# lukifer23/Matrix0

Hardware: AMD Instinct MI355X
Metric: self-play games/sec at 800 sims/move, ResNet-24 53M; 1/2/4/8 MI355X (higher is better)
Workload: dtype f16

## Files before the change

### include/m0_engine.h

```cpp
#ifndef M0_ENGINE_H
#define M0_ENGINE_H

#include <stddef.h>
#include <stdint.h>

#ifdef __cplusplus
extern "C" {
#endif

#define M0_OK 0
#define M0_ERR_INVALID (-1)
#define M0_ERR_UNSUPPORTED (-2)
#define M0_ERR_HIP (-3)
#define M0_ERR_STATE (-4)
#define M0_ERR_NONFINITE (-5)

#define M0_POLICY_SIZE 4672
#define M0_PLANES 19

#define M0_ACT_RELU 1
#define M0_ACT_SILU 2
#define M0_ACT_LEAKY 3

#define M0_SSL_PIECE 1
// ... 109 lines not shown
typedef struct m0_selfplay_stats {
    uint64_t steps, evals, sims, plies, games_finished, games_started;
    double ms_total, ms_net, ms_tree, ms_host;
    uint64_t arena_overflows;
    uint64_t ssl_dropped;
    uint64_t evals_cached;
    int active_games;
    uint64_t rows_tail;
} m0_selfplay_stats;

typedef struct m0_game_record {
    int game_index, moves, resigned, resigner , draw, total_plies ;
    float result;
    float avg_policy_entropy, avg_sims;
    double secs;
    const float* s;
    const float* pi;
    const float* z;
    const uint8_t* legal_mask;
    const float* search_values;
    const uint16_t* played;
    const float* ssl;
    void* owner;
    const char* start_fen;
} m0_game_record;

m0_selfplay* m0_selfplay_create(m0_net* net, const m0_selfplay_cfg* cfg);
void m0_selfplay_destroy(m0_selfplay* sp);
int m0_selfplay_step(m0_selfplay* sp, int steps);
int m0_selfplay_stats_get(m0_selfplay* sp, m0_selfplay_stats* out);
int m0_selfplay_poll(m0_selfplay* sp, m0_game_record* out);
void m0_game_record_free(m0_game_record* rec);
int m0_selfplay_running(m0_selfplay* sp);
int m0_selfplay_set_openings(m0_selfplay* sp, const char* const* fens, int n);
int m0_selfplay_ext_select(m0_selfplay* sp, int* rows, float* planes, int max_rows);
int m0_selfplay_ext_expand(m0_selfplay* sp, const float* logits, const float* values, int rows);
int m0_selfplay_last_batch_nhwc(m0_selfplay* sp, uint16_t* nhwc, int max_rows, int* rows);

m0_selfplay* m0_arena_create(m0_net* net_a, m0_net* net_b, const m0_selfplay_cfg* cfg);
m0_selfplay* m0_arena_create_ext(const m0_selfplay_cfg* cfg);
int m0_arena_ext_select(m0_selfplay* sp, int* rows_a, int* rows_b, float* planes_a, float* planes_b, int max_rows);
int m0_arena_ext_expand(m0_selfplay* sp, const float* logits_a, const float* values_a, int rows_a, const float* logits_b,
                        const float* values_b, int rows_b);
int m0_arena_choose_move(const int32_t* visits, int n, double temp, int ply, int temp_plies, double u);
int m0_san_legal_fen(const char* fen, uint16_t* moves, char* san, int* nlegal);
int m0_san_game(const uint16_t* moves, int n, char* out, int cap);
int m0_san_game_fen(const char* fen, const uint16_t* moves, int n, char* out, int cap);
int m0_fen_after(const char* fen, const char* const* ucis, int n, char* fen_out, int cap);

int m0_search_begin(m0_selfplay* sp, int g, const char* fen, int sims, int dirichlet, int game_uid);
int m0_search_select(m0_selfplay* sp, int* rows, float* planes, int max_rows);
int m0_search_expand(m0_selfplay* sp, const float* logits, const float* values, int rows);
int m0_search_result(m0_selfplay* sp, int g, int* nchild, int32_t* child_n, uint16_t* child_mv, int32_t* child_idx,
                     double* child_prior, double* child_q, double* root_q, int* root_n, int* finished);
int m0_search_advance(m0_selfplay* sp, int g, int slot, int sims, int dirichlet);


#define M0_AN_MAX_LINES 8
#define M0_AN_MAX_PV    16
typedef struct m0_analysis_opts { int multipv, pv_len, dirichlet; } m0_analysis_opts;
typedef struct m0_analysis_line {
    uint16_t move; int32_t policy_index; int32_t visits; float prior; double q;
    int32_t pv_len; uint16_t pv[M0_AN_MAX_PV];
} m0_analysis_line;
typedef struct m0_analysis_result {
    int64_t id; int32_t status;
    int32_t nlegal, overflow, sims, root_n; uint64_t evals;
    float value;
    double root_q; int32_t nlines; m0_analysis_line lines[M0_AN_MAX_LINES];
    int32_t tb_dtm;
    int32_t line_dtm[M0_AN_MAX_LINES];
} m0_analysis_result;
m0_selfplay* m0_analysis_create(m0_net* net, const m0_selfplay_cfg* cfg, const m0_analysis_opts* opts);
m0_selfplay* m0_analysis_create_ext(const m0_selfplay_cfg* cfg, const m0_analysis_opts* opts);
int m0_analysis_submit(m0_selfplay* sp, const char* fen, const char* const* ucis, int n_moves, int sims, int64_t id);
int m0_analysis_step(m0_selfplay* sp, int steps);
int m0_analysis_ext_select(m0_selfplay* sp, int* rows, float* planes, int max_rows);
int m0_analysis_ext_expand(m0_selfplay* sp, const float* logits, const float* values, int rows);
int m0_analysis_poll(m0_selfplay* sp, m0_analysis_result* out);
int m0_analysis_pending(m0_selfplay* sp);
size_t m0_analysis_result_size(void);

#define M0_DECODE_OK 0
#define M0_DECODE_PIECE_VALUE 1
#define M0_DECODE_SQUARE_CLASH 2
#define M0_DECODE_KINGS 3
#define M0_DECODE_PAWN_RANK 4
#define M0_DECODE_NOT_UNIFORM 5
#define M0_DECODE_FLAG_VALUE 6
#define M0_DECODE_CASTLING 7
#define M0_DECODE_COUNTER 8
#define M0_DECODE_OPPONENT_IN_CHECK 9
#define M0_DECODE_TOO_MANY_MOVES 10
#define M0_DECODE_MASK_MISMATCH 11
#define M0_DECODE_HALFMOVE_SATURATED 1
#define M0_DECODE_FULLMOVE_SATURATED 2
#define M0_DECODE_EP_FROM_MASK 4
#define M0_DECODE_NO_MASK 8
int m0_decode_planes(int hip_device, const float* planes, const uint8_t* mask, int n, int32_t* status, int32_t* flags,
                     int32_t* nlegal, char* fens, int fen_stride);
int m0_analysis_submit_planes(m0_selfplay* sp, const float* planes, const uint8_t* mask, int n, int sims, const int64_t* ids,
                              int32_t* status, int32_t* flags);
int m0_analysis_keep_visits(m0_selfplay* sp, int on);
int m0_analysis_poll_visits(m0_selfplay* sp, m0_analysis_result* out, int32_t* nchild, int32_t* policy_idx, int32_t* visits,
                            int cap);

typedef struct m0_tb m0_tb;
m0_tb* m0_tb_build(int hip_device, int max_men);
m0_tb* m0_tb_build_signatures(int hip_device, const char* const* sigs, int n);
m0_tb* m0_tb_load(const char* path);
int m0_tb_save(const m0_tb* tb, const char* path);
void m0_tb_destroy(m0_tb* tb);
int m0_tb_max_men(const m0_tb* tb);
int m0_tb_table(const m0_tb* tb, const char* sig, const uint8_t** bytes, size_t* n);
int m0_tb_table_info(const m0_tb* tb, int i, char* sig8, int* maxd, int* sweeps, double* build_ms);
int m0_tb_probe_fens(const m0_tb* tb, const char* const* fens, int n, uint8_t* hit, int8_t* wdl, int16_t* dtm);
int m0_selfplay_set_tablebase(m0_selfplay* sp, const m0_tb* tb, int max_pieces);
uint64_t m0_selfplay_tb_adjudications(m0_selfplay* sp);
int m0_selfplay_set_search_tablebase(m0_selfplay* sp, const m0_tb* tb, int max_pieces);
uint64_t m0_selfplay_tb_leaves(m0_selfplay* sp);
int m0_tb_root_lines(const m0_tb* tb, const char* fen, int multipv, int pv_len, m0_analysis_result* out);

int m0_sample_move_index(const int32_t* visits, int n, double temperature, double u);
int m0_playout_cap(int sims, double frac, double u);
double m0_temperature_for(int fullmove_number, double t_start, double t_end, int t_moves);
int m0_rules_probe(const m0_selfplay_cfg* cfg, const char* fen, const char* const* ucis, int n, int* flags, float* result);

int m0_san_pattern(const char* token, uint32_t* pattern);
#define M0_MOVE_UCI 0
#define M0_MOVE_RAW 1
int m0_move_pattern(int kind, const char* uci, uint32_t raw, uint32_t* pattern);
#define M0_REPLAY_OK 0
#define M0_REPLAY_ILLEGAL 1
#define M0_REPLAY_AMBIGUOUS 2
#define M0_REPLAY_TOO_LONG 3
#define M0_REPLAY_END_CHECKMATE 1
#define M0_REPLAY_END_STALEMATE 2
#define M0_REPLAY_END_INSUFFICIENT 4
#define M0_REPLAY_END_WHITE_TO_MOVE 8
int m0_replay_games(int hip_device, const char* const* start_fens, const uint32_t* patterns, const int32_t* offsets, int n_games,
                    int max_plies, int max_positions_per_launch, int32_t* plies, int32_t* status, int32_t* end_flags,
                    uint16_t* moves, int32_t* policy_idx, int32_t* nlegal, int8_t* turn, float* planes, uint8_t* mask, float* ssl);

#ifdef __cplusplus
}
#endif
#include "m0_analysis_live.h"
#include "m0_score.h"
#include "m0_ssl_score.h"
#include "m0_gumbel.h"
#include "m0_augment.h"
#include "m0_proof.h"
#include "m0_rowpack.h"
#endif
```

### matrix0_amd/_abi.py

```python
from __future__ import annotations

import ctypes as C
from ctypes import POINTER as P

M0_OK = 0
M0_ERR_INVALID = -1
M0_ERR_UNSUPPORTED = -2
M0_ERR_HIP = -3
M0_ERR_STATE = -4
M0_ERR_NONFINITE = -5
POLICY_SIZE = 4672
ACT = {"relu": 1, "silu": 2, "leaky_relu": 3}
SSL_BITS = {"piece": 1, "threat": 2, "pin": 4, "fork": 8, "control": 16}
AN_MAX_LINES, AN_MAX_PV = 8, 16
DECODE_STATUS = {0: "ok", 1: "piece_value", 2: "square_clash", 3: "kings", 4: "pawn_rank", 5: "not_uniform", 6: "flag_value",
                 7: "castling", 8: "counter", 9: "opponent_in_check", 10: "too_many_moves", 11: "mask_mismatch"}
DECODE_OK, DECODE_MASK_MISMATCH = 0, 11
HALFMOVE_SATURATED, FULLMOVE_SATURATED, EP_FROM_MASK, NO_MASK = 1, 2, 4, 8
REPLAY_STATUS = {0: "ok", 1: "illegal", 2: "ambiguous", 3: "too_long"}
REPLAY_END_BITS = {"checkmate": 1, "stalemate": 2, "insufficient": 4, "white_to_move": 8}
MOVE_UCI, MOVE_RAW = 0, 1
SCORE_MASK = {"legal": 0, "target": 1, "none": 2}
SCORE_COLS = 8
SCORE_COLUMNS = ("policy_loss", "entropy", "value_loss", "rank", "support_mass", "support_size", "value", "flags")
# ... 106 lines not shown
STRUCTS = {"m0_net_cfg": NetCfg, "m0_selfplay_cfg": SelfplayCfg, "m0_selfplay_stats": SelfplayStats,
           "m0_game_record": GameRecord, "m0_analysis_opts": AnalysisOpts, "m0_analysis_line": AnalysisLine,
           "m0_analysis_result": AnalysisResult}

_cfg, _res, _pi32 = P(SelfplayCfg), P(AnalysisResult), P(i32)
_select = (i32, [vp, _pi32, vp, i32])
_expand = (i32, [vp, vp, vp, i32])
_attach = (i32, [vp, vp, i32])
FUNCTIONS = {
    "m0_last_error": (cstr, []),
    "m0_version": (cstr, []),
    "m0_device_count": (i32, []),
    "m0_net_create": (vp, [P(NetCfg), i32]),
    "m0_net_destroy": (None, [vp]),
    "m0_net_load_weight": (i32, [vp, cstr, vp, i32, P(i64), i32]),
    "m0_net_finalize": (i32, [vp]),
    "m0_net_infer": (i32, [vp, vp, i32, vp, vp, vp]),
    "m0_net_tap_info": (i32, [vp, _pi32, _pi32]),
    "m0_net_infer_tap": (i32, [vp, vp, i32, i32, vp, vp, vp, vp, vp, _pi32]),
    "m0_net_ssl_channels": (i32, [vp]),
    "m0_net_param_count": (i64, [vp]),
    "m0_net_flops_per_position": (f64, [vp, i32]),
    "m0_net_bench_forward": (i32, [vp, i32, i32, i32, P(f32)]),
    "m0_net_profile_enable": (i32, [vp, i32]),
    "m0_net_profile_get": (i32, [vp, P(f64), P(f64), P(i64), i32]),
    "m0_net_profile_get_tail": (i32, [vp, P(f64), P(i64)]),
    "m0_dist_unique_id": (i32, [vp]),
    "m0_dist_create": (vp, [i32, i32, cstr, i32]),
    "m0_dist_destroy": (None, [vp]),
    "m0_dist_rank": (i32, [vp]),
    "m0_dist_world": (i32, [vp]),
    "m0_net_broadcast_weights": (i32, [vp, vp, i32]),
    "m0_encode_fens": (i32, [i32, cstrs, i32, vp, vp, vp, vp, vp]),
    "m0_encode_fens_nhwc": (i32, [i32, cstrs, i32, vp]),
    "m0_decode_move_fen": (i32, [i32, cstr, i32, cstr]),
    "m0_ssl_targets_fens": (i32, [i32, cstrs, i32, vp]),
    "m0_move_to_index_fen": (i32, [i32, cstr, cstr, _pi32]),
    "m0_selfplay_create": (vp, [vp, _cfg]),
    "m0_selfplay_destroy": (None, [vp]),
    "m0_selfplay_step": (i32, [vp, i32]),
    "m0_selfplay_stats_get": (i32, [vp, P(SelfplayStats)]),
    "m0_selfplay_poll": (i32, [vp, P(GameRecord)]),
    "m0_game_record_free": (None, [P(GameRecord)]),
    "m0_selfplay_running": (i32, [vp]),
    "m0_selfplay_set_openings": (i32, [vp, cstrs, i32]),
    "m0_selfplay_ext_select": _select,
    "m0_selfplay_ext_expand": _expand,
    "m0_selfplay_last_batch_nhwc": (i32, [vp, vp, i32, _pi32]),
    "m0_arena_create": (vp, [vp, vp, _cfg]),
    "m0_arena_create_ext": (vp, [_cfg]),
    "m0_arena_ext_select": (i32, [vp, _pi32, _pi32, vp, vp, i32]),
    "m0_arena_ext_expand": (i32, [vp, vp, vp, i32, vp, vp, i32]),
    "m0_arena_choose_move": (i32, [vp, i32, f64, i32, i32, f64]),
    "m0_san_legal_fen": (i32, [cstr, vp, vp, _pi32]),
    "m0_san_game": (i32, [vp, i32, cstr, i32]),
    "m0_san_game_fen": (i32, [cstr, vp, i32, cstr, i32]),
    "m0_fen_after": (i32, [cstr, cstrs, i32, cstr, i32]),
    "m0_search_begin": (i32, [vp, i32, cstr, i32, i32, i32]),
    "m0_search_select": _select,
    "m0_search_expand": _expand,
    "m0_search_result": (i32, [vp, i32, _pi32, vp, vp, vp, vp, vp, P(f64), _pi32, _pi32]),
    "m0_search_advance": (i32, [vp, i32, i32, i32, i32]),
    "m0_analysis_create": (vp, [vp, _cfg, P(AnalysisOpts)]),
    "m0_analysis_create_ext": (vp, [_cfg, P(AnalysisOpts)]),
    "m0_analysis_submit": (i32, [vp, cstr, cstrs, i32, i32, i64]),
    "m0_analysis_step": (i32, [vp, i32]),
    "m0_analysis_ext_select": _select,
    "m0_analysis_ext_expand": _expand,
    "m0_analysis_poll": (i32, [vp, _res]),
    "m0_analysis_pending": (i32, [vp]),
    "m0_analysis_result_size": (C.c_size_t, []),
    "m0_decode_planes": (i32, [i32, vp, vp, i32, vp, vp, vp, cstr, i32]),
    "m0_analysis_submit_planes": (i32, [vp, vp, vp, i32, i32, vp, vp, vp]),
    "m0_analysis_keep_visits": (i32, [vp, i32]),
    "m0_analysis_poll_visits": (i32, [vp, _res, _pi32, vp, vp, i32]),
    "m0_tb_build": (vp, [i32, i32]),
    "m0_tb_build_signatures": (vp, [i32, cstrs, i32]),
    "m0_tb_load": (vp, [cstr]),
    "m0_tb_save": (i32, [vp, cstr]),
    "m0_tb_destroy": (None, [vp]),
    "m0_tb_max_men": (i32, [vp]),
    "m0_tb_table": (i32, [vp, cstr, P(P(u8)), P(C.c_size_t)]),
    "m0_tb_table_info": (i32, [vp, i32, cstr, _pi32, _pi32, P(f64)]),
    "m0_tb_probe_fens": (i32, [vp, cstrs, i32, vp, vp, vp]),
    "m0_selfplay_set_tablebase": _attach,
    "m0_selfplay_tb_adjudications": (u64, [vp]),
    "m0_selfplay_set_search_tablebase": _attach,
    "m0_selfplay_tb_leaves": (u64, [vp]),
    "m0_tb_root_lines": (i32, [vp, cstr, i32, i32, _res]),
    "m0_sample_move_index": (i32, [vp, i32, f64, f64]),
    "m0_playout_cap": (i32, [i32, f64, f64]),
    "m0_temperature_for": (f64, [i32, f64, f64, i32]),
    "m0_rules_probe": (i32, [_cfg, cstr, cstrs, i32, _pi32, P(f32)]),
    "m0_san_pattern": (i32, [cstr, P(u32)]),
    "m0_move_pattern": (i32, [i32, cstr, u32, P(u32)]),
    "m0_replay_games": (i32, [i32, cstrs, vp, vp, i32, i32, i32] + [vp] * 10),
}

LIVE_FUNCTIONS = {
    "m0_analysis_submit_keep": (i32, [vp, cstr, cstrs, i32, i32, i64]),
    "m0_analysis_peek": (i32, [vp, i64, _res]),
    "m0_analysis_stop": (i32, [vp, i64]),
    "m0_analysis_continue": (i32, [vp, i64, cstrs, i32, i32, i64, i32, _pi32]),
    "m0_analysis_release": (i32, [vp, i64]),
    "m0_analysis_held": (i32, [vp]),
}

SCORE_STRUCTS = {"m0_score_opts": ScoreOpts}
SCORE_FUNCTIONS = {
    "m0_score_rows": (i32, [i32, vp, vp, vp, vp, vp, i32, P(ScoreOpts), vp]),
    "m0_net_score": (i32, [vp, vp, vp, vp, vp, i32, P(ScoreOpts), vp]),
    "m0_score_bench": (i32, [i32, i32, i32, P(f32), P(f64)]),
}

SSL_SCORE_FUNCTIONS = {
    "m0_ssl_score_rows": (i32, [i32, vp, i32, vp, vp, i32, vp]),
    "m0_net_score_ssl": (i32, [vp, vp, vp, vp, vp, vp, i32, P(ScoreOpts), vp, vp]),
    "m0_ssl_targets_planes": (i32, [i32, vp, i32, vp, vp]),
    "m0_ssl_score_bench": (i32, [i32, i32, i32, i32, i32, P(f32), P(f64)]),
}

GUMBEL_STRUCTS = {"m0_gumbel_cfg": GumbelCfg}
GUMBEL_FUNCTIONS = {
    "m0_selfplay_set_gumbel": (i32, [vp, P(GumbelCfg)]),
    "m0_search_gumbel_result": (i32, [vp, i32, _pi32, P(f64), vp, vp, _pi32]),
    "m0_gumbel_schedule": (i32, [i32, i32, vp, vp]),
    "m0_gumbel_improve": (i32, [i32, vp, vp, vp, vp, f64, P(GumbelCfg), vp, P(f64), _pi32]),
}

AUGMENT_FUNCTIONS = {
    "m0_augment_rows": (i32, [i32, vp, i32, vp, vp, vp, i32, vp, vp, vp]),
    "m0_net_score_aug": (i32, [vp, vp, vp, vp, vp, vp, i32, P(ScoreOpts), vp]),
    "m0_augment_bench": (i32, [i32, i32, i32, P(f32), P(f64)]),
}

PROOF_STRUCTS = {"m0_proof_lines": ProofLines}
PROOF_FUNCTIONS = {
    "m0_selfplay_set_proof": (i32, [vp, i32]),
    "m0_search_proof_result": (i32, [vp, i32, _pi32, _pi32, vp, vp, _pi32]),
    "m0_analysis_last_proof": (i32, [vp, P(ProofLines)]),
    "m0_proof_combine": (i32, [i32, vp, vp, i32, _pi32, _pi32]),
}

ROWPACK_STRUCTS = {"m0_rowpack_pos": RowpackPos, "m0_rowpack_arrays": RowpackArrays}
ROWPACK_FUNCTIONS = {
    "m0_rowpack_pack": (i32, [i32, vp, vp, vp, vp, i32, P(RowpackArrays), vp]),
    "m0_rowpack_unpack": (i32, [i32, P(RowpackArrays), vp, vp, vp, vp]),
    "m0_rowpack_pack_host": (i32, [vp, vp, vp, vp, i32, P(RowpackArrays), vp]),
    "m0_rowpack_unpack_host": (i32, [P(RowpackArrays), vp, vp, vp, vp]),
    "m0_net_score_packed": (i32, [vp, P(RowpackArrays), P(ScoreOpts), vp]),
    "m0_rowpack_bench": (i32, [i32, i32, i32, P(f32), P(f32), P(f64)]),
}


def bind(L) -> list:
    missing = []
    for name, (restype, argtypes) in (list(FUNCTIONS.items()) + list(LIVE_FUNCTIONS.items()) + list(SCORE_FUNCTIONS.items()) +
                                      list(SSL_SCORE_FUNCTIONS.items()) + list(GUMBEL_FUNCTIONS.items()) +
                                      list(AUGMENT_FUNCTIONS.items()) + list(PROOF_FUNCTIONS.items()) +
                                      list(ROWPACK_FUNCTIONS.items())):
        fn = getattr(L, name, None)
        if fn is None:
            missing.append(name)
        else:
            fn.restype, fn.argtypes = restype, argtypes
    return missing
```

### matrix0_amd/backend.py

```python
from __future__ import annotations

import ctypes as C
import threading
from typing import Dict, Optional, Tuple

import numpy as np

from . import _abi, _lib


def resolve_mask_mode(pi: np.ndarray, legal_mask, mask_mode: Optional[str]) -> str:
    if mask_mode is not None:
        if mask_mode not in _abi.SCORE_MASK:
            raise ValueError(f"mask_mode must be one of {sorted(_abi.SCORE_MASK)} or None, got {mask_mode!r}")
        return mask_mode
    if legal_mask is not None:
        return "legal"
    return "none" if bool(((np.asarray(pi) > 0).sum(axis=1) == 1).all()) else "target"


class NonFiniteScore(ValueError):

    def __init__(self, msg: str, rows: np.ndarray, ssl_rows: Optional[np.ndarray] = None):
        super().__init__(msg)
# ... 36 lines not shown
        b.load_state_dict(sd)
        return b

    @classmethod
    def from_checkpoint(cls, model_cfg: dict, ckpt_path: str, device_index: int = 0) -> "M0Backend":
        import torch
        state = torch.load(ckpt_path, map_location="cpu", weights_only=False)
        sd = state
        if isinstance(state, dict):
            for key in ("model_ema", "model", "model_state_dict"):
                if key in state and isinstance(state[key], dict):
                    sd = state[key]
                    break
        return cls.from_state_dict(model_cfg, sd, device_index)

    def infer_np(self, arr: np.ndarray) -> Tuple[np.ndarray, np.ndarray]:
        p, v, _ = self._infer(arr, False)
        return p, v

    def infer_np_ssl(self, arr: np.ndarray):
        return self._infer(arr, True)

    def tap_info(self) -> Tuple[int, int]:
        steps, width = C.c_int(0), C.c_int(0)
        _lib.check(self._L.m0_net_tap_info(self._h, C.byref(steps), C.byref(width)), "m0_net_tap_info")
        return steps.value, width.value

    def infer_tap(self, arr: np.ndarray, step: int):
        return self._infer(arr, True, int(step))

    def _infer(self, arr: np.ndarray, want_ssl: bool, tap_step: Optional[int] = None):
        if not self._finalized:
            raise RuntimeError("weights not loaded")
        a = np.asarray(arr)
        if a.ndim == 3:
            a = a[None]
        if a.ndim != 4 or a.shape[1:] != (self._cfg.planes, 8, 8):
            raise ValueError(f"expected input [B,{self._cfg.planes},8,8], got {a.shape}")
        a = np.ascontiguousarray(a, dtype=np.float32)
        B = a.shape[0]
        pol = np.empty((B, _lib.POLICY_SIZE), dtype=np.float32)
        val = np.empty((B,), dtype=np.float32)
        sslc = self._L.m0_net_ssl_channels(self._h)
        ssl = np.empty((B, sslc, 8, 8), dtype=np.float32) if (want_ssl and sslc > 0) else None
        if tap_step is None:
            _lib.check(self._L.m0_net_infer(self._h, _lib.ptr(a), B, _lib.ptr(pol), _lib.ptr(val), _lib.ptr(ssl)), "m0_net_infer")
        else:
            width = self.tap_info()[1]
            stream = np.empty((B, 64, width), dtype=np.float32)
            second = np.empty((B, 64, width), dtype=np.float32)
            has_second = C.c_int(0)
            _lib.check(self._L.m0_net_infer_tap(self._h, _lib.ptr(a), B, tap_step, _lib.ptr(pol), _lib.ptr(val), _lib.ptr(ssl),
                                                _lib.ptr(stream), _lib.ptr(second), C.byref(has_second)), "m0_net_infer_tap")
        out = None
        if ssl is not None:
            out, off = {}, 0
            for t in self.ssl_tasks:
                n = _lib.SSL_CH[t]
                out[t] = ssl[:, off:off + n]
                off += n
        if tap_step is not None:
            return pol, val, out, stream, (second if has_second.value else None)
        return pol, val, out

    def _score_inputs(self, s, pi, z, legal_mask):
        if not self._finalized:
            raise RuntimeError("weights not loaded")
        a = np.ascontiguousarray(s, dtype=np.float32)
        if a.ndim != 4 or a.shape[1:] != (self._cfg.planes, 8, 8):
            raise ValueError(f"expected input [B,{self._cfg.planes},8,8], got {a.shape}")
        B = a.shape[0]
        pi = np.ascontiguousarray(pi, dtype=np.float32)
        z = np.ascontiguousarray(np.asarray(z).reshape(-1), dtype=np.float32)
        if pi.shape != (B, _lib.POLICY_SIZE) or z.shape != (B,):
            raise ValueError(f"expected pi [{B},{_lib.POLICY_SIZE}] and z [{B}], got {pi.shape} and {z.shape}")
        if legal_mask is not None:
            legal_mask = np.ascontiguousarray(np.asarray(legal_mask).reshape(B, -1), dtype=np.uint8)
            if legal_mask.shape != pi.shape:
                raise ValueError(f"expected legal_mask [{B},{_lib.POLICY_SIZE}], got {legal_mask.shape}")
        return a, pi, z, legal_mask

    def score(self, s: Optional[np.ndarray] = None, pi: Optional[np.ndarray] = None, z: Optional[np.ndarray] = None,
              legal_mask: Optional[np.ndarray] = None, *, mask_mode: Optional[str] = None, label_smoothing: float = 0.0,
              value_loss: str = "mse", huber_delta: float = 1.0, augment=None, packed=None) -> np.ndarray:
        if packed is not None:
            return self._score_packed(packed, mask_mode, label_smoothing, value_loss, huber_delta, s, pi, z, legal_mask, augment)
        if s is None or pi is None or z is None:
            raise ValueError("score needs s, pi and z, or packed rows")
        a, pi, z, legal_mask = self._score_inputs(s, pi, z, legal_mask)
        B = a.shape[0]
        opts = score_opts(resolve_mask_mode(pi, legal_mask, mask_mode), label_smoothing, value_loss, huber_delta)
        rows = np.empty((B, _abi.SCORE_COLS), dtype=np.float32)
        if augment is None:
            call = "m0_net_score"
            rc = self._L.m0_net_score(self._h, _lib.ptr(a), _lib.ptr(pi), _lib.ptr(z), _lib.ptr(legal_mask), B, C.byref(opts),
                                      _lib.ptr(rows))
        else:
            from .encoding import augment_kinds
            call = "m0_net_score_aug"
            kinds = augment_kinds(augment, B)
            rc = self._L.m0_net_score_aug(self._h, _lib.ptr(a), _lib.ptr(pi), _lib.ptr(z), _lib.ptr(legal_mask), _lib.ptr(kinds), B,
                                          C.byref(opts), _lib.ptr(rows))
        if rc == _lib.M0_ERR_NONFINITE:
            raise NonFiniteScore(f"{call} failed ({rc}): {_lib.last_error()}", rows)
        _lib.check(rc, call)
        return rows

    def _score_packed(self, packed, mask_mode, label_smoothing, value_loss, huber_delta, *dense) -> np.ndarray:
        if not self._finalized:
            raise RuntimeError("weights not loaded")
        if any(d is not None for d in dense):
            raise ValueError("packed rows come instead of s, pi, z and legal_mask, and are not augmented")
        from .rowpack import mask_mode_of
        opts = score_opts(resolve_mask_mode(None, None, mask_mode_of(packed, mask_mode)), label_smoothing, value_loss, huber_delta)
        rows = np.empty((packed.n, _abi.SCORE_COLS), dtype=np.float32)
        arrays = packed.c_arrays()
        rc = self._L.m0_net_score_packed(self._h, C.byref(arrays), C.byref(opts), _lib.ptr(rows))
        if rc == _lib.M0_ERR_NONFINITE:
            raise NonFiniteScore(f"m0_net_score_packed failed ({rc}): {_lib.last_error()}", rows)
        _lib.check(rc, "m0_net_score_packed")
        return rows

    def score_ssl(self, s: np.ndarray, pi: np.ndarray, z: np.ndarray, legal_mask: Optional[np.ndarray] = None,
                  ssl_targets: Optional[np.ndarray] = None, *, mask_mode: Optional[str] = None, label_smoothing: float = 0.0,
                  value_loss: str = "mse", huber_delta: float = 1.0) -> Tuple[np.ndarray, np.ndarray]:
        a, pi, z, legal_mask = self._score_inputs(s, pi, z, legal_mask)
        B = a.shape[0]
        if ssl_targets is not None:
            ssl_targets = np.ascontiguousarray(ssl_targets, dtype=np.float32)
            if ssl_targets.size != B * 17 * 64 or ssl_targets.shape[:2] != (B, 17):
                raise ValueError(f"expected ssl_targets [{B},17,8,8], got {ssl_targets.shape}")
        opts = score_opts(resolve_mask_mode(pi, legal_mask, mask_mode), label_smoothing, value_loss, huber_delta)
        rows = np.empty((B, _abi.SCORE_COLS), dtype=np.float32)
        ssl_rows = np.empty((B, _abi.SSL_SCORE_COLS), dtype=np.float32)
        rc = self._L.m0_net_score_ssl(self._h, _lib.ptr(a), _lib.ptr(pi), _lib.ptr(z), _lib.ptr(legal_mask), _lib.ptr(ssl_targets),
                                      B, C.byref(opts), _lib.ptr(rows), _lib.ptr(ssl_rows))
        if rc == _lib.M0_ERR_NONFINITE:
            raise NonFiniteScore(f"m0_net_score_ssl failed ({rc}): {_lib.last_error()}", rows, ssl_rows)
        _lib.check(rc, "m0_net_score_ssl")
        return rows, ssl_rows

    def param_count(self) -> int:
        return int(self._L.m0_net_param_count(self._h))

    def flops_per_position(self, with_ssl: bool = False) -> float:
        return float(self._L.m0_net_flops_per_position(self._h, int(with_ssl)))

    def bench_forward(self, batch: int, iters: int, with_ssl: bool = False) -> float:
        ms = C.c_float(0)
        _lib.check(self._L.m0_net_bench_forward(self._h, int(batch), int(iters), int(with_ssl), C.byref(ms)),
                   "m0_net_bench_forward")
        return float(ms.value)

    def profile_enable(self, on: bool = True) -> None:
        _lib.check(self._L.m0_net_profile_enable(self._h, int(on)), "m0_net_profile_enable")

    def profile_get(self, reset: bool = False):
        ms, fl, n = C.c_double(0), C.c_double(0), C.c_int64(0)
        tms, tn = C.c_double(0), C.c_int64(0)
        _lib.check(self._L.m0_net_profile_get_tail(self._h, C.byref(tms), C.byref(tn)), "m0_net_profile_get_tail")
        self.last_tail_profile = (tms.value, tn.value)
        _lib.check(self._L.m0_net_profile_get(self._h, C.byref(ms), C.byref(fl), C.byref(n), int(reset)), "m0_net_profile_get")
        return ms.value, fl.value, n.value

    @property
    def handle(self):
        return self._h

    def close(self):
        if getattr(self, "_h", None):
            self._L.m0_net_destroy(self._h)
            self._h = None

    def __del__(self):
        try:
            self.close()
        except Exception:
            pass
```

### matrix0_amd/csrc/capi_net.hip

```cpp
#include <hip/hip_runtime.h>
#include <limits.h>
#include <math.h>
#include <string.h>
#include <mutex>
#include <string>
#include <vector>
#include "../../include/m0_engine.h"
#include "net.h"
#include "capi_common.h"
#include "score_core.h"
#include "score_kernels.h"
#include "ssl_score_core.h"
#include "ssl_score_kernels.h"
#include "augment_kernels.h"

thread_local std::string g_m0_last_error;

void m0_set_error(const std::string& s) { g_m0_last_error = s; }

struct m0_net {
    Net* net = nullptr;
    int device = 0;
    hipStream_t stream = nullptr;
    std::mutex mu;
// ... 272 lines not shown
        M0_HIP(hs, hipMemcpyAsync(n->score_pi_dev, pi, cells * 4, hipMemcpyHostToDevice, n->stream));
        M0_HIP(hs, hipMemcpyAsync(n->score_z_dev, z, (size_t)B * 4, hipMemcpyHostToDevice, n->stream));
        if (masked) M0_HIP(hs, hipMemcpyAsync(n->score_mask_dev, legal_mask, cells, hipMemcpyHostToDevice, n->stream));
    }
    if (ssl_rows && ssl_targets)
        M0_HIP(hs, hipMemcpyAsync(n->ssl_targets_dev, ssl_targets, (size_t)B * m0ssl::TARGET_CH * 64 * 4, hipMemcpyHostToDevice, n->stream));
    if (augmented) M0_HIP(hs, hipMemcpyAsync(n->aug_kinds_dev, kinds, (size_t)B, hipMemcpyHostToDevice, n->stream));
    if (!hs.ok()) return m0_hip_error(hs, "H2D copy");
    const float* planes_in = n->planes_dev;
    const float* pi_in = n->score_pi_dev;
    const uint8_t* mask_in = masked ? n->score_mask_dev : nullptr;
    if (augmented) {
        if (!M0_HIP(hs, launch_augment_rows(planes_in, pi_in, mask_in, n->aug_kinds_dev, M0_AUG_NONE, B, n->net->cfg().planes,
                                            n->aug_planes_dev, n->aug_pi_dev, masked ? n->aug_mask_dev : nullptr, n->stream)))
            return m0_hip_error(hs, "augment kernel");
        planes_in = n->aug_planes_dev;
        pi_in = n->aug_pi_dev;
        if (masked) mask_in = n->aug_mask_dev;
    }
    std::string err;
    rc = n->net->forward(planes_in, nullptr, B, n->logits_dev, n->value_dev, ssl_rows ? n->ssl_dev : nullptr, n->stream, err);
    if (rc != M0_OK) { m0_set_error(err); return rc; }
    M0_HIP(hs, launch_score_rows(n->logits_dev, n->value_dev, pi_in, n->score_z_dev, mask_in, B, *opts, n->score_rows_dev, n->stream));
    M0_HIP(hs, hipMemcpyAsync(rows, n->score_rows_dev, (size_t)B * M0_SCORE_COLS * 4, hipMemcpyDeviceToHost, n->stream));
    if (ssl_rows) {
        M0_HIP(hs, launch_ssl_score(n->ssl_dev, tasks, n->planes_dev, ssl_targets ? n->ssl_targets_dev : nullptr, B, n->ssl_rows_dev,
                                    n->stream));
        M0_HIP(hs, hipMemcpyAsync(ssl_rows, n->ssl_rows_dev, (size_t)B * M0_SSL_SCORE_COLS * 4, hipMemcpyDeviceToHost, n->stream));
    }
    if (!M0_HIP(hs, hipStreamSynchronize(n->stream))) return m0_hip_error(hs, "forward and score failed");
    for (int b = 0; b < B; ++b)
        if (((int)rows[(size_t)b * M0_SCORE_COLS + 7] & M0_SCORE_FLAG_NONFINITE) ||
            (ssl_rows && ((int)ssl_rows[(size_t)b * M0_SSL_SCORE_COLS + 15] & M0_SSL_SCORE_FLAG_NONFINITE))) {
            m0_set_error("network produced non-finite outputs (row " + std::to_string(b) + ")");
            return M0_ERR_NONFINITE;
        }
    return M0_OK;
}

int m0_net_score(m0_net* n, const float* planes, const float* pi, const float* z, const uint8_t* legal_mask, int B,
                 const m0_score_opts* opts, float* rows) {
    return net_score(n, planes, pi, z, legal_mask, nullptr, nullptr, false, B, opts, rows, nullptr);
}

int m0_net_score_packed(m0_net* n, const m0_rowpack_arrays* in, const m0_score_opts* opts, float* rows) {
    if (!in || !in->pos || !in->z || in->n <= 0 || in->n > INT_MAX) { m0_set_error("invalid argument"); return M0_ERR_INVALID; }
    return net_score(n, nullptr, nullptr, in->z, nullptr, nullptr, nullptr, false, (int)in->n, opts, rows, nullptr, in);
}

int m0_net_score_aug(m0_net* n, const float* planes, const float* pi, const float* z, const uint8_t* legal_mask, const uint8_t* kinds,
                     int B, const m0_score_opts* opts, float* rows) {
    return net_score(n, planes, pi, z, legal_mask, nullptr, kinds, true, B, opts, rows, nullptr);
}

int m0_net_score_ssl(m0_net* n, const float* planes, const float* pi, const float* z, const uint8_t* legal_mask,
                     const float* ssl_targets, int B, const m0_score_opts* opts, float* rows, float* ssl_rows) {
    if (!ssl_rows) { m0_set_error("null argument"); return M0_ERR_INVALID; }
    return net_score(n, planes, pi, z, legal_mask, ssl_targets, nullptr, false, B, opts, rows, ssl_rows);
}

int m0_net_tap_info(const m0_net* n, int* steps, int* width) {
    if (!n || !steps || !width) { m0_set_error("null argument"); return M0_ERR_INVALID; }
    *steps = n->net->tap_steps();
    *width = n->net->trunk_width();
    return M0_OK;
}

int m0_net_infer_tap(m0_net* n, const float* planes, int B, int step, float* policy, float* value, float* ssl, float* stream,
                     float* second, int* has_second) {
    if (!n || !planes || !policy || !value || !stream || !second || !has_second) {
        m0_set_error("null argument");
        return M0_ERR_INVALID;
    }
    if (B <= 0) { m0_set_error("batch must be positive"); return M0_ERR_INVALID; }
    if (step < 0 || step >= n->net->tap_steps()) { m0_set_error("tap step out of range"); return M0_ERR_INVALID; }
    std::lock_guard<std::mutex> lk(n->mu);
    n->net->set_tap(step);
    const int rc = infer_locked(n, planes, B, policy, value, ssl, stream, second, has_second);
    n->net->set_tap(-1);
    return rc;
}

int m0_net_ssl_channels(const m0_net* n) { return n ? n->net->ssl_channels_total() : 0; }
int64_t m0_net_param_count(const m0_net* n) { return n ? (int64_t)n->net->param_count() : 0; }
double m0_net_flops_per_position(const m0_net* n, int with_ssl) { return n ? n->net->flops_per_position(with_ssl != 0) : 0.0; }

int m0_net_profile_enable(m0_net* n, int on) {
    if (!n) { m0_set_error("net is null"); return M0_ERR_INVALID; }
    std::lock_guard<std::mutex> lk(n->mu);
    n->net->set_profile(on != 0);
    return M0_OK;
}

int m0_net_profile_get(m0_net* n, double* conv_ms, double* conv_flop, int64_t* launches, int reset) {
    if (!n) { m0_set_error("net is null"); return M0_ERR_INVALID; }
    std::lock_guard<std::mutex> lk(n->mu);
    if (conv_ms) *conv_ms = n->net->prof_conv_ms();
    if (conv_flop) *conv_flop = n->net->prof_conv_flop();
    if (launches) *launches = n->net->prof_conv_launches();
    if (reset) n->net->reset_profile();
    return M0_OK;
}

int m0_net_profile_get_tail(m0_net* n, double* tail_ms, int64_t* tail_launches) {
    if (!n) { m0_set_error("net is null"); return M0_ERR_INVALID; }
    std::lock_guard<std::mutex> lk(n->mu);
    if (tail_ms) *tail_ms = n->net->prof_tail_ms();
    if (tail_launches) *tail_launches = n->net->prof_tail_launches();
    return M0_OK;
}

int m0_net_bench_forward(m0_net* n, int B, int iters, int with_ssl, float* ms_per_forward) {
    if (!n || !ms_per_forward || B <= 0 || iters <= 0) { m0_set_error("invalid argument"); return M0_ERR_INVALID; }
    std::lock_guard<std::mutex> lk(n->mu);
    HipStatus& hs = n->net->hip();
    if (!M0_HIP(hs, hipSetDevice(n->device))) return m0_hip_error(hs);
    int rc = ensure_io(n, B);
    if (rc != M0_OK) return rc;
    std::string err;
    if (!(with_ssl & 2)) {
        const int P = n->net->cfg().planes;
        std::vector<float> h((size_t)B * P * 64, 0.f);
        uint64_t s = 0x9E3779B97F4A7C15ull;
        for (size_t i = 0; i < h.size(); ++i) {
            s ^= s << 13; s ^= s >> 7; s ^= s << 17;
            int p = (int)((i / 64) % P);
            if (p < 12) h[i] = ((s >> 20) % 100) < 8 ? 1.f : 0.f;
            else h[i] = (float)((((i / 64 / P) * 7 + p) % 10) / 10.0);
        }
        if (!M0_HIP(hs, hipMemcpy(n->planes_dev, h.data(), h.size() * 4, hipMemcpyHostToDevice))) return m0_hip_error(hs, "H2D copy");
    }
    float* ssl = ((with_ssl & 1) && n->net->ssl_channels_total() > 0) ? n->ssl_dev : nullptr;
    rc = n->net->forward(n->planes_dev, nullptr, B, n->logits_dev, n->value_dev, ssl, n->stream, err);
    if (rc != M0_OK) { m0_set_error(err); return rc; }
    struct Events {
        hipEvent_t e0 = nullptr, e1 = nullptr;
        ~Events() { if (e0) (void)hipEventDestroy(e0); if (e1) (void)hipEventDestroy(e1); }
    } ev;
    M0_HIP(hs, hipEventCreate(&ev.e0)); M0_HIP(hs, hipEventCreate(&ev.e1));
    M0_HIP(hs, hipEventRecord(ev.e0, n->stream));
    for (int i = 0; i < iters && hs.ok(); ++i) {
        rc = n->net->forward(n->planes_dev, nullptr, B, n->logits_dev, n->value_dev, ssl, n->stream, err);
        if (rc != M0_OK) { m0_set_error(err); return rc; }
    }
    M0_HIP(hs, hipEventRecord(ev.e1, n->stream));
    M0_HIP(hs, hipEventSynchronize(ev.e1));
    float ms = 0.f;
    if (!M0_HIP(hs, hipEventElapsedTime(&ms, ev.e0, ev.e1))) return m0_hip_error(hs, "bench forward failed");
    *ms_per_forward = ms / iters;
    n->net->harvest_profile();
    return M0_OK;
}

}
```

### matrix0_amd/csrc/capi_selfplay.hip

```cpp
#include <string.h>
#include <algorithm>
#include <memory>
#include <vector>
#include "selfplay_engine.h"

using namespace m0;

static void fill_tree_cfg(const m0_selfplay_cfg& c, bool match, TreeCfg& t) {
    t.fpu_reduction = c.fpu_reduction; t.draw_penalty = c.draw_penalty; t.virtual_loss = c.virtual_loss;
    t.selection_jitter = c.selection_jitter; t.cpuct = c.cpuct; t.cpuct_start = c.cpuct_start; t.cpuct_end = c.cpuct_end;
    t.cpuct_plies = c.cpuct_plies; t.use_c_base = c.use_c_base; t.cpuct_c_base = c.cpuct_c_base; t.cpuct_c_init = c.cpuct_c_init;
    t.dirichlet_alpha = c.dirichlet_alpha; t.dirichlet_frac = c.dirichlet_frac; t.legal_softmax = c.legal_softmax;
    t.enable_entropy_noise = c.enable_entropy_noise; t.no_instant_backtrack = c.no_instant_backtrack;
    t.virtual_loss_active = c.virtual_loss_active; t.leaves_per_step = c.inference_batch_size;
    t.tt_merge = c.tt_merge; t.raw_legal_priors = c.raw_legal_priors; t.max_children = c.max_children;
    t.min_child_prior = c.min_child_prior;
    t.gumbel = 0;
    t.gumbel_cfg = m0_gumbel_cfg{0, 0.0, 0.0};
    t.proof = 0;
    t.eval_cache = ((match ? c.arena_eval_cache : c.eval_cache) && c.legal_softmax && !c.raw_legal_priors && !c.tt_merge) ? 1 : 0;
}

static bool alloc_tree_arenas(m0_selfplay* sp) {
    const m0_selfplay_cfg& c = sp->cfg;
    long want = c.arena_nodes > 0 ? c.arena_nodes : (long)(c.num_simulations * 1.3 + 64) * 96;
    if (want < 4096) want = 4096;
    sp->cap = (int)want;
    const size_t N = (size_t)sp->G * 2 * sp->cap;
    TreeArrays& t = sp->d.t;
    t.cap = sp->cap;
    t.prior = dalloc<double>(sp, N); t.w = dalloc<double>(sp, N); t.q = dalloc<double>(sp, N);
    t.n = dalloc<int>(sp, N); t.vl = dalloc<int>(sp, N); t.cbase = dalloc<int>(sp, N);
    t.nch = dalloc<int16_t>(sp, N); t.mv = dalloc<uint16_t>(sp, N); t.midx = dalloc<uint16_t>(sp, N);
    sp->d.games = dalloc<GameDev>(sp, sp->G);
    const size_t LS = (size_t)sp->L + 1;
    sp->d.samples = dalloc<Sample>(sp, (size_t)sp->G * LS);
    sp->d.paths = dalloc<int>(sp, (size_t)sp->G * LS * M0_MAX_DEPTH);
    sp->d.leaf_moves = dalloc<uint16_t>(sp, (size_t)sp->G * LS * M0_MAX_CHILDREN);
    return hip_ok(sp, "hipMalloc failed for the search arenas (lower concurrent_games or arena_nodes)");
}

static bool alloc_position_tables(m0_selfplay* sp) {
    sp->d.tt_sides = 1;
    if (!sp->cfg.tt_merge) return true;
    const size_t LS = (size_t)sp->L + 1;
    int tc = 1024;
    while (tc < 2 * sp->cap) tc <<= 1;
    sp->d.tt_cap = tc;
    sp->d.tt_sides = sp->kind == EngineKind::Match ? 2 : 1;
    sp->d.search_nodes = (int)std::min<long>((long)sp->cfg.num_simulations * 48 + 4 * M0_MAX_CHILDREN, (long)sp->cap / 2);
    sp->d.epaths = dalloc<int>(sp, (size_t)sp->G * LS * M0_MAX_DEPTH);
    sp->d.tt_keys = dalloc<uint64_t>(sp, (size_t)sp->G * sp->d.tt_sides * tc);
    sp->d.tt_nodes = dalloc<int>(sp, (size_t)sp->G * sp->d.tt_sides * tc);
    return hip_ok(sp, "hipMalloc failed for the position tables (tt_merge): lower concurrent_games or arena_nodes");
}

static bool alloc_eval_cache(m0_selfplay* sp) {
    if (!sp->tc.eval_cache) return true;
    const size_t LS = (size_t)sp->L + 1;
    int entries = sp->cfg.eval_cache_entries > 0 ? sp->cfg.eval_cache_entries : 16384;
    int sets = 64;
    while (sets * 4 < entries) sets <<= 1;
    EvalCache& ec = sp->d.ec;
    ec.sets = sets;
    ec.sides = sp->kind == EngineKind::Match ? 2 : 1;
    const size_t entries_all = (size_t)sp->G * ec.sides * sets * 4;
    ec.keys = dalloc<uint64_t>(sp, entries_all);
    ec.stamps = dalloc<uint32_t>(sp, entries_all);
    ec.payload = dalloc<float>(sp, entries_all * M0_EC_WORDS);
    ec.hit_stage = dalloc<float>(sp, (size_t)sp->G * LS * M0_EC_WORDS);
    return hip_ok(sp, "hipMalloc failed for the evaluation cache: lower eval_cache_entries or concurrent_games");
}

static bool alloc_batch_buffers(m0_selfplay* sp) {
    const int nreg = sp->kind == EngineKind::Match ? 2 : 1;
    sp->d.hist = dalloc<uint64_t>(sp, (size_t)sp->G * M0_HIST_CAP);
    sp->d.results = dalloc<RootResult>(sp, sp->G);
    sp->d.row_counter = dalloc<int>(sp, 4);
    sp->d.x0 = dalloc<_Float16>(sp, (size_t)(nreg * sp->rows_max + 4) * 64 * 32);
    sp->logits_dev = dalloc<float>(sp, (size_t)nreg * sp->rows_max * 4672);
    sp->values_dev = dalloc<float>(sp, (size_t)nreg * sp->rows_max + 4);
    sp->d.net_row_base = sp->rows_max;
    if (sp->cfg.ssl_in_forward && sp->net && sp->net->ssl_channels_total() > 0)
        sp->ssl_dev = dalloc<float>(sp, (size_t)sp->rows_max * sp->net->ssl_channels_total() * 64);
    if (sp->cfg.ssl_targets) {
        sp->ssl_cap = sp->cfg.max_game_len > 0 ? sp->cfg.max_game_len + 1 : 513;
        sp->ssl_pos_dev = dalloc<Pos>(sp, sp->ssl_cap);
        sp->ssl_out_dev = dalloc<float>(sp, (size_t)sp->ssl_cap * 17 * 64);
        if (!hip_ok(sp, "hipMalloc failed for the SSL target staging buffers")) return false;
    }
    sp->ids_dev = dalloc<int>(sp, sp->G);
    sp->roots_dev = dalloc<int>(sp, sp->G);
    sp->d.logits = sp->logits_dev; sp->d.values = sp->values_dev;
    sp->d.G = sp->G; sp->d.L = sp->L;
    return hip_ok(sp, "hipMalloc failed for the batch buffers (lower concurrent_games or inference_batch_size)");
}

static bool make_tail_view(m0_selfplay* sp) {
    if (!(sp->cfg.tail_split && sp->net && sp->kind != EngineKind::Match && sp->net->cfg().channels > 256 && sp->net->cfg().channels <= 320 &&
          sp->rows_max >= 2048)) return true;
    M0_HIP(sp->hip, create_stream_cu_mask_env("M0_TAIL_CU_MASK", &sp->stream_tail));
    M0_HIP(sp->hip, hipEventCreateWithFlags(&sp->ev_sel, hipEventDisableTiming));
    M0_HIP(sp->hip, hipEventCreateWithFlags(&sp->ev_tail, hipEventDisableTiming));
    if (!hip_ok(sp, "hipStreamCreate / hipEventCreate failed (tail split)")) return false;
    sp->net_tail = sp->net->shared_view(sp->stream_tail);
    std::string werr;
    sp->half_split = sp->cfg.tail_split == 2;
    if (sp->net_tail->ensure_workspace(sp->half_split ? sp->rows_max / 2 + 1024 : 1023, werr) != M0_OK) {
        m0_set_error("tail split: " + werr);
        return false;
    }
    return true;
}

static bool build_engine(m0_selfplay* sp) {
    if (!alloc_tree_arenas(sp) || !alloc_position_tables(sp) || !alloc_eval_cache(sp) || !alloc_batch_buffers(sp)) return false;
    sp->hg.assign(sp->G, GameDev());
    for (auto& g : sp->hg) memset(&g, 0, sizeof(GameDev));
    sp->games.assign(sp->G, HostGame());
    sp->hres.resize(sp->G);
    sp->hsamples.resize((size_t)sp->G * (sp->L + 1));
    sp->prev_done.assign(sp->G, 0);
    for (hipEvent_t* e : {&sp->ev0, &sp->ev1, &sp->ev2, &sp->ev3}) M0_HIP(sp->hip, hipEventCreate(e));
    if (!hip_ok(sp, "hipEventCreate failed") || !make_tail_view(sp)) return false;
    std::string err;
    if (sp->net && sp->net->ensure_workspace(sp->rows_max, err) != M0_OK) { m0_set_error(err); return false; }
    if (sp->net && sp->net_b && sp->net_b->ensure_workspace(sp->rows_max, err) != M0_OK) { m0_set_error(err); return false; }
    M0_HIP(sp->hip, hipStreamSynchronize(sp->stream));
    return hip_ok(sp, "clearing the search arenas failed");
}

m0_selfplay* m0::engine_create(m0_net* nh, m0_net* nh_b, const m0_selfplay_cfg* cfg, EngineKind kind) {
    if (!cfg) { m0_set_error("cfg is null"); return nullptr; }
    if (cfg->concurrent_games <= 0 || cfg->inference_batch_size <= 0 || cfg->num_simulations <= 0) {
        m0_set_error("concurrent_games, inference_batch_size and num_simulations must be positive");
        return nullptr;
    }
    int ndev = 0;
    if (hipGetDeviceCount(&ndev) != hipSuccess || ndev <= 0) { m0_set_error("no HIP device available (no CPU fallback)"); return nullptr; }
    std::unique_ptr<m0_selfplay, decltype(&m0_selfplay_destroy)> owner(new m0_selfplay(), &m0_selfplay_destroy);
    m0_selfplay* sp = owner.get();
    sp->cfg = *cfg;
    sp->nethandle = nh;
    sp->nethandle_b = nh_b;
    sp->net = m0_net_impl(nh);
    sp->net_b = m0_net_impl(nh_b);
    sp->kind = kind;
    const bool match = kind == EngineKind::Match;
    sp->cfg.arena_mode = match ? 1 : 0;
    if (match) sp->cfg.eval_cache = 0;
    else { sp->cfg.arena_eval_cache = 0; sp->cfg.arena_paired_openings = 0; }
    fill_tree_cfg(sp->cfg, match, sp->tc);
    sp->device = nh ? m0_net_device(nh) : 0;
    if (nh) forward_gate_join(sp);
    M0_HIP(sp->hip, hipSetDevice(sp->device));
    if (nh) sp->stream = m0_net_stream(nh);
    else { M0_HIP(sp->hip, hipStreamCreateWithFlags(&sp->stream, hipStreamNonBlocking)); sp->own_stream = true; }
    sp->G = cfg->concurrent_games;
    sp->L = cfg->inference_batch_size;
    sp->rows_max = (sp->G * (sp->L + 1) + 3) & ~3;
    memset(&sp->stats, 0, sizeof(sp->stats));
    memset(&sp->d, 0, sizeof(sp->d));
    return hip_ok(sp, "engine stream") && build_engine(sp) ? owner.release() : nullptr;
}

static int leaf_planes(m0_selfplay* sp, int rows_a, float* planes_a, int rows_b, float* planes_b) {
    sync_games_d2h(sp);
    if (!M0_HIP(sp->hip, hipMemcpy(sp->hsamples.data(), sp->d.samples, sizeof(Sample) * (size_t)sp->G * (sp->L + 1), hipMemcpyDeviceToHost)))
        return m0_hip_error(sp->hip, "device sync failed");
    const int base = sp->d.net_row_base;
    for (int g = 0; g < sp->G; ++g) {
        if (!sp->hg[g].active) continue;
        for (int s = 0; s < sp->hg[g].nsamples; ++s) {
            const Sample& smp = sp->hsamples[(size_t)g * (sp->L + 1) + s];
            if (!sample_owns_row(smp.kind) || smp.row < 0) continue;
            if (smp.row < rows_a) encode_planes_f32(smp.pos, planes_a + (size_t)smp.row * 19 * 64);
            else if (smp.row >= base && smp.row < base + rows_b) encode_planes_f32(smp.pos, planes_b + (size_t)(smp.row - base) * 19 * 64);
        }
    }
    return M0_OK;
}

static void upload_eval(m0_selfplay* sp, size_t row_base, const float* logits, const float* values, int rows) {
    if (rows <= 0) return;
    M0_HIP(sp->hip, hipMemcpyAsync(sp->logits_dev + row_base * 4672, logits, (size_t)rows * 4672 * 4, hipMemcpyHostToDevice, sp->stream));
    M0_HIP(sp->hip, hipMemcpyAsync(sp->values_dev + row_base, values, (size_t)rows * 4, hipMemcpyHostToDevice, sp->stream));
}

int m0::ext_select_impl(m0_selfplay* sp, int* rows_a, int* rows_b, float* planes_a, float* planes_b, int max_rows) {
    if (sp->ext_pending) { m0_set_error("m0_selfplay_ext_expand outstanding"); return M0_ERR_STATE; }
    if (!planes_a || (sp->kind == EngineKind::Match && !planes_b) || max_rows < sp->G * (sp->L + 1)) {
        m0_set_error("planes buffer too small: concurrent_games * (inference_batch_size + 1) rows are required");
        return M0_ERR_INVALID;
    }
    int rc = refill(sp);
    if (rc != M0_OK) return rc;
    int r = 0;
    if ((rc = run_select(sp, &r)) != M0_OK) return rc;
    const int rb = sp->kind == EngineKind::Match ? sp->rows2[1] : 0;
    if (r > sp->rows_max || rb > sp->rows_max) { m0_set_error("row counter overflow"); return M0_ERR_STATE; }
    *rows_a = r;
    if (rows_b) *rows_b = rb;
    sp->last_rows = r;
    sp->last_rows_b = rb;
    sp->ext_pending = true;
    if (r + rb > 0) return leaf_planes(sp, r, planes_a, rb, planes_b);
    return M0_OK;
}

int m0::ext_expand_impl(m0_selfplay* sp, const float* logits_a, const float* values_a, int rows_a, const float* logits_b,
                           const float* values_b, int rows_b) {
    if (!sp->ext_pending) { m0_set_error("no m0_selfplay_ext_select outstanding"); return M0_ERR_STATE; }
    if (rows_a != sp->last_rows || rows_b != sp->last_rows_b) { m0_set_error("rows does not match the last select"); return M0_ERR_INVALID; }
    if ((rows_a > 0 && (!logits_a || !values_a)) || (rows_b > 0 && (!logits_b || !values_b))) { m0_set_error("null argument"); return M0_ERR_INVALID; }
    upload_eval(sp, 0, logits_a, values_a, rows_a);
    upload_eval(sp, (size_t)sp->d.net_row_base, logits_b, values_b, rows_b);
    sp->ext_pending = false;
    M0_HIP(sp->hip, hipEventRecord(sp->ev0, sp->stream)); M0_HIP(sp->hip, hipEventRecord(sp->ev1, sp->stream));
    return finish_step(sp, rows_a + rows_b, now_ms());
}

bool m0::kind_accepted(const m0_selfplay* sp, const char* what, unsigned kinds) {
    if (kinds & (1u << (int)sp->kind)) return true;
    static const char* const is_a[] = {"a self-play engine", "a match engine", "an analysis engine"};
    const char* only = kinds == KIND_SELFPLAY ? "self-play engines" : kinds == KIND_MATCH ? "match engines"
                     : kinds == KIND_ANALYSIS ? "analysis engines" : "self-play and match engines";
    m0_set_error(std::string(what) + ": " + only + " only, this is " + is_a[(int)sp->kind]);
    return false;
}

extern "C" {

m0_selfplay* m0_selfplay_create(m0_net* nh, const m0_selfplay_cfg* cfg) { return engine_create(nh, nullptr, cfg, EngineKind::SelfPlay); }

m0_selfplay* m0_arena_create(m0_net* net_a, m0_net* net_b, const m0_selfplay_cfg* cfg) {
    if (!net_a || !net_b) { m0_set_error("m0_arena_create needs two networks"); return nullptr; }
    if (m0_net_device(net_a) != m0_net_device(net_b)) { m0_set_error("both networks must live on the same HIP device"); return nullptr; }
    if (cfg && (cfg->ssl_in_forward || cfg->ssl_targets)) { m0_set_error("arena games carry no SSL outputs"); return nullptr; }
    return engine_create(net_a, net_b, cfg, EngineKind::Match);
}

m0_selfplay* m0_arena_create_ext(const m0_selfplay_cfg* cfg) {
    if (cfg && (cfg->ssl_in_forward || cfg->ssl_targets)) { m0_set_error("arena games carry no SSL outputs"); return nullptr; }
    return engine_create(nullptr, nullptr, cfg, EngineKind::Match);
}

void m0_selfplay_destroy(m0_selfplay* sp) {
    if (!sp) return;
    forward_gate_leave(sp);
    (void)hipSetDevice(sp->device);
    if (sp->stream) (void)hipStreamSynchronize(sp->stream);
    if (sp->stream_tail) (void)hipStreamSynchronize(sp->stream_tail);
    delete sp->net_tail;
    if (sp->ev_sel) (void)hipEventDestroy(sp->ev_sel);
    if (sp->ev_tail) (void)hipEventDestroy(sp->ev_tail);
    if (sp->stream_tail) (void)hipStreamDestroy(sp->stream_tail);
    for (void* p : sp->allocs) (void)hipFree(p);
    for (auto& r : sp->done_meta) delete (GameRecordOwner*)r.owner;
    delete sp->an;
    if (sp->ev0) { (void)hipEventDestroy(sp->ev0); (void)hipEventDestroy(sp->ev1); (void)hipEventDestroy(sp->ev2); (void)hipEventDestroy(sp->ev3); }
    if (sp->own_stream && sp->stream) (void)hipStreamDestroy(sp->stream);
    delete sp;
}

int m0_selfplay_set_openings(m0_selfplay* sp, const char* const* fens, int n) {
    if (!sp || n < 0 || (n > 0 && !fens)) { m0_set_error("invalid argument"); return M0_ERR_INVALID; }
    M0_ENGINE_CALL(sp, "m0_selfplay_set_openings", KIND_GAMES, false);
    if (sp->stats.games_started != 0) { m0_set_error("set the opening book before the first step"); return M0_ERR_STATE; }
    std::vector<Pos> book(n);
    for (int i = 0; i < n; ++i)
        if (!fens[i] || parse_fen(fens[i], book[i]) != 0) { m0_set_error(std::string("bad FEN at index ") + std::to_string(i)); return M0_ERR_INVALID; }
    sp->book.swap(book);
    sp->book_fens.assign(fens, fens + n);
    return M0_OK;
}

int m0_selfplay_ext_select(m0_selfplay* sp, int* rows, float* planes, int max_rows) {
    if (!sp || !rows) { m0_set_error("null argument"); return M0_ERR_INVALID; }
    M0_ENGINE_CALL(sp, "m0_selfplay_ext_select", KIND_SELFPLAY, true);
    return ext_select_impl(sp, rows, nullptr, planes, nullptr, max_rows);
}

int m0_selfplay_ext_expand(m0_selfplay* sp, const float* logits, const float* values, int rows) {
    M0_ENGINE_CALL(sp, "m0_selfplay_ext_expand", KIND_SELFPLAY, true);
    return ext_expand_impl(sp, logits, values, rows, nullptr, nullptr, 0);
}

int m0_arena_ext_select(m0_selfplay* sp, int* rows_a, int* rows_b, float* planes_a, float* planes_b, int max_rows) {
    if (!sp || !rows_a || !rows_b) { m0_set_error("null argument"); return M0_ERR_INVALID; }
    M0_ENGINE_CALL(sp, "m0_arena_ext_select", KIND_MATCH, true);
    return ext_select_impl(sp, rows_a, rows_b, planes_a, planes_b, max_rows);
}

int m0_arena_ext_expand(m0_selfplay* sp, const float* logits_a, const float* values_a, int rows_a, const float* logits_b,
                        const float* values_b, int rows_b) {
    M0_ENGINE_CALL(sp, "m0_arena_ext_expand", KIND_MATCH, true);
    return ext_expand_impl(sp, logits_a, values_a, rows_a, logits_b, values_b, rows_b);
}

int m0_selfplay_step(m0_selfplay* sp, int steps) {
    M0_ENGINE_CALL(sp, "m0_selfplay_step", KIND_GAMES, true);
    if (sp->ext_pending) { m0_set_error("m0_selfplay_ext_expand outstanding"); return M0_ERR_STATE; }
    int rc = refill(sp);
    for (int i = 0; i < steps && rc == M0_OK; ++i) {
        if (sp->stats.active_games == 0 && sp->stats.steps > 0) break;
        rc = one_step(sp);
    }
    return rc;
}

int m0_selfplay_stats_get(m0_selfplay* sp, m0_selfplay_stats* out) {
    if (!sp || !out) { m0_set_error("null argument"); return M0_ERR_INVALID; }
    M0_ENGINE_CALL(sp, "m0_selfplay_stats_get", KIND_ANY, false);
    *out = sp->stats;
    return M0_OK;
}

int m0_selfplay_poll(m0_selfplay* sp, m0_game_record* out) {
    if (!sp || !out) { m0_set_error("null argument"); return M0_ERR_INVALID; }
    M0_ENGINE_CALL(sp, "m0_selfplay_poll", KIND_GAMES, false);
    if (sp->done_meta.empty()) return 0;
    *out = sp->done_meta.front();
    sp->done_meta.pop_front();
    return 1;
}

void m0_game_record_free(m0_game_record* rec) {
    if (rec && rec->owner) { delete (GameRecordOwner*)rec->owner; rec->owner = nullptr; }
}

int m0_selfplay_running(m0_selfplay* sp) {
    M0_ENGINE_CALL_OR(0, sp, "m0_selfplay_running", KIND_ANY, false);
    if (sp->stats.games_started == 0) return 1;
    if (sp->stats.active_games > 0) return 1;
    return (sp->cfg.total_games <= 0 || sp->next_game < sp->cfg.total_games) ? 1 : 0;
}

int m0_search_begin(m0_selfplay* sp, int g, const char* fen, int sims, int dirichlet, int game_uid) {
    if (!sp || !fen || g < 0 || g >= sp->G || sims <= 0) { m0_set_error("invalid argument"); return M0_ERR_INVALID; }
// ... 97 lines not shown
```

### matrix0_amd/csrc/conv_epilogue.h

```cpp
#pragma once
#include "kernel_common.h"

typedef _Float16 half2v __attribute__((ext_vector_type(2)));

template <int ACT>
__device__ __forceinline__ float act_fast(float v) {
    if constexpr (ACT == ACT_RELU) return v > 0.f ? v : 0.f;
    else if constexpr (ACT == ACT_SILU) return v * __builtin_amdgcn_rcpf(1.f + __expf(-v));
    else if constexpr (ACT == ACT_LEAKY) return v > 0.f ? v : 0.05f * v;
    else if constexpr (ACT == ACT_SIGMOID) return __builtin_amdgcn_rcpf(1.f + __expf(-v));
    else if constexpr (ACT == ACT_TANH) return tanhf(v);
    else return v;
}
template <int NT>
__device__ __forceinline__ char* conv_stage_base(char* lds_wave, int lane) {
    return lds_wave + (4 * (lane >> 5) + (lane & 1)) * (NT * 64) + ((lane & 31) >> 1) * 4;
}

template <int NT, int MI, int NI>
__device__ __forceinline__ void conv_stage_tile(const float (&v)[16], char* wbase, int lane) {
    constexpr int ROWB = NT * 64;
    const bool odd = (lane & 1) != 0;
    static_for<0, 8>([&](auto rp_) __attribute__((always_inline)) {
        constexpr int r0 = 2 * decltype(rp_)::value;
        const float v0 = v[r0], v1 = v[r0 + 1];
        const float send = odd ? v0 : v1;
        const float recv = __builtin_bit_cast(
            float, __builtin_amdgcn_update_dpp(0, __builtin_bit_cast(int, send), 0xB1, 0xF, 0xF, true));
        const half2v h = {(_Float16)(odd ? recv : v0), (_Float16)(odd ? v1 : recv)};
        *reinterpret_cast<half2v*>(wbase + (MI * 32 + (r0 & 3) + 8 * (r0 >> 2)) * ROWB + NI * 64) = h;
    });
}

template <int NT, int FENCE_EVERY = 0>
__device__ __forceinline__ void conv_stage_flush(const GemmArgs& a, const char* lds_wave, int m0, int n0, int wm, int wn,
                                                 int lane) {
    constexpr int NCH = NT * 4;
    const uint32_t ldo2 = (uint32_t)a.ldo * 2u;
    char* out = reinterpret_cast<char*>(a.out) + ((size_t)(m0 + wm * 64) * a.ldo + n0 + wn * NT * 32) * 2;
    const int rows_valid = a.Mvalid - (m0 + wm * 64);
    int row = lane / NCH, ch = lane - row * NCH;
#pragma unroll
    for (int it = 0; it < NCH; ++it) {
        if (FENCE_EVERY > 0 && it % (FENCE_EVERY > 0 ? FENCE_EVERY : 1) == 0) asm volatile("" ::: "memory");
        const uint4 v = *reinterpret_cast<const uint4*>(lds_wave + (it * 64 + lane) * 16);
        if (row < rows_valid) *reinterpret_cast<uint4*>(out + ((uint32_t)row * ldo2 + (uint32_t)ch * 16u)) = v;
        ch += 64 % NCH; row += 64 / NCH;
        if (ch >= NCH) { ch -= NCH; row += 1; }
    }
}

__device__ __forceinline__ void gn16_mean_rstd(float s, float ss, float& mean, float& rstd) {
    mean = s * (1.f / 1024.f);
    float var = ss * (1.f / 1024.f) - mean * mean;
    var = var > 0.f ? var : 0.f;
    rstd = rsqrtf(var + 1e-5f);
}
__device__ __forceinline__ void gn16_affine(float mean, float rstd, const float& gamma, const float& beta, float& scale,
                                            float& shift) {
    scale = gamma * rstd;
    shift = beta - mean * scale;
}

template <int NI, int NT>
__device__ __forceinline__ void conv_gn_column(const float16v (&acc)[2][NT], const float* gamma, const float* beta, int col,
                                               float& scale, float& shift) {
    float s = 0.f, ss = 0.f;
    static_for<0, 2>([&](auto mi_) __attribute__((always_inline)) {
        const float16v av = acc[decltype(mi_)::value][NI];
        static_for<0, 16>([&](auto r_) __attribute__((always_inline)) { const float v = av[decltype(r_)::value]; s += v; ss += v * v; });
    });
#pragma unroll
    for (int o = 1; o <= 8; o <<= 1) { s += __shfl_xor(s, o); ss += __shfl_xor(ss, o); }
    s += __shfl_xor(s, 32); ss += __shfl_xor(ss, 32);
    float mean, rstd;
    gn16_mean_rstd(s, ss, mean, rstd);
    gn16_affine(mean, rstd, gamma[col], beta[col], scale, shift);
}

template <ConvEpi EPI, int ACT, int NT>
__device__ __forceinline__ void conv_tile_epilogue(float16v (&acc)[2][NT], const GemmArgs& a, char* lds_wave, int m0,
                                                   int n0, int wm, int wn, int lane, int out_col0 = 0) {
    const int half = lane >> 5;
    const int r31 = lane & 31;
    const int colbase = n0 + wn * NT * 32 + r31;
    char* wbase = conv_stage_base<NT>(lds_wave, lane);
    if constexpr (EPI == EPI_GN) {
        static_for<0, NT>([&](auto ni_) __attribute__((always_inline)) {
            constexpr int ni = decltype(ni_)::value;
            const int col = colbase + ni * 32;
            float g, sh;
            conv_gn_column<ni>(acc, a.gn_gamma, a.gn_beta, col, g, sh);
            static_for<0, 2>([&](auto mi_) __attribute__((always_inline)) {
                constexpr int mi = decltype(mi_)::value;
                float v[16];
                static_for<0, 16>([&](auto r_) __attribute__((always_inline)) {
                    constexpr int r = decltype(r_)::value;
                    v[r] = act_fast<ACT>(acc[mi][ni][r] * g + sh);
                });
                if (a.posenc != nullptr) {
                    static_for<0, 16>([&](auto r_) __attribute__((always_inline)) {
                        constexpr int r = decltype(r_)::value;
                        const int sq = mi * 32 + (r & 3) + 8 * (r >> 2) + 4 * half;
                        v[r] += a.posenc[(size_t)sq * a.N + col];
                    });
                }
                conv_stage_tile<NT, mi, ni>(v, wbase, lane);
            });
        });
        conv_stage_flush<NT>(a, lds_wave, m0, n0 - out_col0, wm, wn, lane);
    }
    if constexpr (EPI == EPI_PLAIN) {
        const float oscale = a.out_scale;
        const bool want_stats = a.out_stats != nullptr;
        float* stats = a.out_stats + ((size_t)(m0 / 64 + wm) * a.N + colbase) * 2;
        static_for<0, NT>([&](auto ni_) __attribute__((always_inline)) {
            constexpr int ni = decltype(ni_)::value;
            const float bias = a.bias != nullptr ? a.bias[colbase + ni * 32] : 0.f;
            float s = 0.f, ss = 0.f;
            static_for<0, 2>([&](auto mi_) __attribute__((always_inline)) {
                constexpr int mi = decltype(mi_)::value;
                float v[16];
                static_for<0, 16>([&](auto r_) __attribute__((always_inline)) {
                    constexpr int r = decltype(r_)::value;
                    v[r] = act_fast<ACT>(acc[mi][ni][r] + bias) * oscale;
                    s += v[r]; ss += v[r] * v[r];
                });
                conv_stage_tile<NT, mi, ni>(v, wbase, lane);
            });
            if (want_stats) {
                s += __shfl_xor(s, 32);
                ss += __shfl_xor(ss, 32);
                if (lane < 32) { stats[ni * 64] = s; stats[ni * 64 + 1] = ss; }
            }
        });
        conv_stage_flush<NT>(a, lds_wave, m0, n0, wm, wn, lane);
    }
    if constexpr (EPI == EPI_ELEMENT) {
        const int ldo = a.ldo;
        const int rowbase = m0 + wm * 64 + 4 * half;
        const int epi_act = a.epi_act;
        const float oscale = a.out_scale;
        const bool want_stats = a.out_stats != nullptr;
        const bool has_mul = a.mul != nullptr;
        const bool f32out = a.out_f32 != 0;
        static_for<0, NT>([&](auto ni_) __attribute__((always_inline)) {
            constexpr int ni = decltype(ni_)::value;
            const int col = colbase + ni * 32;
            const float bias = a.bias != nullptr ? a.bias[col] : 0.f;
            float s = 0.f, ss = 0.f;
            static_for<0, 2>([&](auto mi_) __attribute__((always_inline)) {
                constexpr int mi = decltype(mi_)::value;
                const float16v av = acc[mi][ni];
                static_for<0, 16>([&](auto r_) __attribute__((always_inline)) {
                    constexpr int r = decltype(r_)::value;
                    const int row = rowbase + mi * 32 + (r & 3) + 8 * (r >> 2);
                    float v = av[r] + bias;
                    if (epi_act != ACT_NONE) v = act_apply(v, epi_act);
                    if (has_mul) v *= (float)a.mul[(size_t)row * ldo + col];
                    v *= oscale;
                    s += v; ss += v * v;
                    if (row < a.Mvalid) {
                        if (f32out) reinterpret_cast<float*>(a.out)[(size_t)row * ldo + col] = v;
                        else reinterpret_cast<_Float16*>(a.out)[(size_t)row * ldo + col] = (_Float16)v;
                    }
                });
            });
            if (want_stats) {
                s += __shfl_xor(s, 32);
                ss += __shfl_xor(ss, 32);
                if (lane < 32) {
                    float* st = a.out_stats + ((size_t)(m0 / 64 + wm) * a.N + col) * 2;
                    st[0] = s; st[1] = ss;
                }
            }
        });
    }
}
```

### matrix0_amd/csrc/conv_gemm.hip

```cpp
#include "kernel_common.h"
#include "conv_epilogue.h"

template <int TAPS, int WN, int NT, int KC, ConvEpi EPI = EPI_ELEMENT, int ACT = ACT_NONE>
__global__ __launch_bounds__(256 * WN) void conv_gemm_kernel(GemmArgs a) {
    constexpr int NB = WN * NT * 32;
    constexpr int NTHR = 256 * WN;
    constexpr int AST = KC + 8;
    constexpr int APIX = (TAPS == 9) ? 100 : 64;
    constexpr int A_ELEMS = 4 * APIX * AST;
    constexpr int W_ELEMS = NB * AST;
    constexpr int A_PIECES = 4 * 64 * KC / 8;
    constexpr int W_PIECES = NB * KC / 8;
    constexpr int A_PER = (A_PIECES + NTHR - 1) / NTHR;
    constexpr int W_PER = (W_PIECES + NTHR - 1) / NTHR;
    constexpr int K8 = KC / 8;

    extern __shared__ __attribute__((aligned(16))) char smem[];
    _Float16* A_lds = reinterpret_cast<_Float16*>(smem);
    _Float16* W_lds = A_lds + A_ELEMS;

    const int tid = threadIdx.x;
    const int lane = tid & 63;
    const int wave = tid >> 6;
    const int wm = wave % 4;
    const int wn = wave / 4;
    const int m0 = blockIdx.x * 256;
    const int n0 = blockIdx.y * NB;
    const int Cin = a.Cin;
    const int nchunk = Cin / KC;
    const int Npad = a.Npad;

    if (TAPS == 9) {
        for (int i = tid; i < A_ELEMS / 8; i += NTHR)
            reinterpret_cast<uint4*>(A_lds)[i] = make_uint4(0, 0, 0, 0);
    }
    __syncthreads();

    float16v acc[2][NT];
    static_for<0, 2>([&](auto mi) __attribute__((always_inline)) {
        static_for<0, NT>([&](auto ni) __attribute__((always_inline)) {
            acc[decltype(mi)::value][decltype(ni)::value] = float16v{0.f, 0.f, 0.f, 0.f, 0.f, 0.f, 0.f, 0.f,
                                                                      0.f, 0.f, 0.f, 0.f, 0.f, 0.f, 0.f, 0.f};
        });
    });

    int apix[2];
#pragma unroll
    for (int mi = 0; mi < 2; ++mi) {
        int px = mi * 32 + (lane & 31);
        if (TAPS == 9) apix[mi] = wm * 100 + ((px >> 3) + 1) * 10 + (px & 7) + 1;
        else apix[mi] = wm * 64 + px;
    }
    const int khalf = 8 * (lane >> 5);

    uint4 areg[A_PER];
    uint4 wreg[W_PER];

    auto load_A = [&](int chunk) {
#pragma unroll
        for (int i = 0; i < A_PER; ++i) {
            int p = tid + i * NTHR;
            if (A_PIECES % NTHR == 0 || p < A_PIECES) {
                int row = p / K8, c8 = p % K8;
                areg[i] = *reinterpret_cast<const uint4*>(a.in + (size_t)(m0 + row) * Cin + chunk * KC + c8 * 8);
            }
        }
    };
    auto store_A = [&](int chunk) {
#pragma unroll
        for (int i = 0; i < A_PER; ++i) {
            int p = tid + i * NTHR;
            if (A_PIECES % NTHR == 0 || p < A_PIECES) {
                int row = p / K8, c8 = p % K8;
                int b = row >> 6, px = row & 63;
                uint4 v = areg[i];
                int pix = (TAPS == 9) ? (b * 100 + ((px >> 3) + 1) * 10 + (px & 7) + 1) : row;
                *reinterpret_cast<uint4*>(A_lds + pix * AST + c8 * 8) = v;
            }
        }
    };
    auto load_W = [&](int step) {
        int chunk = step / TAPS, tap = step % TAPS;
        const _Float16* src = a.w + ((size_t)(tap * nchunk + chunk) * Npad + n0) * KC;
#pragma unroll
        for (int i = 0; i < W_PER; ++i) {
            int p = tid + i * NTHR;
            if (W_PIECES % NTHR == 0 || p < W_PIECES)
                wreg[i] = *reinterpret_cast<const uint4*>(src + (size_t)p * 8);
        }
    };
    auto store_W = [&](int buf) {
#pragma unroll
        for (int i = 0; i < W_PER; ++i) {
            int p = tid + i * NTHR;
            if (W_PIECES % NTHR == 0 || p < W_PIECES) {
                int n = p / K8, k8 = p % K8;
                *reinterpret_cast<uint4*>(W_lds + buf * W_ELEMS + n * AST + k8 * 8) = wreg[i];
            }
        }
    };

    const int nsteps = nchunk * TAPS;
    load_A(0);
    load_W(0);
    for (int s = 0; s < nsteps; ++s) {
        const int chunk = s / TAPS, tap = s % TAPS;
        if (tap == 0) {
            if (s > 0) __syncthreads();
            store_A(chunk);
        }
        store_W(s & 1);
        __syncthreads();
        if (s + 1 < nsteps) {
            load_W(s + 1);
            if ((s + 1) % TAPS == 0) load_A((s + 1) / TAPS);
        }
        const int tapoff = (TAPS == 9) ? ((tap / 3 - 1) * 10 + (tap % 3 - 1)) : 0;
        const _Float16* Wb = W_lds + (s & 1) * W_ELEMS + (wn * NT * 32 + (lane & 31)) * AST + khalf;
        static_for<0, KC / 16>([&](auto kk_) __attribute__((always_inline)) {
            constexpr int kk = decltype(kk_)::value;
            half8 af0 = *reinterpret_cast<const half8*>(A_lds + (apix[0] + tapoff) * AST + kk * 16 + khalf);
            half8 af1 = *reinterpret_cast<const half8*>(A_lds + (apix[1] + tapoff) * AST + kk * 16 + khalf);
            static_for<0, NT>([&](auto ni_) __attribute__((always_inline)) {
                constexpr int ni = decltype(ni_)::value;
                half8 bf = *reinterpret_cast<const half8*>(Wb + ni * 32 * AST + kk * 16);
                acc[0][ni] = __builtin_amdgcn_mfma_f32_32x32x16_f16(af0, bf, acc[0][ni], 0, 0, 0);
                acc[1][ni] = __builtin_amdgcn_mfma_f32_32x32x16_f16(af1, bf, acc[1][ni], 0, 0, 0);
            });
        });
    }

    if constexpr (EPI == EPI_GN) {
        __syncthreads();
        GemmArgs o = a;
        int out_col0 = 0;
        if (a.out2 != nullptr && n0 + wn * NT * 32 >= a.nsplit) { o.out = a.out2; o.ldo = a.ldo2; out_col0 = a.nsplit; }
        conv_tile_epilogue<EPI_GN, ACT, NT>(acc, o, smem + wave * (64 * 64 * NT), m0, n0, wm, wn, lane, out_col0);
    } else {
        conv_tile_epilogue<EPI_ELEMENT, ACT_NONE, NT>(acc, a, smem, m0, n0, wm, wn, lane);
    }
}

template <int TAPS, int WN, int NT, int KC>
static size_t conv_gemm_lds() {
    constexpr int NB = WN * NT * 32;
    constexpr int AST = KC + 8;
    constexpr int APIX = (TAPS == 9) ? 100 : 64;
    const size_t main_loop = (size_t)(4 * APIX * AST + 2 * NB * AST) * 2 + 64;
    const size_t staging = (size_t)WN * 4 * 64 * 64 * NT;
    return main_loop > staging ? main_loop : staging;
}

template <int TAPS, int WN, int NT, int KC, ConvEpi EPI = EPI_ELEMENT, int ACT = ACT_NONE>
static hipError_t launch_conv_gemm_t(const GemmArgs& a, hipStream_t st) {
    constexpr int NB = WN * NT * 32;
    size_t lds = conv_gemm_lds<TAPS, WN, NT, KC>();
    static DeviceOnce once;
    hipError_t e = once.run([] {
        return hipFuncSetAttribute(reinterpret_cast<const void*>(&conv_gemm_kernel<TAPS, WN, NT, KC, EPI, ACT>),
                                   hipFuncAttributeMaxDynamicSharedMemorySize, 160 * 1024);
    });
    if (e != hipSuccess) return e;
    dim3 grid(a.Mrows / 256, a.Npad / NB);
    hipLaunchKernelGGL((conv_gemm_kernel<TAPS, WN, NT, KC, EPI, ACT>), grid, dim3(256 * WN), lds, st, a);
    return hipGetLastError();
}
template <int ACT>
static hipError_t launch_conv_gemm_gn(const GemmArgs& a, int taps, hipStream_t st) {
    if (a.bias != nullptr || a.mul != nullptr || a.out_stats != nullptr || a.out_f32 || a.out_scale != 1.f || a.Npad != a.N)
        return hipErrorInvalidValue;
    if (taps == 9) return a.Npad % 64 == 0 && a.out2 == nullptr ? launch_conv_gemm_t<9, 1, 2, 32, EPI_GN, ACT>(a, st) : hipErrorInvalidValue;
    if (a.posenc != nullptr) return hipErrorInvalidValue;
    if (a.out2 != nullptr) return a.Npad == 192 && a.nsplit == 64 ? launch_conv_gemm_t<1, 3, 2, 32, EPI_GN, ACT>(a, st) : hipErrorInvalidValue;
    if (a.Npad == 160) return launch_conv_gemm_t<1, 1, 5, 32, EPI_GN, ACT>(a, st);
    if (a.Npad == 128) return launch_conv_gemm_t<1, 2, 2, 32, EPI_GN, ACT>(a, st);
    if (a.Npad == 64) return launch_conv_gemm_t<1, 1, 2, 32, EPI_GN, ACT>(a, st);
    if (a.Npad == 32) return launch_conv_gemm_t<1, 1, 1, 32, EPI_GN, ACT>(a, st);
    return hipErrorInvalidValue;
}

hipError_t launch_conv_big(const GemmArgs& a, int taps, hipStream_t st);
hipError_t launch_conv_zs(const GemmArgs& a, hipStream_t st);

int conv_gemm_tile_n(int Cin, int Npad) {
    return (Npad % 320 == 0 && Cin % 64 == 0) ? 320 : 32;
}
int conv_gemm_kc(int Cin, int Npad) {
    return (Npad % 320 == 0 && Cin % 64 == 0) ? 64 : 32;
}

hipError_t launch_conv_gemm(const GemmArgs& a, int taps, hipStream_t st) {
    if (a.Mrows % 256 != 0 || a.Cin % 32 != 0 || a.Npad % 32 != 0) return hipErrorInvalidValue;
    const bool big = conv_gemm_tile_n(a.Cin, a.Npad) == 320;
    if (a.gn_gamma != nullptr && !big) {
        if (a.epi_act == ACT_SILU) return launch_conv_gemm_gn<ACT_SILU>(a, taps, st);
        if (a.epi_act == ACT_RELU) return launch_conv_gemm_gn<ACT_RELU>(a, taps, st);
        return hipErrorInvalidValue;
    }
    if (taps == 9) {
        if (big) {
            if (!a.w_pp) return hipErrorInvalidValue;
            return launch_conv_zs(a, st);
        }
        return launch_conv_gemm_t<9, 1, 1, 32>(a, st);
    } else if (taps == 1) {
        if (big) return a.w_pp ? hipErrorInvalidValue : launch_conv_big(a, 1, st);
        if (a.Mrows / 256 >= 256 && a.Npad % 64 == 0) return launch_conv_gemm_t<1, 1, 2, 32>(a, st);
        return launch_conv_gemm_t<1, 1, 1, 32>(a, st);
    }
    return hipErrorInvalidValue;
}
```

### matrix0_amd/csrc/net.h

```cpp
#pragma once
#include <hip/hip_runtime.h>
#include <stdint.h>
#include <map>
#include <string>
#include <vector>
#include "../../include/m0_engine.h"
#include "hip_check.h"
#include "net_kernels.h"

namespace net_pack { struct GemmShape; }

inline int ceil_to(int v, int m) { return (v + m - 1) / m * m; }

struct HostTensor {
    std::vector<float> data;
    std::vector<int64_t> shape;
};

struct PackedGemm {
    _Float16* w = nullptr;
    float* bias = nullptr;
    int taps = 1, Cin = 0, N = 0;
    bool pp = false;
};

struct NormParams {
    float* gamma = nullptr;
    float* beta = nullptr;
};

struct HostNorm { std::vector<float> gamma, beta; };

struct ResBlockW {
    PackedGemm conv1, conv2;
    NormParams bn1, bn2;
    float *se_w1 = nullptr, *se_b1 = nullptr, *se_w2 = nullptr, *se_b2 = nullptr;
    void* se_wf = nullptr;
    int se_hidden = 0;
};

struct AttnW {
    PackedGemm qkv, proj;
    NormParams ln;
    float* rel_bias = nullptr;
    void* blk_w = nullptr;
    _Float16* blk_bias = nullptr;
};

struct TowerLayer {
    int kind;
    int index;
    bool skip;
    int next_bn1 = -1;
};

struct SslHeadW {
    PackedGemm c0, c1;
    NormParams n;
    int out_ch = 0;
};

struct ConvNormOpts {
    const float* posenc = nullptr;
    const _Float16* res = nullptr;
    const NormParams* next_bn1 = nullptr;
};

class Net {
public:
    explicit Net(const m0_net_cfg& cfg, int device, hipStream_t stream);
    ~Net();
    Net* shared_view(hipStream_t stream) const;
    static const char* check_supported(const m0_net_cfg& cfg);
    int load(const char* name, const void* data, int dtype, const int64_t* shape, int ndim, std::string& err);
    int finalize(std::string& err);
    bool ready() const { return finalized_; }
    HipStatus& hip() { return *hip_; }
    const std::vector<void*>& device_buffers() const { return dev_allocs_; }
    const std::vector<size_t>& device_buffer_bytes() const { return dev_sizes_; }

    int forward(const float* planes_dev, const _Float16* nhwc_dev, int B, float* logits_dev, float* value_dev,
                float* ssl_dev, hipStream_t st, std::string& err);
    int ensure_workspace(int B, std::string& err);
    int ssl_channels_total() const;
    const m0_net_cfg& cfg() const { return cfg_; }
    size_t param_count() const { return nparams_; }
    double flops_per_position(bool with_ssl) const;
    _Float16* input_nhwc() { return X0_; }
    int tap_steps() const { return 3 + (int)tower_.size(); }
    int trunk_width() const { return Cp_; }
    void set_tap(int step) { tap_step_ = step; }
    const _Float16* tap_stream() const { return TAPX_; }
    const _Float16* tap_second() const { return TAPA_; }
    bool tap_has_second() const { return tap_second_; }
    void set_profile(bool on) { profile_ = on; }
    void harvest_profile();
    double prof_conv_ms() const { return prof_ms_; }
    double prof_conv_flop() const { return prof_flop_; }
    long prof_conv_launches() const { return prof_launches_; }
    void reset_profile() { prof_ms_ = 0; prof_flop_ = 0; prof_launches_ = 0; prof_tail_ms_ = 0; prof_tail_launches_ = 0; }
    double prof_tail_ms() const { return prof_tail_ms_; }
    long prof_tail_launches() const { return prof_tail_launches_; }

private:
    m0_net_cfg cfg_;
    int device_;
    hipStream_t stream_ = nullptr;
    HipStatus own_hip_, *hip_ = &own_hip_;
    struct Switches { bool fuse_tail = true, fuse_attn = true; int attn_grid = 0; } sw_;
    struct Plan {
        bool fuse_tail = false;
        bool fuse_attn = false;
        bool gn_small = false;
        int act = 0, vact = 0;
        int first_bn1 = -1;
    } plan_;
    bool finalized_ = false;
    size_t nparams_ = 0;
    std::map<std::string, HostTensor> sd_;
    std::vector<void*> dev_allocs_;
    std::vector<size_t> dev_sizes_;
    std::vector<void*> ws_allocs_;

    int C_ = 0, Cs_ = 0 ;
    int Cp_ = 0;
    PackedGemm stem_;
    NormParams stem_n_;
    float* posenc_ = nullptr;
    PackedGemm pst_, inter_;
    NormParams pst_n_, inter_n_;
    std::vector<ResBlockW> res_;
    std::vector<AttnW> att_;
    std::vector<TowerLayer> tower_;
    PackedGemm ph_conv_, pfc1_, pfc2_;
    PackedGemm hv_;
    NormParams hv_n_;
    NormParams ph_n_;
    float logit_scale_ = 1.f;
    PackedGemm vh0_, vh3_, vfc1_, vfc2_, vgate_, vfc3_;
    NormParams vh1_n_, vh4_n_;
    std::vector<SslHeadW> ssl_;
    uint64_t* mask_dev_ = nullptr;

    bool profile_ = false;
    std::vector<hipEvent_t> pev_;
    std::vector<double> pflop_;
    std::vector<char> ptail_;
    size_t pev_used_ = 0;
    double prof_ms_ = 0, prof_flop_ = 0, prof_tail_ms_ = 0;
    long prof_launches_ = 0, prof_tail_launches_ = 0;

    int wsB_ = 0, wsM_ = 0;
    _Float16 *X0_ = nullptr, *XA_ = nullptr, *XB_ = nullptr, *T1_ = nullptr, *T2_ = nullptr, *QKV_ = nullptr,
             *O_ = nullptr, *AA_ = nullptr;
    float *S1_ = nullptr, *S2_ = nullptr, *G_ = nullptr;
    _Float16 *PH_ = nullptr, *PH2_ = nullptr, *VH_ = nullptr, *VH2_ = nullptr, *F1_ = nullptr, *F2_ = nullptr,
             *F3_ = nullptr, *F4_ = nullptr, *SH_ = nullptr, *SH2_ = nullptr, *SO_ = nullptr;
    float* VAL_ = nullptr;
    float* SPK_ = nullptr;
    int tap_step_ = -1;
    bool tap_second_ = false;
    _Float16 *TAPX_ = nullptr, *TAPA_ = nullptr;

    const HostTensor* get(const std::string& k, std::string& err);
    const HostTensor* get(const std::string& k, size_t count, std::string& err);
    int upload_bytes(void*& dst, const void* src, size_t bytes, std::string& err);
    template <class P, class T>
    int upload(P*& dst, const std::vector<T>& v, std::string& err);
    int pack_gemm(PackedGemm& g, const std::string& wkey, const std::string& bkey, const net_pack::GemmShape& s, std::string& err,
                  std::vector<_Float16>* keep = nullptr);
    int upload_norm(NormParams& n, const std::string& prefix, int C_real, int C_pad, std::string& err, HostNorm* keep = nullptr);
    int pack_chess_features(std::string& err);
    int pack_se(ResBlockW& r, const std::string& prefix, std::string& err);
    int pack_attn(AttnW& a, bool skip, const std::string& prefix, std::string& err);
    int pack_joint_head(const std::vector<_Float16>& ph_w, const std::vector<_Float16>& vh_w, const HostNorm& ph_n,
                        const HostNorm& vh_n, std::string& err);
    int pack_ssl_heads(std::string& err);
    void make_plan();
    void* dalloc(size_t bytes, bool ws);
    const NormParams* bn1(int res_index) const { return res_index < 0 ? nullptr : &res_[res_index].bn1; }
    template <class Launch>
    hipError_t profiled(bool on, hipStream_t st, double flop, bool tail, Launch&& launch);
    hipError_t run_gemm(const PackedGemm& g, GemmArgs a, hipStream_t st);
    hipError_t conv_norm_act(const PackedGemm& g, const NormParams& n, const _Float16* in, _Float16* out, _Float16* scratch,
                             int Mrows, hipStream_t st, const ConvNormOpts& o = ConvNormOpts());
    hipError_t se_gate(const ResBlockW& r, const float* stats, int boards, hipStream_t st);
};
```

### matrix0_amd/csrc/net.hip

```cpp
#include "net.h"
#include <math.h>
#include <string.h>
#include <algorithm>
#include <stdlib.h>

const char* Net::check_supported(const m0_net_cfg& c) {
    if (!c.norm_group) return "HIP path supports norm='group' only (BatchNorm configs are not built)";
    if (!c.preact) return "HIP path supports preact=true only";
    if (c.channels % 32 != 0 || c.channels < 32 || c.channels > 384) return "channels must be a multiple of 32 in [32,384]";
    if (c.planes < 1 || c.planes > 32) return "planes must be in [1,32]";
    if (c.attention && (c.attention_heads <= 0 || c.channels % c.attention_heads != 0 ||
                        c.channels / c.attention_heads != 16))
        return "attention head_dim (channels/attention_heads) must be 16";
    if (c.activation != M0_ACT_SILU && c.activation != M0_ACT_RELU) return "activation must be silu or relu";
    if (c.blocks < 1) return "blocks must be >= 1";
    if (c.policy_factor_rank < 0) return "policy_factor_rank must be >= 0";
    if (c.self_supervised && c.ssl_tasks && (c.channels / 2) % 16 != 0) return "ssl heads need channels/2 % 16 == 0";
    return nullptr;
}

Net::Net(const m0_net_cfg& cfg, int device, hipStream_t stream) : cfg_(cfg), device_(device), stream_(stream) {
    auto off = [](const char* name) { const char* e = getenv(name); return e && e[0] == '0'; };
    sw_.fuse_tail = !off("M0_FUSE_TAIL");
    sw_.fuse_attn = !off("M0_FUSE_ATTN");
    if (const char* e = getenv("M0_ATTN_GRID")) sw_.attn_grid = std::max(0, atoi(e));
    C_ = cfg.channels;
    Cp_ = (C_ > 256 && C_ < 320) ? 320 : C_;
    Cs_ = ceil_to(std::max(16, C_ / 2), 32);
    int k = cfg.attention_every_k;
    int stride = std::max(1, cfg.infer_attention_stride);
    int att_seen = 0;
    for (int i = 0; i < cfg.blocks; ++i) {
        tower_.push_back({0, (int)res_.size(), false});
        res_.emplace_back();
        if (cfg.attention && k > 0 && (i % k) == (k - 1)) {
            ++att_seen;
            bool skip = stride > 1 && (att_seen % stride) != 0;
            tower_.push_back({1, (int)att_.size(), skip});
            att_.emplace_back();
        }
    }
}

Net* Net::shared_view(hipStream_t stream) const {
    Net* v = new Net(*this);
    v->stream_ = stream;
    v->dev_allocs_.clear(); v->dev_sizes_.clear();
    v->ws_allocs_.clear(); v->wsB_ = 0; v->wsM_ = 0;
    v->tap_step_ = -1; v->TAPX_ = v->TAPA_ = nullptr;
    v->sd_.clear();
    v->pev_.clear(); v->pflop_.clear(); v->ptail_.clear(); v->pev_used_ = 0; v->profile_ = false;
    v->prof_ms_ = v->prof_flop_ = v->prof_tail_ms_ = 0; v->prof_launches_ = v->prof_tail_launches_ = 0;
    return v;
}

Net::~Net() {
    for (hipEvent_t e : pev_) (void)hipEventDestroy(e);
    for (void* p : dev_allocs_) (void)hipFree(p);
    for (void* p : ws_allocs_) (void)hipFree(p);
}

void* Net::dalloc(size_t bytes, bool ws) {
    void* p = nullptr;
    if (bytes == 0) bytes = 16;
    if (!M0_HIP(*hip_, hipMalloc(&p, bytes))) return nullptr;
    (ws ? ws_allocs_ : dev_allocs_).push_back(p);
    if (!ws) dev_sizes_.push_back(bytes);
    M0_HIP(*hip_, hipMemsetAsync(p, 0, bytes, stream_));
    if (!ws) M0_HIP(*hip_, hipStreamSynchronize(stream_));
    return hip_->ok() ? p : nullptr;
}

int Net::ssl_channels_total() const {
    int n = 0;
    for (auto& h : ssl_) n += h.out_ch;
    return n;
}

double Net::flops_per_position(bool with_ssl) const {
    const double C = C_;
    double mac = 64.0 * cfg_.planes * 9 * C;
    if (cfg_.chess_features) mac += 64.0 * C * C * (cfg_.piece_square_tables ? 1 : 0) + 64.0 * C * C * 9;
    for (auto& L : tower_) {
        if (L.kind == 0) {
            mac += 2 * 64.0 * C * C * 9;
            if (cfg_.se) mac += 2.0 * C * res_[L.index].se_hidden;
        } else if (!L.skip) {
            mac += 64.0 * C * 3 * C + 64.0 * C * C;
            double nb = (cfg_.attention_unmasked_mix > 0.f && cfg_.attention_unmasked_mix < 1.f) ? 2.0 : 1.0;
            mac += 64.0 * 64.0 * C * (1.0 + nb);
        }
    }
    mac += 64.0 * C * 64;
    if (cfg_.policy_factor_rank > 0) mac += 4096.0 * cfg_.policy_factor_rank + (double)cfg_.policy_factor_rank * M0_POLICY_SIZE;
    else mac += 4096.0 * M0_POLICY_SIZE;
    mac += 64.0 * C * 128 + 64.0 * 128 * 128 + 8192.0 * 2 * C + 2.0 * C * C + C * C + C;
    if (with_ssl) for (auto& h : ssl_) mac += 64.0 * C * (C / 2) + 64.0 * (C / 2) * h.out_ch;
    return 2.0 * mac;
}

int Net::ensure_workspace(int B, std::string& err) {
    const int Bp = std::max(ceil_to(B, 4), wsB_);
    const int Mfc = std::max(ceil_to(B, 256), wsM_);
    const bool want_tap = tap_step_ >= 0;
    if (Bp <= wsB_ && Mfc <= wsM_ && (!want_tap || TAPX_)) return M0_OK;
    M0_HIP(*hip_, hipSetDevice(device_));
    M0_HIP(*hip_, hipDeviceSynchronize());
    for (void* p : ws_allocs_) M0_HIP(*hip_, hipFree(p));
    if (!hip_->ok()) { err = "workspace: " + hip_->message(); return M0_ERR_HIP; }
    ws_allocs_.clear();
    const size_t C = Cp_;
    const size_t nb = Bp, nh = std::max(Bp, Mfc);
    const size_t Cst = std::max<size_t>(C, 128);
    auto H = [&](size_t elems) { return (_Float16*)dalloc(elems * 2, true); };
    auto F = [&](size_t elems) { return (float*)dalloc(elems * 4, true); };
    X0_ = H(nb * 64 * 32);
    XA_ = H(nb * 64 * C); XB_ = H(nb * 64 * C); T1_ = H(nb * 64 * C); T2_ = H(nb * 64 * C); AA_ = H(nb * 64 * C);
    QKV_ = H(nb * 64 * 3 * C); O_ = H(nb * 64 * C);
    S1_ = F(nb * Cst * 2); S2_ = F(nb * Cst * 2); G_ = F(nb * Cst);
    PH_ = H(nh * 64 * 64); PH2_ = H(nh * 64 * 64);
    VH_ = H(nh * 64 * 128); VH2_ = H(nh * 64 * 128);
    const size_t rp = cfg_.policy_factor_rank > 0 ? ceil_to(cfg_.policy_factor_rank, 32) : 32;
    F1_ = H((size_t)Mfc * rp);
    F2_ = H((size_t)Mfc * ceil_to(2 * C_, 32)); F3_ = H((size_t)Mfc * ceil_to(C_, 32)); F4_ = H((size_t)Mfc * ceil_to(C_, 32));
    SH_ = H(nb * 64 * Cs_); SH2_ = H(nb * 64 * Cs_); SO_ = H(nb * 64 * 32);
    VAL_ = F((size_t)Mfc * 32);
    SPK_ = F((size_t)8 * Mfc * ceil_to(2 * C_, 32));
    TAPX_ = TAPA_ = nullptr;
    if (want_tap) { TAPX_ = H(nb * 64 * C); TAPA_ = H(nb * 64 * C); }
    M0_HIP(*hip_, hipStreamSynchronize(stream_));
    if (!M0_HIP(*hip_, hipGetLastError())) {
        err = "workspace hipMalloc / clear failed: " + hip_->message(); wsB_ = wsM_ = 0; return M0_ERR_HIP;
    }
    wsB_ = Bp; wsM_ = Mfc;
    return M0_OK;
}

static GemmArgs gemm_args(const PackedGemm& g, const _Float16* in, void* out, int Mrows, int epi_act = ACT_NONE) {
    GemmArgs a;
    memset(&a, 0, sizeof(a));
    a.in = in; a.w = g.w; a.out = out; a.bias = g.bias;
    a.Mrows = Mrows; a.Mvalid = Mrows; a.Cin = g.Cin; a.N = g.N; a.Npad = g.N; a.ldo = g.N;
    a.epi_act = epi_act; a.out_scale = 1.f; a.w_pp = g.pp ? 1 : 0;
    return a;
}

static EwArgs ew_args(const _Float16* t, _Float16* y, int C, int act) {
    EwArgs e;
    memset(&e, 0, sizeof(e));
    e.t = t; e.y = y; e.C = C; e.act = act;
    return e;
}
static void ew_next_bn1(EwArgs& e, const NormParams* next_bn1, _Float16* y2) {
    if (next_bn1) { e.y2 = y2; e.gn2_gamma = next_bn1->gamma; e.gn2_beta = next_bn1->beta; }
}

static double conv3x3_flop(const PackedGemm& g, int rows) { return 2.0 * (double)rows * (double)g.N * (double)g.Cin * 9.0; }

template <class Launch>
hipError_t Net::profiled(bool on, hipStream_t st, double flop, bool tail, Launch&& launch) {
    if (!on) return launch();
    if (pev_used_ + 2 > pev_.size()) {
        for (int i = 0; i < 2; ++i) { hipEvent_t e; if (!M0_HIP(*hip_, hipEventCreate(&e))) return hip_->code(); pev_.push_back(e); }
    }
    M0_HIP(*hip_, hipEventRecord(pev_[pev_used_], st));
    hipError_t rc = hip_->ok() ? launch() : hip_->code();
    if (rc == hipSuccess && !M0_HIP(*hip_, hipEventRecord(pev_[pev_used_ + 1], st))) rc = hip_->code();
    pev_used_ += 2;
    pflop_.push_back(flop);
    ptail_.push_back(tail ? 1 : 0);
    return rc;
}

hipError_t Net::run_gemm(const PackedGemm& g, GemmArgs a, hipStream_t st) {
    const bool big = conv_gemm_tile_n(g.Cin, g.N) == 320;
    const bool splitk = g.taps == 1 && big && g.Cin >= 4096 && (g.Cin >> 6) % 8 == 0 && !a.gn_gamma && !a.mul && !a.out_stats &&
                        !a.out_f32 && a.out_scale == 1.f && SPK_ != nullptr && (size_t)g.N <= (size_t)ceil_to(2 * C_, 32) &&
                        a.Mrows <= wsM_;
    return profiled(profile_ && g.taps == 9 && big, st, conv3x3_flop(g, a.Mvalid), false, [&]() -> hipError_t {
        if (!splitk) return launch_conv_gemm(a, g.taps, st);
        _Float16* out = (_Float16*)a.out;
        const int act = a.epi_act;
        a.out = SPK_; a.bias = nullptr; a.epi_act = ACT_NONE; a.out_f32 = 1; a.ksplit = 8;
        hipError_t rc = launch_conv_gemm(a, g.taps, st);
        return rc != hipSuccess ? rc : launch_splitk_reduce(SPK_, 8, a.Mrows, g.N, g.bias, act, out, st);
    });
}

hipError_t Net::se_gate(const ResBlockW& r, const float* stats, int boards, hipStream_t st) {
    SeGateArgs g;
    g.t_stats = stats; g.w1 = r.se_w1; g.b1 = r.se_b1; g.w2 = r.se_w2; g.b2 = r.se_b2;
    g.gate = G_; g.B = boards; g.C = Cp_; g.hidden = r.se_hidden; g.act = plan_.act;
    return launch_se_gate(g, st);
}

hipError_t Net::conv_norm_act(const PackedGemm& g, const NormParams& n, const _Float16* in, _Float16* out, _Float16* scratch,
                              int Mrows, hipStream_t st, const ConvNormOpts& o) {
    const bool big = conv_gemm_tile_n(g.Cin, g.N) == 320;
    GemmArgs a = gemm_args(g, in, out, Mrows);
    if (big && o.res && plan_.fuse_tail) {
        a.epi_act = plan_.act; a.res = o.res; a.pre_gamma = n.gamma; a.pre_beta = n.beta;
        if (o.next_bn1) { a.y2 = AA_; a.gn_gamma = o.next_bn1->gamma; a.gn_beta = o.next_bn1->beta; }
        return launch_conv_gemm(a, g.taps, st);
    }
    const bool epilogue = big ? g.taps == 9
                              : plan_.gn_small && (g.taps == 9 ? g.Cin == 32 : g.N == 32 || g.N == 64 || g.N == 128 || g.N == 160);
    if (epilogue && !o.res && !o.next_bn1) {
        a.gn_gamma = n.gamma; a.gn_beta = n.beta; a.epi_act = plan_.act; a.posenc = o.posenc;
        return run_gemm(g, a, st);
    }
    a.out = scratch; a.out_stats = S1_;
    hipError_t rc = run_gemm(g, a, st);
    if (rc != hipSuccess) return rc;
    EwArgs e = ew_args(scratch, out, g.N, plan_.act);
    e.t_stats = S1_; e.gn_gamma = n.gamma; e.gn_beta = n.beta; e.res = o.res; e.posenc = o.posenc;
    ew_next_bn1(e, o.next_bn1, AA_);
    return launch_ew_board(e, Mrows / 64, st);
}

void Net::harvest_profile() {
    for (size_t i = 0; i + 1 < pev_used_; i += 2) {
        float ms = 0.f;
        if (hipEventElapsedTime(&ms, pev_[i], pev_[i + 1]) == hipSuccess) {
            prof_ms_ += ms; prof_flop_ += pflop_[i / 2]; prof_launches_++;
            if (ptail_[i / 2]) { prof_tail_ms_ += ms; prof_tail_launches_++; }
        }
    }
    pev_used_ = 0;
    pflop_.clear();
    ptail_.clear();
}

int Net::forward(const float* planes_dev, const _Float16* nhwc_dev, int B, float* logits_dev, float* value_dev,
                 float* ssl_dev, hipStream_t st, std::string& err) {
    if (!finalized_) { err = "weights not finalized"; return M0_ERR_STATE; }
    if (B <= 0) { err = "batch must be positive"; return M0_ERR_INVALID; }
    if (int rc = ensure_workspace(B, err)) return rc;
    HipStatus& hs = *hip_;
    const int Bp = ceil_to(B, 4);
    const int Mc = Bp * 64;
    const int Mfc = ceil_to(B, 256);
    const int act = plan_.act, vact = plan_.vact;
    const int C = Cp_;

    const _Float16* x0 = nhwc_dev;
    if (!x0) {
        if (!planes_dev) { err = "no input"; return M0_ERR_INVALID; }
        M0_HIP(hs, launch_planes_to_nhwc(planes_dev, X0_, B, cfg_.planes, st));
        x0 = X0_;
    }
    _Float16* xa = XA_;
    _Float16* xb = XB_;
    const NormParams* first_bn1 = bn1(plan_.first_bn1);
    auto tap = [&](int step, const _Float16* stream, bool second) {
        if (step != tap_step_) return;
        const size_t bytes = (size_t)Mc * C * sizeof(_Float16);
        M0_HIP(hs, hipMemcpyAsync(TAPX_, stream, bytes, hipMemcpyDeviceToDevice, st));
        if (second) M0_HIP(hs, hipMemcpyAsync(TAPA_, AA_, bytes, hipMemcpyDeviceToDevice, st));
        tap_second_ = second;
    };
    ConvNormOpts so;
    if (cfg_.chess_features) so.posenc = posenc_; else so.next_bn1 = first_bn1;
    M0_HIP(hs, conv_norm_act(stem_, stem_n_, x0, xa, T1_, Mc, st, so));
    tap(0, xa, so.next_bn1 != nullptr);
    if (cfg_.chess_features) {
        if (cfg_.piece_square_tables) {
            ConvNormOpts po;
            po.res = xa;
            M0_HIP(hs, conv_norm_act(pst_, pst_n_, xa, xb, T1_, Mc, st, po));
            std::swap(xa, xb);
        }
        tap(1, xa, false);
        ConvNormOpts io;
        io.res = xa; io.next_bn1 = first_bn1;
        M0_HIP(hs, conv_norm_act(inter_, inter_n_, xa, xb, T1_, Mc, st, io));
        std::swap(xa, xb);
        tap(2, xa, first_bn1 != nullptr);
    } else {
        tap(1, xa, false);
        tap(2, xa, false);
    }
    for (size_t li = 0; li < tower_.size(); ++li) {
        const TowerLayer& L = tower_[li];
        const NormParams* next_bn1 = bn1(L.next_bn1);
        if (L.kind == 0) {
            const ResBlockW& r = res_[L.index];
            M0_HIP(hs, conv_norm_act(r.conv1, r.bn2, AA_, T1_, T2_, Mc, st));
            if (plan_.fuse_tail) {
                GemmArgs a = gemm_args(r.conv2, T1_, xb, Mc, act);
                a.res = xa;
                if (next_bn1) { a.y2 = AA_; a.gn_gamma = next_bn1->gamma; a.gn_beta = next_bn1->beta; }
                if (cfg_.se) { a.se_w1 = r.se_w1; a.se_b1 = r.se_b1; a.se_w2 = r.se_w2; a.se_b2 = r.se_b2; a.se_hidden = r.se_hidden;
                               a.se_wf = r.se_wf; }
                M0_HIP(hs, profiled(profile_, st, conv3x3_flop(r.conv2, Mc), true, [&] { return launch_conv_gemm(a, 9, st); }));
            } else {
                GemmArgs a = gemm_args(r.conv2, T1_, T2_, Mc);
                a.out_stats = S2_;
                M0_HIP(hs, run_gemm(r.conv2, a, st));
                EwArgs e = ew_args(T2_, xb, C, act);
                e.t_stats = S2_; e.res = xa;
                if (cfg_.se) { M0_HIP(hs, se_gate(r, S2_, Bp, st)); e.gate = G_; }
                ew_next_bn1(e, next_bn1, AA_);
                M0_HIP(hs, launch_ew_board(e, Bp, st));
            }
        } else {
            if (L.skip) { tap(3 + (int)li, xa, false); continue; }
            const AttnW& w = att_[L.index];
            const float inv_sqrt_d = 1.f / sqrtf((float)(C_ / cfg_.attention_heads));
            if (plan_.fuse_attn && w.blk_w != nullptr) {
                AttnBlockArgs ab;
                memset(&ab, 0, sizeof(ab));
                ab.x = xa; ab.wpack = w.blk_w; ab.bias = w.blk_bias; ab.mask = mask_dev_;
                ab.ln_g = w.ln.gamma; ab.ln_b = w.ln.beta; ab.y = xb;
                if (next_bn1) { ab.y2 = AA_; ab.gn2_gamma = next_bn1->gamma; ab.gn2_beta = next_bn1->beta; }
                ab.B = Bp; ab.ln_count = C_; ab.act = act; ab.grid_cap = sw_.attn_grid; ab.mix = cfg_.attention_unmasked_mix; ab.inv_sqrt_d = inv_sqrt_d;
                M0_HIP(hs, launch_attn_block(ab, st));
            } else {
                M0_HIP(hs, run_gemm(w.qkv, gemm_args(w.qkv, xa, QKV_, Mc), st));
                AttnArgs aa;
                aa.qkv = QKV_; aa.rel_bias = w.rel_bias; aa.mask = mask_dev_; aa.o = O_;
                aa.B = Bp; aa.H = C / 16; aa.C = C; aa.mix = cfg_.attention_unmasked_mix;
                aa.inv_sqrt_d = inv_sqrt_d;
                M0_HIP(hs, launch_attn_core(aa, st));
                M0_HIP(hs, run_gemm(w.proj, gemm_args(w.proj, O_, T1_, Mc), st));
                EwArgs e = ew_args(T1_, xb, C, act);
                e.res = xa; e.ln_g = w.ln.gamma; e.ln_b = w.ln.beta; e.ln_count = C_;
                ew_next_bn1(e, next_bn1, AA_);
                M0_HIP(hs, launch_ew_board(e, Bp, st));
            }
        }
        std::swap(xa, xb);
        tap(3 + (int)li, xa, next_bn1 != nullptr);
    }
    const bool joint = plan_.gn_small;
    if (joint) {
        GemmArgs a = gemm_args(hv_, xa, PH2_, Mc, act);
        a.gn_gamma = hv_n_.gamma; a.gn_beta = hv_n_.beta;
        a.ldo = 64; a.out2 = VH2_; a.ldo2 = 128; a.nsplit = 64;
        M0_HIP(hs, launch_conv_gemm(a, 1, st));
    } else {
        M0_HIP(hs, conv_norm_act(ph_conv_, ph_n_, xa, PH2_, PH_, Mc, st));
    }
    const bool factored = cfg_.policy_factor_rank > 0;
    if (factored) M0_HIP(hs, run_gemm(pfc1_, gemm_args(pfc1_, PH2_, F1_, Mfc, ACT_RELU), st));
    const PackedGemm& plast = factored ? pfc2_ : pfc1_;
    GemmArgs pl = gemm_args(plast, factored ? F1_ : PH2_, logits_dev, Mfc);
    pl.Mvalid = B; pl.out_f32 = 1; pl.out_scale = logit_scale_;
    M0_HIP(hs, run_gemm(plast, pl, st));
    if (!joint) M0_HIP(hs, conv_norm_act(vh0_, vh1_n_, xa, VH2_, VH_, Mc, st));
    _Float16* vflat = joint ? VH_ : VH2_;
    M0_HIP(hs, conv_norm_act(vh3_, vh4_n_, VH2_, vflat, VH_, Mc, st));
    M0_HIP(hs, run_gemm(vfc1_, gemm_args(vfc1_, vflat, F2_, Mfc, vact), st));
    M0_HIP(hs, run_gemm(vfc2_, gemm_args(vfc2_, F2_, F3_, Mfc, vact), st));
    GemmArgs vg = gemm_args(vgate_, F3_, F4_, Mfc, ACT_SIGMOID);
    vg.mul = F3_;
    M0_HIP(hs, run_gemm(vgate_, vg, st));
    GemmArgs v3 = gemm_args(vfc3_, F4_, VAL_, Mfc, ACT_TANH);
    v3.out_f32 = 1;
    M0_HIP(hs, run_gemm(vfc3_, v3, st));
    M0_HIP(hs, hipMemcpy2DAsync(value_dev, 4, VAL_, 32 * 4, 4, B, hipMemcpyDeviceToDevice, st));
    if (ssl_dev && !ssl_.empty()) {
        const int ctot = ssl_channels_total();
        int coff = 0;
        for (auto& h : ssl_) {
            M0_HIP(hs, conv_norm_act(h.c0, h.n, xa, SH2_, SH_, Mc, st));
            M0_HIP(hs, run_gemm(h.c1, gemm_args(h.c1, SH2_, SO_, Mc), st));
            M0_HIP(hs, launch_nhwc_to_nchw_f32(SO_, ssl_dev, B, 32, h.out_ch, ctot, coff, st));
            coff += h.out_ch;
        }
    }
    if (!hs.ok()) { err = "kernel launch failed: " + hs.message(); return M0_ERR_HIP; }
    return M0_OK;
}
```

### matrix0_amd/csrc/net_kernels.h

```cpp
#pragma once
#include <hip/hip_runtime.h>
#include <stdint.h>

enum { ACT_NONE = 0, ACT_RELU = 1, ACT_SILU = 2, ACT_LEAKY = 3, ACT_SIGMOID = 4, ACT_TANH = 5 };

enum ConvEpi {
    EPI_PLAIN,
    EPI_GN,
    EPI_ELEMENT,
    EPI_TAIL,
    EPI_TAIL_PRE,
};

constexpr int TAIL_SE_HMAX = 96;

struct GemmArgs {
    const _Float16* in;
    const _Float16* w;
    void* out;
    const float* gn_gamma;
    const float* gn_beta;
    const float* bias;
    const _Float16* mul;
    float* out_stats;
    int Mrows;
    int Mvalid;
    int Cin;
    int N;
    int Npad;
    int ldo;
    int epi_act;
    int out_f32;
    float out_scale;
    int ksplit;
    int w_pp;
    const _Float16* res;
    const float* pre_gamma;
    const float* pre_beta;
    _Float16* y2;
    const float* se_w1;
    const float* se_b1;
    const float* se_w2;
    const float* se_b2;
    int se_hidden;
    const void* se_wf;
    const float* posenc;
    void* out2;
    int ldo2;
    int nsplit;
};

struct EwArgs {
    const _Float16* t;
    const float* t_stats;
    const float* gn_gamma;
    const float* gn_beta;
    const float* gate;
    const _Float16* res;
    const float* posenc;
    const float* ln_g;
    const float* ln_b;
    int ln_count;
    _Float16* y;
    float* out_stats;
    _Float16* y2;
    const float* gn2_gamma;
    const float* gn2_beta;
    int C;
    int act;
};

struct SeGateArgs {
    const float* t_stats;
    const float* w1;
    const float* b1;
    const float* w2;
    const float* b2;
    float* gate;
    int B, C, hidden, act;
};

struct AttnArgs {
    const _Float16* qkv;
    const float* rel_bias;
    const uint64_t* mask;
    _Float16* o;
    int B, H, C;
    float mix;
    float inv_sqrt_d;
};

struct AttnBlockArgs {
    const _Float16* x;
    const void* wpack;
    const _Float16* bias;
    const uint64_t* mask;
    const float* ln_g;
    const float* ln_b;
    const float* gn2_gamma;
    const float* gn2_beta;
    _Float16* y;
    _Float16* y2;
    int B;
    int ln_count;
    int act;
    int grid_cap;
    float mix;
    float inv_sqrt_d;
};
hipError_t launch_attn_block(const AttnBlockArgs& a, hipStream_t st);
hipError_t launch_splitk_reduce(const float* part, int splits, int M, int N, const float* bias, int act, _Float16* out,
                                hipStream_t st);
size_t attn_block_pack_bytes();

hipError_t launch_conv_gemm(const GemmArgs& a, int taps, hipStream_t st);
int conv_gemm_tile_n(int Cin, int Npad);
int conv_gemm_kc(int Cin, int Npad);
hipError_t launch_ew_board(const EwArgs& a, int boards, hipStream_t st);
hipError_t launch_se_gate(const SeGateArgs& a, hipStream_t st);
hipError_t launch_attn_core(const AttnArgs& a, hipStream_t st);
hipError_t launch_planes_to_nhwc(const float* x, void* y, int B, int P, hipStream_t st);
hipError_t launch_nhwc_to_nchw_f32(const void* x, float* y, int B, int ld, int n, int ctot, int coff, hipStream_t st);
```

### matrix0_amd/csrc/net_pack.hip

```cpp
#include "net.h"
#include "net_pack.h"
#include "attn_math.h"
#include <math.h>
#include <string.h>
#include <algorithm>

namespace pk = net_pack;

static const char* kSslNames[5] = {"piece", "threat", "pin", "fork", "control"};
static const int kSslOut[5] = {13, 1, 1, 1, 3};

#define TRY(x) do { int rc_ = (x); if (rc_ != M0_OK) return rc_; } while (0)

int Net::load(const char* name, const void* data, int dtype, const int64_t* shape, int ndim, std::string& err) {
    if (finalized_) { err = "weights already finalized"; return M0_ERR_STATE; }
    if (!name || (!data && ndim >= 0)) { err = "null argument"; return M0_ERR_INVALID; }
    HostTensor t;
    size_t n = 1;
    for (int i = 0; i < ndim; ++i) { t.shape.push_back(shape[i]); n *= (size_t)shape[i]; }
    t.data.resize(n);
    if (dtype == 0) memcpy(t.data.data(), data, n * 4);
    else if (dtype == 1) {
        const _Float16* h = (const _Float16*)data;
        for (size_t i = 0; i < n; ++i) t.data[i] = (float)h[i];
// ... 18 lines not shown

int Net::upload_bytes(void*& dst, const void* src, size_t bytes, std::string& err) {
    void* d = dalloc(bytes, false);
    if (d && bytes) M0_HIP(*hip_, hipMemcpy(d, src, bytes, hipMemcpyHostToDevice));
    if (!hip_->ok()) { err = "weight upload failed: " + hip_->message(); return M0_ERR_HIP; }
    dst = d;
    return M0_OK;
}

template <class P, class T>
int Net::upload(P*& dst, const std::vector<T>& v, std::string& err) {
    void* d = nullptr;
    TRY(upload_bytes(d, v.data(), v.size() * sizeof(T), err));
    dst = (P*)d;
    return M0_OK;
}

int Net::pack_gemm(PackedGemm& g, const std::string& wkey, const std::string& bkey, const pk::GemmShape& s, std::string& err,
                   std::vector<_Float16>* keep) {
    const HostTensor* w = get(wkey, (size_t)s.N_real * s.Cin_real * s.taps, err);
    if (!w) return M0_ERR_INVALID;
    nparams_ += w->data.size();
    const bool big = conv_gemm_kc(s.Cin_pad, s.N_pad) == 64;
    const bool pp = big && s.taps == 9;
    const std::vector<_Float16> p =
        pk::gemm_weights<_Float16>(w->data.data(), pp ? pk::GEMM_BIG_3X3 : big ? pk::GEMM_BIG_1X1 : pk::GEMM_SMALL, s);
    TRY(upload(g.w, p, err));
    g.taps = s.taps; g.Cin = s.Cin_pad; g.N = s.N_pad; g.pp = pp;
    g.bias = nullptr;
    if (!bkey.empty()) {
        const HostTensor* b = get(bkey, s.N_real, err);
        if (!b) return M0_ERR_INVALID;
        nparams_ += s.N_real;
        TRY(upload(g.bias, pk::zero_padded<float>(b->data.data(), s.N_real, s.N_pad), err));
    }
    if (keep) *keep = p;
    return M0_OK;
}

static pk::GemmShape fc(int Cin_real, int Cin_pad, int N_real, int N_pad) { return {1, Cin_real, Cin_pad, N_real, N_pad}; }
static pk::GemmShape conv3x3(int Cin_real, int Cin_pad, int N_real, int N_pad) { return {9, Cin_real, Cin_pad, N_real, N_pad}; }
static pk::GemmShape flattened(int ch, int N_real, int N_pad) {
    pk::GemmShape s = fc(ch * 64, ch * 64, N_real, N_pad);
    s.flatten_ch = ch;
    return s;
}

int Net::upload_norm(NormParams& n, const std::string& prefix, int C_real, int C_pad, std::string& err, HostNorm* keep) {
    const HostTensor* g = get(prefix + ".weight", C_real, err);
    if (!g) return M0_ERR_INVALID;
    const HostTensor* b = get(prefix + ".bias", C_real, err);
    if (!b) return M0_ERR_INVALID;
    nparams_ += 2 * (size_t)C_real;
    HostNorm h = {pk::zero_padded<float>(g->data.data(), C_real, C_pad), pk::zero_padded<float>(b->data.data(), C_real, C_pad)};
    TRY(upload(n.gamma, h.gamma, err));
    TRY(upload(n.beta, h.beta, err));
    if (keep) *keep = std::move(h);
    return M0_OK;
}

int Net::pack_chess_features(std::string& err) {
    const int C = C_, P = Cp_;
    const HostTensor* pe = get("chess_features.position_encoding", (size_t)C * 64, err);
    if (!pe) return M0_ERR_INVALID;
    nparams_ += pe->data.size();
    TRY(upload(posenc_, pk::transposed<float>(pe->data.data(), C, 64, 64, P), err));
    if (cfg_.piece_square_tables) {
        TRY(pack_gemm(pst_, "chess_features.pst_conv.weight", "", fc(C, P, C, P), err));
        TRY(upload_norm(pst_n_, "chess_features.pst_norm", C, P, err));
    }
    TRY(pack_gemm(inter_, "chess_features.interaction_conv.weight", "", conv3x3(C, P, C, P), err));
    return upload_norm(inter_n_, "chess_features.interaction_norm", C, P, err);
}

int Net::pack_se(ResBlockW& r, const std::string& p, std::string& err) {
    const int C = C_, P = Cp_;
    const int hd = std::max(8, (int)(C * cfg_.se_ratio));
    r.se_hidden = hd;
    const HostTensor* w1 = get(p + ".se_fc1.weight", (size_t)hd * C, err); if (!w1) return M0_ERR_INVALID;
    const HostTensor* b1 = get(p + ".se_fc1.bias", hd, err); if (!b1) return M0_ERR_INVALID;
    const HostTensor* w2 = get(p + ".se_fc2.weight", (size_t)hd * C, err); if (!w2) return M0_ERR_INVALID;
    const HostTensor* b2 = get(p + ".se_fc2.bias", C, err); if (!b2) return M0_ERR_INVALID;
    nparams_ += (size_t)2 * hd * C + hd + C;
    const std::vector<float> w1t = pk::transposed<float>(w1->data.data(), hd, C, P, hd);
    const std::vector<float> w2t = pk::transposed<float>(w2->data.data(), C, hd, hd, P);
    TRY(upload(r.se_w1, w1t, err));
    TRY(upload(r.se_b1, b1->data, err));
    TRY(upload(r.se_w2, w2t, err));
    if (P == 320 && hd <= TAIL_SE_HMAX) TRY(upload(r.se_wf, pk::se_fragments<_Float16>(w1t.data(), w2t.data(), hd), err));
    return upload(r.se_b2, pk::zero_padded<float>(b2->data.data(), C, P), err);
}

int Net::pack_attn(AttnW& a, bool skip, const std::string& p, std::string& err) {
    const int C = C_, P = Cp_, H = cfg_.attention_heads;
    if (skip) {
        for (const char* k : {".qkv.weight", ".proj.weight", ".norm.weight", ".norm.bias", ".rel_bias"}) {
            auto it = sd_.find(p + k);
            if (it != sd_.end()) nparams_ += it->second.data.size();
        }
        return M0_OK;
    }
    pk::GemmShape qkv = fc(C, P, 3 * C, 3 * P);
    if (P != C) { qkv.qkv_heads = H; qkv.qkv_heads_pad = P / 16; }
    TRY(pack_gemm(a.qkv, p + ".qkv.weight", "", qkv, err));
    TRY(pack_gemm(a.proj, p + ".proj.weight", "", fc(C, P, C, P), err));
    TRY(upload_norm(a.ln, p + ".norm", C, P, err));
    std::vector<float> rbs;
    if (cfg_.attention_relbias) {
        const HostTensor* rb = get(p + ".rel_bias", (size_t)H * 4096, err); if (!rb) return M0_ERR_INVALID;
        nparams_ += rb->data.size();
        rbs.resize(rb->data.size());
        for (size_t i = 0; i < rbs.size(); ++i) rbs[i] = rb->data[i] * kLog2e;
    }
    if (P == 320) {
        const HostTensor* wq = get(p + ".qkv.weight", (size_t)3 * C * C, err);
        const HostTensor* wp = get(p + ".proj.weight", (size_t)C * C, err);
        if (!wq || !wp) return M0_ERR_INVALID;
        if (C != H * 16 || pk::kAttnPackElems * 2 != attn_block_pack_bytes()) { err = "shape mismatch for " + p; return M0_ERR_INVALID; }
        TRY(upload(a.blk_w, pk::attn_block_weights<_Float16>(wq->data.data(), wp->data.data(), H), err));
        TRY(upload(a.blk_bias, pk::attn_block_bias<_Float16>(rbs.empty() ? nullptr : rbs.data(), H), err));
    }
    if (cfg_.attention_relbias)
        TRY(upload(a.rel_bias, pk::zero_padded<float>(rbs.data(), rbs.size(), (size_t)(P / 16) * 4096), err));
    return M0_OK;
}

int Net::pack_joint_head(const std::vector<_Float16>& ph_w, const std::vector<_Float16>& vh_w, const HostNorm& ph_n,
                         const HostNorm& vh_n, std::string& err) {
    TRY(upload(hv_.w, pk::joint_columns(ph_w, 64, vh_w, 128, Cp_), err));
    hv_.taps = 1; hv_.Cin = Cp_; hv_.N = 192; hv_.pp = false; hv_.bias = nullptr;
    TRY(upload(hv_n_.gamma, pk::joined(ph_n.gamma, vh_n.gamma), err));
    return upload(hv_n_.beta, pk::joined(ph_n.beta, vh_n.beta), err);
}

int Net::pack_ssl_heads(std::string& err) {
    for (int t = 0; t < 5; ++t) {
        if (!(cfg_.ssl_tasks & (1 << t))) continue;
        SslHeadW h;
        h.out_ch = kSslOut[t];
        std::string p = std::string("ssl_heads.") + kSslNames[t];
        TRY(pack_gemm(h.c0, p + ".0.weight", "", fc(C_, Cp_, C_ / 2, Cs_), err));
        TRY(upload_norm(h.n, p + ".1", C_ / 2, Cs_, err));
        TRY(pack_gemm(h.c1, p + ".3.weight", "", fc(C_ / 2, Cs_, h.out_ch, 32), err));
        ssl_.push_back(h);
    }
    return M0_OK;
}

void Net::make_plan() {
    const bool big = conv_gemm_tile_n(Cp_, Cp_) == 320;
    plan_.fuse_tail = big && sw_.fuse_tail &&
                      (!cfg_.se || (res_[0].se_hidden <= TAIL_SE_HMAX && res_[0].se_hidden % 4 == 0));
    plan_.fuse_attn = big && sw_.fuse_attn;
    plan_.gn_small = Cp_ % 64 == 0;
    plan_.act = cfg_.activation == M0_ACT_SILU ? ACT_SILU : ACT_RELU;
    plan_.vact = cfg_.value_activation == M0_ACT_SILU ? ACT_SILU : (cfg_.value_activation == M0_ACT_LEAKY ? ACT_LEAKY : ACT_RELU);
    int next = -1;
    for (size_t i = tower_.size(); i-- > 0;) {
        TowerLayer& L = tower_[i];
        if (L.kind == 1 && L.skip) continue;
        L.next_bn1 = next;
        next = L.kind == 0 ? L.index : -1;
    }
    plan_.first_bn1 = next;
}

int Net::finalize(std::string& err) {
    if (finalized_) return M0_OK;
    if (!M0_HIP(*hip_, hipSetDevice(device_))) { err = hip_->message(); return M0_ERR_HIP; }
    const int C = C_, P = Cp_;
    nparams_ = 0;
    TRY(pack_gemm(stem_, "stem.0.weight", "", conv3x3(cfg_.planes, 32, C, P), err));
    TRY(upload_norm(stem_n_, "stem.1", C, P, err));
    if (cfg_.chess_features) TRY(pack_chess_features(err));
    int ti = 0;
    for (auto& L : tower_) {
        std::string p = "tower." + std::to_string(ti++);
        if (L.kind == 0) {
            ResBlockW& r = res_[L.index];
            TRY(pack_gemm(r.conv1, p + ".conv1.weight", "", conv3x3(C, P, C, P), err));
            TRY(pack_gemm(r.conv2, p + ".conv2.weight", "", conv3x3(C, P, C, P), err));
            TRY(upload_norm(r.bn1, p + ".bn1", C, P, err));
            TRY(upload_norm(r.bn2, p + ".bn2", C, P, err));
            if (cfg_.se) TRY(pack_se(r, p, err));
        } else {
            TRY(pack_attn(att_[L.index], L.skip, p, err));
        }
    }
    TRY(upload(mask_dev_, pk::attn_mask(), err));
    std::vector<_Float16> ph_w, vh_w;
    HostNorm ph_n, vh_n;
    TRY(pack_gemm(ph_conv_, "policy_head.0.weight", "", fc(C, P, 64, 64), err, &ph_w));
    TRY(upload_norm(ph_n_, "policy_head.1", 64, 64, err, &ph_n));
    if (cfg_.policy_factor_rank > 0) {
        const int r = cfg_.policy_factor_rank, rp = ceil_to(r, 32);
        TRY(pack_gemm(pfc1_, "policy_fc1.weight", "policy_fc1.bias", flattened(64, r, rp), err));
        TRY(pack_gemm(pfc2_, "policy_fc2.weight", "policy_fc2.bias", fc(r, rp, M0_POLICY_SIZE, M0_POLICY_SIZE), err));
    } else {
        TRY(pack_gemm(pfc1_, "policy_fc.weight", "policy_fc.bias", flattened(64, M0_POLICY_SIZE, M0_POLICY_SIZE), err));
    }
    {
        const HostTensor* ls = get("_policy_logit_scale_raw", err); if (!ls) return M0_ERR_INVALID;
        nparams_ += 1;
        double raw = ls->data.empty() ? 0.0 : ls->data[0];
        double sp = raw > 20.0 ? raw : log1p(exp(raw));
        logit_scale_ = (float)std::min(5.0, sp + 1e-3);
    }
    TRY(pack_gemm(vh0_, "value_head.0.weight", "", fc(C, P, 128, 128), err, &vh_w));
    TRY(upload_norm(vh1_n_, "value_head.1", 128, 128, err, &vh_n));
    TRY(pack_gemm(vh3_, "value_head.3.weight", "", fc(128, 128, 128, 128), err));
    TRY(upload_norm(vh4_n_, "value_head.4", 128, 128, err));
    TRY(pack_joint_head(ph_w, vh_w, ph_n, vh_n, err));
    const int h1 = 2 * C, h1p = ceil_to(h1, 32), h2 = C, h2p = ceil_to(C, 32);
    TRY(pack_gemm(vfc1_, "value_fc1.weight", "value_fc1.bias", flattened(128, h1, h1p), err));
    TRY(pack_gemm(vfc2_, "value_fc2.weight", "value_fc2.bias", fc(h1, h1p, h2, h2p), err));
    TRY(pack_gemm(vgate_, "value_gate.0.weight", "value_gate.0.bias", fc(h2, h2p, h2, h2p), err));
    TRY(pack_gemm(vfc3_, "value_fc3.weight", "value_fc3.bias", fc(h2, h2p, 1, 32), err));
    if (cfg_.self_supervised) TRY(pack_ssl_heads(err));
    sd_.clear();
    if (!M0_HIP(*hip_, hipDeviceSynchronize())) { err = "weight upload failed: " + hip_->message(); return M0_ERR_HIP; }
    make_plan();
    finalized_ = true;
    return M0_OK;
}
```

### matrix0_amd/csrc/selfplay.hip

```cpp
#include <math.h>
#include <string.h>
#include <atomic>
#include "selfplay_engine.h"
#include "tb.h"

namespace m0 {

static bool nn_cache_miss(m0_selfplay* sp, uint64_t key) {
    auto it = sp->nn_map.find(key);
    if (it != sp->nn_map.end()) {
        sp->nn_lru.splice(sp->nn_lru.end(), sp->nn_lru, it->second);
        return false;
    }
    sp->nn_lru.push_back(key);
    sp->nn_map[key] = std::prev(sp->nn_lru.end());
    if (sp->nn_lru.size() > 10000) { sp->nn_map.erase(sp->nn_lru.front()); sp->nn_lru.pop_front(); }
    return true;
}

static void seed_game_dev(GameDev& g, uint64_t base, int uid) {
    g.seed_jitter = derive_seed(base, uid, PURPOSE_JITTER);
    g.seed_noise = derive_seed(base, uid, PURPOSE_NOISE);
    g.seed_dir = derive_seed(base, uid, PURPOSE_DIRICHLET);
    g.seed_gumbel = derive_seed(base, uid, PURPOSE_GUMBEL);
// ... 282 lines not shown
    }
    return true;
}

int apply_advances(m0_selfplay* sp) {
    const bool ok = launch_advances(sp);
    sp->adv.clear();
    return ok ? M0_OK : m0_hip_error(sp->hip, "advance failed");
}

static void count_active_games(m0_selfplay* sp) {
    int act = 0;
    for (int s = 0; s < sp->G; ++s) act += sp->games[s].in_use ? 1 : 0;
    sp->stats.active_games = act;
}

static void start_games(m0_selfplay* sp) {
    for (int s = 0; s < sp->G; ++s) {
        if (sp->games[s].in_use) continue;
        if (sp->cfg.total_games > 0 && sp->next_game >= sp->cfg.total_games) break;
        start_game(sp, s);
    }
}

static int start_first_games(m0_selfplay* sp) {
    if (sp->stats.games_started != 0) return M0_OK;
    if (!sync_games_d2h(sp)) return m0_hip_error(sp->hip, "device sync failed");
    start_games(sp);
    const int rc = apply_advances(sp);
    if (rc != M0_OK) return rc;
    count_active_games(sp);
    return M0_OK;
}

int refill(m0_selfplay* sp) {
    switch (sp->kind) {
    case EngineKind::Analysis: return analysis_refill(sp);
    default: return start_first_games(sp);
    }
}

static int harvest_games(m0_selfplay* sp) {
    if (!M0_HIP(sp->hip, hipMemcpy(sp->hres.data(), sp->d.results, sizeof(RootResult) * sp->G, hipMemcpyDeviceToHost)))
        return m0_hip_error(sp->hip, "harvest failed");
    if (sp->tc.gumbel && !M0_HIP(sp->hip, hipMemcpy(sp->hgres.data(), sp->d.gumbel_results, sizeof(GumbelResult) * sp->G, hipMemcpyDeviceToHost)))
        return m0_hip_error(sp->hip, "harvest failed");
    if (sp->tc.proof && !M0_HIP(sp->hip, hipMemcpy(sp->hpres.data(), sp->d.proof_results, sizeof(ProofResult) * sp->G, hipMemcpyDeviceToHost)))
        return m0_hip_error(sp->hip, "harvest failed");
    for (int s = 0; s < sp->G; ++s) {
        if (!(sp->hg[s].active && sp->hg[s].finished)) continue;
        if (sp->hg[s].overflow) sp->stats.arena_overflows++;
        finish_search(sp, s);
    }
    start_games(sp);
    return apply_advances(sp);
}

static int harvest(m0_selfplay* sp) {
    switch (sp->kind) {
    case EngineKind::Analysis: return analysis_harvest(sp);
    default: return harvest_games(sp);
    }
}

static constexpr int M0_MAX_DEVICES = 16;
static std::mutex g_forward_gate[M0_MAX_DEVICES];
static std::atomic<int> g_engines_with_net[M0_MAX_DEVICES];
static bool forward_gate_enabled() {
    static const bool on = [] { const char* v = getenv("M0_FORWARD_GATE"); return v && v[0] == '1'; }();
    return on;
}

struct ForwardGate {
    std::mutex* m = nullptr;
    hipStream_t st = nullptr;
    ForwardGate(int device, hipStream_t stream, bool has_rows) : st(stream) {
        if (has_rows && forward_gate_enabled() && (unsigned)device < (unsigned)M0_MAX_DEVICES &&
            g_engines_with_net[device].load(std::memory_order_relaxed) > 1) {
            m = &g_forward_gate[device];
            m->lock();
        }
    }
    void release() {
        if (m) { (void)hipStreamSynchronize(st); m->unlock(); m = nullptr; }
    }
    ~ForwardGate() { release(); }
};

void forward_gate_join(m0_selfplay* sp) {
    if ((unsigned)sp->device < (unsigned)M0_MAX_DEVICES) { g_engines_with_net[sp->device].fetch_add(1); sp->counted = true; }
}
void forward_gate_leave(m0_selfplay* sp) {
    if (sp->counted) g_engines_with_net[sp->device].fetch_sub(1);
}

int finish_step(m0_selfplay* sp, int rows, double t0) {
    M0_HIP(sp->hip, hipEventRecord(sp->ev2, sp->stream));
    M0_HIP(sp->hip, launch_expand(sp->d, sp->tc, sp->stream));
    M0_HIP(sp->hip, hipEventRecord(sp->ev3, sp->stream));
    if (!sync_games_d2h(sp)) return m0_hip_error(sp->hip, "step failed");
    if (sp->net) sp->net->harvest_profile();
    if (sp->net_b) sp->net_b->harvest_profile();
    float ms_sel = 0, ms_net = 0, ms_exp = 0;
    M0_HIP(sp->hip, hipEventElapsedTime(&ms_sel, sp->ev0, sp->ev1));
    M0_HIP(sp->hip, hipEventElapsedTime(&ms_net, sp->ev1, sp->ev2));
    if (!M0_HIP(sp->hip, hipEventElapsedTime(&ms_exp, sp->ev2, sp->ev3))) return m0_hip_error(sp->hip, "step failed");
    sp->stats.ms_net += ms_net; sp->stats.ms_tree += ms_sel + ms_exp;
    sp->stats.steps++; sp->stats.evals += (uint64_t)rows;
    const double t1 = now_ms();
    bool any = false;
    if (sp->tc.eval_cache) {
        uint64_t h = 0;
        for (int s = 0; s < sp->G; ++s) h += sp->hg[s].cache_hits;
        sp->stats.evals_cached = h;
    }
    for (int s = 0; s < sp->G; ++s) {
        if (!sp->hg[s].active) continue;
        const int delta = sp->hg[s].sims_done - sp->prev_done[s];
        if (delta > 0) { sp->stats.sims += (uint64_t)delta; sp->prev_done[s] = sp->hg[s].sims_done; }
        if (sp->hg[s].finished) any = true;
    }
    if (any) { const int rc = harvest(sp); if (rc != M0_OK) return rc; }
    count_active_games(sp);
    const double t2 = now_ms();
    sp->stats.ms_host += t2 - t1;
    sp->stats.ms_total += t2 - t0;
    return M0_OK;
}

struct RowSplit { int main_rows, tail_rows; };
static RowSplit split_rows(int rows, bool have_tail, bool half_split) {
    int main_rows = rows;
    if (have_tail && rows >= 2048 && (rows & 1023) != 0) main_rows = rows & ~1023;
    if (have_tail && half_split && rows >= 4096) main_rows = ((rows / 2) + 1023) & ~1023;
    return {main_rows, rows - main_rows};
}

int one_step(m0_selfplay* sp) {
    std::string err;
    const double t0 = now_ms();
    M0_HIP(sp->hip, hipEventRecord(sp->ev0, sp->stream));
    int rows = 0;
    if (run_select(sp, &rows) != M0_OK) return M0_ERR_HIP;
    if (!M0_HIP(sp->hip, hipEventRecord(sp->ev1, sp->stream))) return m0_hip_error(sp->hip, "step failed");
    if (rows > sp->rows_max || sp->rows2[1] > sp->rows_max) { m0_set_error("row counter overflow"); return M0_ERR_STATE; }
    ForwardGate gate(sp->device, sp->stream, rows > 0 || sp->rows2[1] > 0);
    if (rows > 0) {
        if (!sp->net) { m0_set_error("m0_selfplay_step needs a network (use the split-step API without one)"); return M0_ERR_STATE; }
        const auto [main_rows, tail_rows] = split_rows(rows, sp->net_tail != nullptr, sp->half_split);
        float* ssl = sp->cfg.ssl_in_forward ? sp->ssl_dev : nullptr;
        if (tail_rows > 0 && !M0_HIP(sp->hip, hipEventRecord(sp->ev_sel, sp->stream)))
            return m0_hip_error(sp->hip, "step failed");
        m0_net_lock(sp->nethandle);
        int rc = sp->net->forward(nullptr, sp->d.x0, main_rows, sp->logits_dev, sp->values_dev, ssl, sp->stream, err);
        if (rc == M0_OK && tail_rows > 0 && M0_HIP(sp->hip, hipStreamWaitEvent(sp->stream_tail, sp->ev_sel, 0))) {
            const size_t sslw = ssl ? (size_t)sp->net->ssl_channels_total() * 64 : 0;
            rc = sp->net_tail->forward(nullptr, sp->d.x0 + (size_t)main_rows * 64 * 32, tail_rows, sp->logits_dev + (size_t)main_rows * 4672,
                                       sp->values_dev + main_rows, ssl ? ssl + (size_t)main_rows * sslw : nullptr, sp->stream_tail, err);
            M0_HIP(sp->hip, hipEventRecord(sp->ev_tail, sp->stream_tail));
            M0_HIP(sp->hip, hipStreamWaitEvent(sp->stream, sp->ev_tail, 0));
        }
        m0_net_unlock(sp->nethandle);
        if (rc != M0_OK) { sp->hip.check(sp->net->hip()); m0_set_error(err); return rc; }
        if (!sp->hip.ok()) return m0_hip_error(sp->hip, "step failed");
        sp->stats.rows_tail += (uint64_t)tail_rows;
    }
    if (sp->rows2[1] > 0) {
        if (!sp->net_b) { m0_set_error("rows for a second network without one"); return M0_ERR_STATE; }
        const size_t b = (size_t)sp->d.net_row_base;
        m0_net_lock(sp->nethandle_b);
        int rc = sp->net_b->forward(nullptr, sp->d.x0 + b * 64 * 32, sp->rows2[1], sp->logits_dev + b * 4672,
                                    sp->values_dev + b, nullptr, sp->stream, err);
        m0_net_unlock(sp->nethandle_b);
        if (rc != M0_OK) { sp->hip.check(sp->net_b->hip()); m0_set_error(err); return rc; }
        rows += sp->rows2[1];
    }
    gate.release();
    return finish_step(sp, rows, t0);
}

}
```

### matrix0_amd/csrc/selfplay_engine.h

```cpp
#pragma once
#include <hip/hip_runtime.h>
#include <chrono>
#include <deque>
#include <list>
#include <mutex>
#include <string>
#include <unordered_map>
#include <vector>
#include "../../include/m0_engine.h"
#include "capi_common.h"
#include "chess_core.h"
#include "host_rules.h"
#include "net.h"
#include "tree.h"

namespace m0 {

inline double now_ms() {
    return std::chrono::duration<double, std::milli>(std::chrono::steady_clock::now().time_since_epoch()).count();
}

struct GameRecordOwner {
    std::vector<float> s, pi, z, search_values, ssl;
    std::vector<uint8_t> legal_mask;
    std::vector<uint16_t> played;
    std::string start_fen;
};

struct HostGame : Line {
    bool in_use = false;
    int game_index = 0;
    std::vector<Pos> rec_pos;
    std::vector<float> states, pis, search_values;
    std::vector<int8_t> turns;
    std::vector<uint8_t> masks;
    std::vector<int> sims_used;
    int nstates = 0;
    double entropy_sum = 0.0;
    int entropy_count = 0;
    ResignState resign;
    HStream rng;
    double t0 = 0.0;
    int cur_sims = 0;
    bool a_is_white = true;
    int book_index = -1;
};

enum class EngineKind { SelfPlay, Match, Analysis };
constexpr unsigned KIND_SELFPLAY = 1u << (int)EngineKind::SelfPlay, KIND_MATCH = 1u << (int)EngineKind::Match,
                   KIND_ANALYSIS = 1u << (int)EngineKind::Analysis, KIND_GAMES = KIND_SELFPLAY | KIND_MATCH,
                   KIND_ANY = KIND_GAMES | KIND_ANALYSIS;

struct AdvanceList {
    std::vector<int> slots, roots;
    void push(int slot, int root) { slots.push_back(slot); roots.push_back(root); }
    void clear() { slots.clear(); roots.clear(); }
    bool empty() const { return slots.empty(); }
};

struct AnalysisJob { Line line; int sims; int nlegal; int64_t id; bool keep = false; };
struct Analysis {
    m0_analysis_opts opts;
    std::deque<AnalysisJob> queue;
    std::deque<AnalysisJob> policy_queue;
    std::deque<m0_analysis_result> done;
    std::deque<std::vector<int32_t>> done_children;
    std::deque<m0_proof_lines> done_proof;
    m0_proof_lines last_proof = {};
    m0_proof_lines* proof_dev = nullptr;
    std::vector<m0_proof_lines> hproof;
    std::vector<AnalysisJob> slot_job;
    std::vector<uint8_t> held;
    int* reroot_in_dev = nullptr;
    RerootOut* reroot_out_dev = nullptr;
    std::vector<int> finished;
    std::vector<m0_analysis_line> hlines;
    std::vector<int> hnlines;
    std::vector<float> hvalues;
    std::vector<Pos> hpos;
    m0_analysis_line* lines_dev = nullptr;
    int* nlines_dev = nullptr;
    float* value_out_dev = nullptr;
    Pos* pos_dev = nullptr;
    int32_t* nlegal_dev = nullptr;
    uint16_t* moves_dev = nullptr;
    int32_t* idx_dev = nullptr;
    bool keep_visits = false;
    int32_t* child_idx_dev = nullptr;
    int32_t* child_n_dev = nullptr;
    int32_t* nchild_dev = nullptr;
    std::vector<int32_t> hchild_idx, hchild_n, hnchild;
};

}

struct m0_selfplay {
    m0::EngineKind kind = m0::EngineKind::SelfPlay;
    m0_selfplay_cfg cfg;
    TreeCfg tc;
    m0_net* nethandle = nullptr;
    m0_net* nethandle_b = nullptr;
    Net* net = nullptr;
    Net* net_b = nullptr;
    Net* net_tail = nullptr;
    hipStream_t stream_tail = nullptr;
    hipEvent_t ev_sel = nullptr, ev_tail = nullptr;
    bool half_split = false;
    int device = 0;
    hipStream_t stream = nullptr;
    bool own_stream = false;
    int G = 0, L = 0, cap = 0, rows_max = 0;
    TreeDev d;
    std::vector<void*> allocs;
    HipStatus hip;
    std::vector<GameDev> hg;
    std::vector<m0::HostGame> games;
    std::vector<RootResult> hres;
    float* logits_dev = nullptr;
    float* values_dev = nullptr;
    float* ssl_dev = nullptr;
    m0::Pos* ssl_pos_dev = nullptr;
    float* ssl_out_dev = nullptr;
    int ssl_cap = 0;
    m0::AdvanceList adv;
    int* ids_dev = nullptr;
    int* roots_dev = nullptr;
    std::deque<m0_game_record> done_meta;
    m0_selfplay_stats stats;
    int next_game = 0;
    hipEvent_t ev0 = nullptr, ev1 = nullptr, ev2 = nullptr, ev3 = nullptr;
    std::mutex mu;
    std::vector<Sample> hsamples;
    std::vector<int> prev_done;
    int last_rows = 0, last_rows_b = 0;
    int rows2[2] = {0, 0};
    std::vector<m0::Pos> book;
    std::vector<std::string> book_fens;
    std::list<uint64_t> nn_lru;
    std::unordered_map<uint64_t, std::list<uint64_t>::iterator> nn_map;
    bool ext_pending = false;
    bool counted = false;
    m0::Analysis* an = nullptr;
    const m0_tb* tb = nullptr;
    int tb_max_pieces = 0;
    uint64_t tb_adjudications = 0;
    std::vector<GumbelResult> hgres;
    bool search_begun = false;
    std::vector<ProofResult> hpres;
};

namespace m0 {

template <typename T>
T* dalloc(m0_selfplay* sp, size_t count) {
    void* p = nullptr;
    size_t bytes = count * sizeof(T);
    if (bytes == 0) bytes = 16;
    if (!M0_HIP(sp->hip, hipMalloc(&p, bytes))) return nullptr;
    sp->allocs.push_back(p);
    M0_HIP(sp->hip, hipMemsetAsync(p, 0, bytes, sp->stream));
    return (T*)p;
}
inline bool hip_ok(m0_selfplay* sp, const char* context) {
    if (!sp->hip.ok()) m0_hip_error(sp->hip, context);
    return sp->hip.ok();
}

bool kind_accepted(const m0_selfplay* sp, const char* what, unsigned kinds);
#define M0_ENGINE_CALL_OR(null_result, sp, what, kinds, on_device)                    \
    if (!(sp)) { m0_set_error(what ": sp is null"); return null_result; }             \
    std::lock_guard<std::mutex> lk((sp)->mu);                                         \
    if (!m0::kind_accepted(sp, what, kinds)) return M0_ERR_STATE;                     \
    if ((on_device) && !M0_HIP((sp)->hip, hipSetDevice((sp)->device))) return m0_hip_error((sp)->hip)
#define M0_ENGINE_CALL(sp, what, kinds, on_device) M0_ENGINE_CALL_OR(M0_ERR_INVALID, sp, what, kinds, on_device)

void forward_gate_join(m0_selfplay* sp);
void forward_gate_leave(m0_selfplay* sp);
bool sync_games_d2h(m0_selfplay* sp);
bool sync_games_h2d(m0_selfplay* sp);
HostGame& occupy_slot(m0_selfplay* sp, int slot, Line&& line, int uid);
void begin_search(m0_selfplay* sp, int slot, int sims, bool dirichlet, int root);
void arm_slot_search(m0_selfplay* sp, int slot, int sims, bool dirichlet, bool fresh);
int apply_advances(m0_selfplay* sp);
int run_select(m0_selfplay* sp, int* rows_out);
int refill(m0_selfplay* sp);
int one_step(m0_selfplay* sp);
int finish_step(m0_selfplay* sp, int rows, double t0);

m0_selfplay* engine_create(m0_net* nh, m0_net* nh_b, const m0_selfplay_cfg* cfg, EngineKind kind);
int ext_select_impl(m0_selfplay* sp, int* rows_a, int* rows_b, float* planes_a, float* planes_b, int max_rows);
int ext_expand_impl(m0_selfplay* sp, const float* logits_a, const float* values_a, int rows_a, const float* logits_b,
                    const float* values_b, int rows_b);

int analysis_refill(m0_selfplay* sp);
int analysis_harvest(m0_selfplay* sp);

}
```

### matrix0_amd/csrc/tree.h

```cpp
#pragma once
#include <hip/hip_runtime.h>
#include <stdint.h>
#include "chess_core.h"
namespace m0 { struct TbSet; }
#include "../../include/m0_engine.h"
#include "gumbel_core.h"
#include "proof_core.h"

#define M0_MAX_DEPTH 256
#define M0_HIST_CAP 192
#define M0_MAX_CHILDREN 256
static_assert(M0_MAX_CHILDREN == m0::M0_GUMBEL_MAX_K, "gumbel_core.h and include/m0_gumbel.h count on 256 root children at most");
constexpr int M0_NHWC_C = 32;

struct TreeCfg {
    double fpu_reduction;
    double draw_penalty;
    double virtual_loss;
    double selection_jitter;
    double cpuct;
    double cpuct_start, cpuct_end;
    int cpuct_plies;
    int use_c_base;
    double cpuct_c_base, cpuct_c_init;
    double dirichlet_alpha, dirichlet_frac;
    int legal_softmax;
    int enable_entropy_noise;
    int no_instant_backtrack;
    int virtual_loss_active;
    int leaves_per_step;
    int tt_merge;
    int raw_legal_priors;
    int max_children;
    double min_child_prior;
    int eval_cache;
    int gumbel;
    m0_gumbel_cfg gumbel_cfg;
    int proof;
};

#define M0_EC_MAXLEGAL 64
#define M0_EC_WORDS 66
struct EvalCache {
    uint64_t* keys;
    uint32_t* stamps;
    float* payload;
    float* hit_stage;
    int sets;
    int sides;
};

struct GameDev {
    m0::Pos root_pos;
    int root;
    int next;
    int arena;
    int active;
    int sims_done, sims_target;
    int need_dirichlet;
    int root_q_from_v;
    int flip_root_v;
    int root_fresh;
    int hist_len;
    int nsamples;
    int overflow;
    int finished;
    int root_n;
    double root_q;
    double root_v;
    uint64_t seed_jitter, seed_noise, seed_dir;
    uint64_t ctr_jitter, ctr_noise, ctr_dir;
    uint64_t evals;
    int net_id;
    int reinfer;
    uint64_t cache_hits;
    uint32_t cache_clock[2];
    int ec_clear;
    int side_next[2];
    int root_found;
    uint64_t tb_leaves;
    uint64_t seed_gumbel, ctr_gumbel;
    int gumbel_drawn;
    int gumbel_miss;
};

enum SampleKind : int {
    SK_NONE = 0,
    SK_EVAL = 1,
    SK_ROOT_INIT = 2,
    SK_TERMINAL = 3,
    SK_ROOT_VALUE = 4,
    SK_CACHED = 5,
    SK_SHARED = 6,
};
M0_HD bool sample_owns_row(int kind) { return kind == SK_EVAL || kind == SK_ROOT_INIT || kind == SK_ROOT_VALUE; }
M0_HD bool sample_holds_inflight(int kind) { return kind == SK_EVAL || kind == SK_TERMINAL || kind == SK_CACHED || kind == SK_SHARED; }

struct Sample {
    m0::Pos pos;
    int kind;
    uint64_t ckey;
    int leaf;
    int depth;
    int row;
    int nlegal;
};
static_assert(sizeof(Sample) == 104, "the host copies Sample arrays device-to-host: the layout must not move");

struct TreeArrays {
    double* prior;
    double* w;
    double* q;
    int* n;
    int* vl;
    int* cbase;
    int16_t* nch;
    uint16_t* mv;
    uint16_t* midx;
    int cap;
    int16_t* proof;
};

struct RootResult {
    int nchild;
    int root_n;
    double root_q;
    int child_node[M0_MAX_CHILDREN];
    int child_n[M0_MAX_CHILDREN];
    uint16_t child_mv[M0_MAX_CHILDREN];
    uint16_t child_idx[M0_MAX_CHILDREN];
    double child_prior[M0_MAX_CHILDREN];
    double child_q[M0_MAX_CHILDREN];
};

struct GumbelResult {
    int pick;
    double v_mix;
    double pi[M0_MAX_CHILDREN];
    double gl[M0_MAX_CHILDREN];
};

struct ProofResult {
    int state, plies;
    int pick;
    int16_t child[M0_MAX_CHILDREN];
};

struct TreeDev {
    TreeArrays t;
    GameDev* games;
    Sample* samples;
    int* paths;
    int* epaths;
    uint64_t* tt_keys;
    int* tt_nodes;
    int tt_cap;
    EvalCache ec;
    int search_nodes;
    int tt_sides;
    uint16_t* leaf_moves;
    uint64_t* hist;
    RootResult* results;
    int* row_counter;
    int net_row_base;
    _Float16* x0;
    const float* logits;
    const float* values;
    int G;
    int L;
    const m0::TbSet* tb_set;
    int tb_max_pieces;
    double* gumbel_gl;
    GumbelResult* gumbel_results;
    ProofResult* proof_results;
};

hipError_t launch_select(const TreeDev& d, const TreeCfg& c, hipStream_t st);
hipError_t launch_expand(const TreeDev& d, const TreeCfg& c, hipStream_t st);
enum RootMode : int {
    ROOT_FRESH = -1,
    ROOT_FROM_SIDE_TABLE = -2,
    ROOT_FIRST_OF_GAME = -3,
};
hipError_t launch_advance(const TreeDev& d, const int* game_ids_dev, const int* child_slots_dev, int count, hipStream_t st);
#define M0_REROOT_MAX_MOVES 8
struct RerootOut { int32_t kept, n; double q; };
hipError_t launch_reroot_moves(const TreeDev& d, const int* slots_dev, const int* nmoves_dev, const int* moves_dev ,
                               int count, RerootOut* out_dev, hipStream_t st);

hipError_t launch_encode_positions(const m0::Pos* pos_dev, int n, float* planes_f32_dev ,
                                   _Float16* nhwc_dev , uint8_t* mask_dev ,
                                   int32_t* nlegal_dev, uint16_t* moves_dev , int32_t* idx_dev ,
                                   hipStream_t st);

hipError_t launch_decode_planes(const float* planes_dev, const uint8_t* mask_dev, int n, m0::Pos* pos_dev, int32_t* status_dev,
                                int32_t* flags_dev, int32_t* nlegal_dev, hipStream_t st);

hipError_t launch_analysis_lines(const TreeDev& d, const int* slots_dev, int count, int multipv, int pv_len,
                                 m0_analysis_line* lines_dev, int* nlines_dev, hipStream_t st, m0_proof_lines* proof_dev = nullptr);
hipError_t launch_root_children(const TreeDev& d, const int* slots_dev, int count, int32_t* policy_idx_dev, int32_t* visits_dev,
                                int32_t* nchild_dev, hipStream_t st);
hipError_t launch_policy_lines(const float* logits_dev, const float* values_dev, const int32_t* nlegal_dev, const uint16_t* moves_dev,
                               const int32_t* idx_dev, int rows, int multipv, m0_analysis_line* lines_dev, int* nlines_dev,
                               float* value_out_dev, hipStream_t st);

hipError_t launch_ssl_targets(const m0::Pos* pos_dev, int n, float* out_dev, hipStream_t st);
hipError_t launch_ssl_targets_planes(const float* planes_dev, int n, float* out_dev, int32_t* status_dev, hipStream_t st);

hipError_t launch_replay_games(const m0::Pos* start_dev, const uint32_t* patterns_dev, const int32_t* offsets_dev ,
                               int n_games, int max_plies, m0::Pos* pos_dev, uint16_t* moves_dev, int32_t* policy_idx_dev,
                               int32_t* nlegal_dev, int8_t* turn_dev, int32_t* plies_dev, int32_t* status_dev,
                               int32_t* end_flags_dev, hipStream_t st);
```

### matrix0_amd/csrc/tree_expand.hip

```cpp
#include "tree_device.h"
#include "tree_gumbel.h"
#include "tree_proof.h"
#include "eval_cache.h"

struct ExpandScratch {
    float pr[M0_MAX_CHILDREN];
    uint8_t keep[M0_MAX_CHILDREN];
    float total;
    int bad;
};

struct ExpandEnv {
    Arena A;
    int cap;
    GameDev* gd;
    uint64_t* TK; int* TN; int tt_cap;
    ExpandScratch* X;
    int lane;
};
struct LeafLogits {
    const float* row;
    const float* legal;
    float* store;
};
__device__ __forceinline__ LeafLogits logits_of_row(const float* row, float* store) { return LeafLogits{row, nullptr, store}; }
__device__ __forceinline__ LeafLogits logits_of_cache(const float* payload) { return LeafLogits{nullptr, payload + EC_LOGITS, nullptr}; }

static __device__ float np_sum_f32_dev(const float* a, int n) {
    auto block = [&](const float* b, int m) -> float {
        if (m < 8) { float r = 0.f; for (int i = 0; i < m; ++i) r += b[i]; return r; }
        float r[8];
        for (int j = 0; j < 8; ++j) r[j] = b[j];
        int i;
        for (i = 8; i < m - (m % 8); i += 8)
            for (int j = 0; j < 8; ++j) r[j] += b[i + j];
        float res = ((r[0] + r[1]) + (r[2] + r[3])) + ((r[4] + r[5]) + (r[6] + r[7]));
        for (; i < m; ++i) res += b[i];
        return res;
    };
    if (n <= 128) return block(a, n);
    int n2 = n / 2;
    n2 -= n2 % 8;
    return block(a, n2) + block(a + n2, n - n2);
}

__device__ __forceinline__ void priors_raw(const float* lg, const int (&idx)[CPL], int n, int lane, ExpandScratch* X, float (&pr)[CPL]) {
#pragma unroll
    for (int k = 0; k < CPL; ++k) { const int i = lane + 64 * k; if (i < n) X->pr[i] = lg[idx[k]]; }
    __syncthreads();
    if (lane == 0) X->total = np_sum_f32_dev(X->pr, n);
    __syncthreads();
    const float total = X->total;
    const bool ok = isfinite(total) && total > 0.f;
#pragma unroll
    for (int k = 0; k < CPL; ++k) { const int i = lane + 64 * k; pr[k] = i < n ? (ok ? X->pr[i] / total : 1.0f / (float)n) : 0.f; }
    __syncthreads();
}

__device__ __forceinline__ void priors_uniform(int n, float (&pr)[CPL]) {
#pragma unroll
    for (int k = 0; k < CPL; ++k) pr[k] = 1.0f / (float)n;
}

__device__ __forceinline__ void priors_legal_softmax(const LeafLogits& src, const int (&idx)[CPL], int n, int lane, GameDev* gd,
                                                     const TreeCfg& c, float (&pr)[CPL]) {
    double ent = 0.0;
    float l[CPL];
#pragma unroll
    for (int k = 0; k < CPL; ++k) {
        const int i = lane + 64 * k;
        l[k] = i < n ? (src.legal ? src.legal[i] : src.row[idx[k]]) : -3.0e38f;
        if (src.store && i < n && i < M0_EC_MAXLEGAL) src.store[EC_LOGITS + i] = l[k];
    }
    wave_softmax(l, n, lane, pr);
#pragma unroll
    for (int k = 0; k < CPL; ++k) {
        const int i = lane + 64 * k;
        if (i < n) ent -= (double)pr[k] * log((double)pr[k] + 1e-8);
    }
    ent = wave_sum_d(ent);
    const double ratio = ent / fmax(1e-9, log((double)(n > 1 ? n : 1)));
    if (c.enable_entropy_noise && ratio > 0.9) {
        const uint64_t ctr = gd->ctr_noise;
        const uint64_t seed = gd->seed_noise;
        double dd[CPL], ds = 0.0;
#pragma unroll
        for (int k = 0; k < CPL; ++k) {
            const int i = lane + 64 * k;
            dd[k] = 0.0;
            if (i < n) { dd[k] = fmax((double)pr[k] + 0.1 * normal_at(seed, ctr + 2ull * (uint64_t)i), 1e-8); ds += dd[k]; }
        }
        ds = wave_sum_d(ds);
#pragma unroll
        for (int k = 0; k < CPL; ++k) pr[k] = (float)(dd[k] / ds);
        if (lane == 0) gd->ctr_noise = ctr + 2ull * (uint64_t)n;
    }
}

__device__ __forceinline__ void priors_full_softmax(const float* lg, const int (&idx)[CPL], int n, int lane, GameDev* gd,
                                                    const TreeCfg& c, float (&pr)[CPL]) {
    float mx = -3.0e38f;
    double ent = 0.0;
    for (int j = lane; j < M0_POLICY_SIZE; j += 64) mx = fmaxf(mx, lg[j]);
    mx = wave_max_f(mx);
    double sum = 0.0;
    for (int j = lane; j < M0_POLICY_SIZE; j += 64) sum += exp((double)(lg[j] - mx));
    sum = wave_sum_d(sum);
    const double fsum = sum;
    for (int j = lane; j < M0_POLICY_SIZE; j += 64) {
        const double pj = (double)(float)(exp((double)(lg[j] - mx)) / sum);
        ent -= pj * log(pj + 1e-8);
    }
#pragma unroll
    for (int k = 0; k < CPL; ++k) { const int i = lane + 64 * k; pr[k] = i < n ? (float)(exp((double)(lg[idx[k]] - mx)) / sum) : 0.f; }
    ent = wave_sum_d(ent);
    const double ratio = ent / fmax(1e-9, log((double)(n > 1 ? n : 1)));
    if (c.enable_entropy_noise && ratio > 0.9) {
        const uint64_t ctr = gd->ctr_noise;
        const uint64_t seed = gd->seed_noise;
        double ds = 0.0;
        for (int j = lane; j < M0_POLICY_SIZE; j += 64)
            ds += fmax((double)(float)(exp((double)(lg[j] - mx)) / fsum) + 0.1 * normal_at(seed, ctr + 2ull * (uint64_t)j), 1e-8);
        ds = wave_sum_d(ds);
#pragma unroll
        for (int k = 0; k < CPL; ++k) {
            const int i = lane + 64 * k;
            if (i < n) {
                const int j = idx[k];
                pr[k] = (float)(fmax((double)pr[k] + 0.1 * normal_at(seed, ctr + 2ull * (uint64_t)j), 1e-8) / ds);
            }
        }
        if (lane == 0) gd->ctr_noise = ctr + 2ull * (uint64_t)M0_POLICY_SIZE;
    }
}

__device__ __forceinline__ void priors_renormalise(int n, int lane, float (&pr)[CPL]) {
    double tot = 0.0;
#pragma unroll
    for (int k = 0; k < CPL; ++k) { const int i = lane + 64 * k; if (i < n) { if (!(pr[k] >= 0.f) || !isfinite(pr[k])) pr[k] = 0.f; tot += (double)pr[k]; } }
    tot = wave_sum_d(tot);
    const float totf = (float)tot;
    if (totf > 0.f && isfinite(totf)) {
#pragma unroll
        for (int k = 0; k < CPL; ++k) pr[k] = pr[k] / totf;
    } else priors_uniform(n, pr);
}

__device__ __forceinline__ int prune_children(const TreeCfg& c, const float (&pr)[CPL], int n, int lane, ExpandScratch* X, int (&slot)[CPL]) {
#pragma unroll
    for (int k = 0; k < CPL; ++k) slot[k] = lane + 64 * k;
    if (!(c.max_children > 0 || c.min_child_prior > 0.0)) return n;
#pragma unroll
    for (int k = 0; k < CPL; ++k) {
        const int i = lane + 64 * k;
        if (i < n) { X->pr[i] = pr[k]; X->keep[i] = (c.min_child_prior > 0.0 && !((double)pr[k] >= c.min_child_prior)) ? 0 : 1; }
    }
    __syncthreads();
    int kept = 0;
    for (int j = 0; j < n; ++j) kept += X->keep[j];
    const bool topk = c.max_children > 0 && kept > c.max_children;
    const int nkeep = topk ? c.max_children : kept;
#pragma unroll
    for (int k = 0; k < CPL; ++k) {
        const int i = lane + 64 * k;
        slot[k] = -1;
        if (i < n && X->keep[i]) {
            int r = 0;
            if (topk) { for (int j = 0; j < n; ++j) r += (X->keep[j] && (X->pr[j] > pr[k] || (X->pr[j] == pr[k] && j < i))) ? 1 : 0; }
            else { for (int j = 0; j < i; ++j) r += X->keep[j]; }
            if (r < nkeep) slot[k] = r;
        }
    }
    __syncthreads();
    return nkeep;
}

__device__ __forceinline__ bool write_children(const ExpandEnv& E, int leaf, const Pos& pos, const Move (&mvv)[CPL], const int (&idx)[CPL],
                                               const float (&pr)[CPL], const int (&slot)[CPL], int n, int nkeep, bool reg_children,
                                               double q0) {
    const Arena& A = E.A;
    GameDev* gd = E.gd;
    const int lane = E.lane;
    const int cb = gd->next;
    if (cb + nkeep > E.cap) { if (lane == 0) gd->overflow = 1; return false; }
#pragma unroll
    for (int k = 0; k < CPL; ++k) {
        const int i = lane + 64 * k;
        if (i < n && slot[k] >= 0) {
            const int ci = cb + slot[k];
            node_reset(A, ci, (double)pr[k], mvv[k], (uint16_t)idx[k]);
            if (q0 != 0.0) A.q[ci] = q0;
            if (E.TK && reg_children) {
                Pos q = pos;
                make_move(q, mvv[k]);
                tt_insert(E.TK, E.TN, E.tt_cap, tt_key_of(q), ci);
            }
        }
    }
    if (E.TK && !reg_children && lane == 0) tt_insert(E.TK, E.TN, E.tt_cap, tt_key_of(pos), leaf);
    if (lane == 0) { A.cbase[leaf] = cb; A.nch[leaf] = (int16_t)nkeep; gd->next = cb + nkeep; }
    __syncthreads();
    return true;
}

__device__ __forceinline__ double child_seed_q(const TreeCfg& c, const Arena& A, const int* path, int depth) {
    if (c.tt_merge || depth < 1) return 0.0;
    const double pq = A.q[path[depth - 1]];
    return pq != 0.0 ? -pq : 0.0;
}

__device__ __forceinline__ bool expand_node(const ExpandEnv& E, const TreeCfg& c, int leaf, const Pos& pos, const uint16_t* smoves, int n,
                                   const LeafLogits& src, bool is_root, bool reg_children, double q0) {
    const int lane = E.lane;
    if (n <= 0) return true;
    bool bad = false;
    if (!src.legal) bad = row_nonfinite(src.row, lane);
    bad = __any(bad);
    if (lane == 0) E.X->bad = bad ? 1 : 0;
    float pr[CPL];
    int idx[CPL];
    Move mvv[CPL];
#pragma unroll
    for (int k = 0; k < CPL; ++k) {
        const int i = lane + 64 * k;
        pr[k] = 0.f; idx[k] = 0; mvv[k] = 0;
        if (i < n) { mvv[k] = smoves[i]; idx[k] = move_to_index(pos, mvv[k]); }
    }
    if (c.raw_legal_priors && c.legal_softmax && !is_root) priors_raw(src.row, idx, n, lane, E.X, pr);
    else if (bad) priors_uniform(n, pr);
    else {
        if (c.legal_softmax) priors_legal_softmax(src, idx, n, lane, E.gd, c, pr);
        else priors_full_softmax(src.row, idx, n, lane, E.gd, c, pr);
        priors_renormalise(n, lane, pr);
    }
    int slot[CPL];
    const int nkeep = prune_children(c, pr, n, lane, E.X, slot);
    return write_children(E, leaf, pos, mvv, idx, pr, slot, n, nkeep, reg_children, q0);
}

__device__ __forceinline__ bool expand_evaluated(const TreeDev& d, const TreeCfg& c, const ExpandEnv& E, int g, const Sample& smp,
                                                 const uint16_t* moves, const float* lg, float v, double q0) {
    const Arena& A = E.A;
    GameDev* gd = E.gd;
    const int lane = E.lane, kind = smp.kind, leaf = smp.leaf;
    const Pos pos = smp.pos;
    float* cw = nullptr;
    size_t ce = 0;
    const uint64_t ckey = kind == SK_EVAL ? smp.ckey : 0ull;
    if (ckey != 0 && isfinite(v)) {
        ce = ec_choose_victim(d.ec, gd, g, ckey, lane);
        cw = ec_payload(d.ec, ce);
        ec_invalidate(d.ec, ce, lane);
    }
    const bool ok = expand_node(E, c, leaf, pos, moves, smp.nlegal, logits_of_row(lg, cw), kind == SK_ROOT_INIT,
                                !(kind == SK_ROOT_INIT && gd->root_fresh), q0);
    if (c.eval_cache && kind == SK_EVAL && lane == 0 && A.nch[leaf] < 0) A.cbase[leaf] = -1;
    const int sig = cw ? legal_sig(moves, smp.nlegal, lane) : 0;
    if (cw && lane == 0) {
        if (ok && !E.X->bad) ec_publish(d.ec, gd, ce, ckey, v, sig);
    }
    return ok;
}

__device__ __forceinline__ bool retry_refused_shared(const TreeCfg& c, const ExpandEnv& E, const Sample* S, int s, const uint16_t* LM,
                                                     const float* logits, const int* path) {
    const int leaf = S[s].leaf, row = S[s].row;
    int s0 = 0;
    while (s0 < s && !(S[s0].kind == SK_EVAL && S[s0].row == row)) ++s0;
    if (s0 >= s) return true;
    const Pos pos = S[s].pos;
    return expand_node(E, c, leaf, pos, LM + (size_t)s0 * M0_MAX_CHILDREN, S[s].nlegal,
                       logits_of_row(logits + (size_t)row * M0_POLICY_SIZE, nullptr), false, true,
                       child_seed_q(c, E.A, path, S[s].depth));
}

__device__ __forceinline__ void release_inflight(const TreeDev& d, const TreeCfg& c, const Arena& A, int g, const Sample* S, const int* P,
                                                 int ns, int lane) {
    for (int s = lane; s < ns; s += 64) {
        if (sample_holds_inflight(S[s].kind)) {
            const int* path = (c.tt_merge ? d.epaths + (size_t)g * (d.L + 1) * M0_MAX_DEPTH : P) + (size_t)s * M0_MAX_DEPTH;
            for (int dd = 1; dd <= S[s].depth; ++dd) atomicSub(&A.vl[path[dd]], 1);
        }
    }
}

__device__ __forceinline__ void write_root_result(RootResult* R, const Arena& A, int root, int lane) {
    const int k = A.nch[root] > 0 ? A.nch[root] : 0;
    const int cb = A.cbase[root];
    for (int i = lane; i < k; i += 64) {
        R->child_node[i] = cb + i; R->child_n[i] = A.n[cb + i];
        R->child_mv[i] = A.mv[cb + i]; R->child_idx[i] = A.midx[cb + i];
        R->child_prior[i] = A.prior[cb + i]; R->child_q[i] = A.q[cb + i];
    }
    if (lane == 0) { R->nchild = k; R->root_n = A.n[root]; R->root_q = A.q[root]; }
}

__global__ __launch_bounds__(64) void expand_kernel(TreeDev d, TreeCfg c) {
    __shared__ ExpandScratch X;
    const int g = blockIdx.x, lane = threadIdx.x;
    GameDev* gd = &d.games[g];
    if (!gd->active) return;
    uint64_t* TK = c.tt_merge ? d.tt_keys + tt_table_of(d, g, gd) : nullptr;
    int* TN = c.tt_merge ? d.tt_nodes + tt_table_of(d, g, gd) : nullptr;
    const uint16_t* LM = d.leaf_moves + (size_t)g * (d.L + 1) * M0_MAX_CHILDREN;
    const int ns = gd->nsamples;
    const Arena A = arena_of(d.t, g, gd->arena);
    const bool proven = c.proof && A.proof[gd->root] != 0;
    if (ns <= 0 && !(proven && !gd->finished)) return;
    const ExpandEnv E{A, d.t.cap, gd, TK, TN, d.tt_cap, &X, lane};
    const Sample* S = d.samples + (size_t)g * (d.L + 1);
    const int* P = d.paths + (size_t)g * (d.L + 1) * M0_MAX_DEPTH;
    const bool may_repeat = c.tt_merge != 0;
    int sims = 0;
    uint64_t evals = 0, hits = 0;
    bool refused = false;
    for (int s = 0; s < ns; ++s) {
        const int kind = S[s].kind;
        const int* path = P + (size_t)s * M0_MAX_DEPTH;
        const uint16_t* moves = LM + (size_t)s * M0_MAX_CHILDREN;
        if (kind == SK_SHARED) {
            const float v = d.values[S[s].row];
            if (refused) {
                __builtin_amdgcn_fence(__ATOMIC_SEQ_CST, "agent");
                if (A.nch[S[s].leaf] < 0) retry_refused_shared(c, E, S, s, LM, d.logits, path);
            }
            backprop(A, path, S[s].depth, (double)v, lane, may_repeat, NoMirror{});
            ++sims; ++hits;
            __syncthreads();
        } else if (kind == SK_CACHED) {
            const int leaf = S[s].leaf, depth = S[s].depth;
            const float* pay = ec_hit_stage(d, g, s);
            const float v = pay[EC_VALUE];
            if (A.nch[leaf] < 0) {
                const Pos pos = S[s].pos;
                refused |= !expand_node(E, c, leaf, pos, moves, S[s].nlegal, logits_of_cache(pay), false, true,
                                        child_seed_q(c, A, path, depth));
            }
            backprop(A, path, depth, (double)v, lane, may_repeat, NoMirror{});
            ++sims; ++hits;
            __syncthreads();
        } else if (kind == SK_EVAL || kind == SK_ROOT_INIT) {
            const int leaf = S[s].leaf, depth = S[s].depth, row = S[s].row;
            const float* lg = d.logits + (size_t)row * M0_POLICY_SIZE;
            const float v = d.values[row];
            if (A.nch[leaf] < 0) refused |= !expand_evaluated(d, c, E, g, S[s], moves, lg, v, child_seed_q(c, A, path, depth));
            ++evals;
            if (kind == SK_EVAL) {
                backprop(A, path, depth, (double)v, lane, may_repeat, NoMirror{});
                ++sims;
            } else {
                const double rv = root_value(gd, v);
                if (lane == 0) {
                    gd->root_v = rv;
                    if (gd->root_q_from_v) { A.q[leaf] = rv; gd->root_q_from_v = 0; }
                }
            }
            __syncthreads();
        } else if (kind == SK_TERMINAL) {
            ++sims;
        } else if (kind == SK_ROOT_VALUE) {
            const double rv = root_value(gd, d.values[S[s].row]);
            if (lane == 0) gd->root_v = rv;
            ++evals;
        }
    }
    if (c.virtual_loss_active) release_inflight(d, c, A, g, S, P, ns, lane);
    __syncthreads();
    const int done = gd->sims_done + sims;
    const int root = gd->root;
    const bool fin = ((A.nch[root] >= 0 || gd->overflow) && done >= gd->sims_target) || proven;
    if (lane == 0) {
        gd->sims_done = done;
        gd->evals += evals;
        gd->cache_hits += hits;
        gd->finished = fin ? 1 : 0;
        gd->root_n = A.n[root];
        gd->root_q = A.q[root];
    }
    if (fin) write_root_result(d.results + g, A, root, lane);
    if (fin && c.gumbel) write_gumbel_result(d, c, A, gd, g, root, lane);
    if (fin && c.proof) write_proof_result(d, A, g, root, lane);
}

hipError_t launch_expand(const TreeDev& d, const TreeCfg& c, hipStream_t st) {
    hipLaunchKernelGGL(expand_kernel, dim3(d.G), dim3(64), 0, st, d, c);
    return hipGetLastError();
}
```

Measured before the change: 1.163.

## Compute per-row non-finite logit flags in policy GEMM epilogue for expand

Adds a per-row flag buffer recording whether any policy logit is non-finite. The flag is computed inside the final policy GEMM epilogue when the factored head shape allows, or by a small separate kernel otherwise. The tree expand kernel then reads one byte instead of scanning all 4672 logits per evaluated leaf for NaN/Inf. This trades a full-row reread in the expand kernel for extra compare logic and a memset in the GEMM epilogue, plus a new specialized GEMM instantiation.

Result: no change. 1.164, median of 3 (+0.1%).

```diff
diff --git a/include/m0_engine.h b/include/m0_engine.h
--- a/include/m0_engine.h
+++ b/include/m0_engine.h
@@ -285,4 +285,5 @@
 #include "m0_augment.h"
 #include "m0_proof.h"
 #include "m0_rowpack.h"
+#include "m0_row_flags.h"
 #endif
diff --git a/include/m0_row_flags.h b/include/m0_row_flags.h
--- /dev/null
+++ b/include/m0_row_flags.h
@@ -0,0 +1,12 @@
+#ifndef M0_ROW_FLAGS_H
+#define M0_ROW_FLAGS_H
+#ifdef __cplusplus
+extern "C" {
+#endif
+
+int m0_net_logit_flags(m0_net* net, const float* planes, int B, float* policy, float* value, uint8_t* flags);
+
+#ifdef __cplusplus
+}
+#endif
+#endif
diff --git a/matrix0_amd/_abi.py b/matrix0_amd/_abi.py
--- a/matrix0_amd/_abi.py
+++ b/matrix0_amd/_abi.py
@@ -282,13 +282,17 @@
     "m0_rowpack_bench": (i32, [i32, i32, i32, P(f32), P(f32), P(f64)]),
 }
 
+ROW_FLAGS_FUNCTIONS = {
+    "m0_net_logit_flags": (i32, [vp, vp, i32, vp, vp, vp]),
+}
+
 
 def bind(L) -> list:
     missing = []
     for name, (restype, argtypes) in (list(FUNCTIONS.items()) + list(LIVE_FUNCTIONS.items()) + list(SCORE_FUNCTIONS.items()) +
                                       list(SSL_SCORE_FUNCTIONS.items()) + list(GUMBEL_FUNCTIONS.items()) +
                                       list(AUGMENT_FUNCTIONS.items()) + list(PROOF_FUNCTIONS.items()) +
-                                      list(ROWPACK_FUNCTIONS.items())):
+                                      list(ROWPACK_FUNCTIONS.items()) + list(ROW_FLAGS_FUNCTIONS.items())):
         fn = getattr(L, name, None)
         if fn is None:
             missing.append(name)
diff --git a/matrix0_amd/backend.py b/matrix0_amd/backend.py
--- a/matrix0_amd/backend.py
+++ b/matrix0_amd/backend.py
@@ -212,6 +212,18 @@
                    "m0_net_bench_forward")
         return float(ms.value)
 
+    def logit_flags(self, x: np.ndarray):
+        a = np.ascontiguousarray(x, dtype=np.float32)
+        if a.ndim != 4 or a.shape[1:] != (self._cfg.planes, 8, 8):
+            raise ValueError(f"expected input [B,{self._cfg.planes},8,8], got {a.shape}")
+        B = a.shape[0]
+        pol = np.empty((B, _lib.POLICY_SIZE), dtype=np.float32)
+        val = np.empty((B,), dtype=np.float32)
+        flags = np.empty((B,), dtype=np.uint8)
+        _lib.check(self._L.m0_net_logit_flags(self._h, _lib.ptr(a), B, _lib.ptr(pol), _lib.ptr(val), _lib.ptr(flags)),
+                   "m0_net_logit_flags")
+        return pol, val, flags
+
     def profile_enable(self, on: bool = True) -> None:
         _lib.check(self._L.m0_net_profile_enable(self._h, int(on)), "m0_net_profile_enable")
 
diff --git a/matrix0_amd/csrc/capi_net.hip b/matrix0_amd/csrc/capi_net.hip
--- a/matrix0_amd/csrc/capi_net.hip
+++ b/matrix0_amd/csrc/capi_net.hip
@@ -448,4 +448,29 @@
     return M0_OK;
 }
 
-}
+int m0_net_logit_flags(m0_net* n, const float* planes, int B, float* policy, float* value, uint8_t* flags) {
+    if (!n || !planes || !flags || B <= 0) { m0_set_error("invalid argument"); return M0_ERR_INVALID; }
+    std::lock_guard<std::mutex> lk(n->mu);
+    HipStatus& hs = n->net->hip();
+    if (!M0_HIP(hs, hipSetDevice(n->device))) return m0_hip_error(hs);
+    int rc = ensure_io(n, B);
+    if (rc != M0_OK) return rc;
+    struct Flags {
+        uint8_t* p = nullptr;
+        ~Flags() { if (p) (void)hipFree(p); }
+    } fl;
+    if (!M0_HIP(hs, hipMalloc((void**)&fl.p, (size_t)B))) return m0_hip_error(hs, "hipMalloc failed for the row flags");
+    M0_HIP(hs, hipMemsetAsync(fl.p, 0xff, (size_t)B, n->stream));
+    M0_HIP(hs, hipMemcpyAsync(n->planes_dev, planes, (size_t)B * n->net->cfg().planes * 64 * 4, hipMemcpyHostToDevice, n->stream));
+    if (!hs.ok()) return m0_hip_error(hs, "H2D copy");
+    std::string err;
+    rc = n->net->forward(n->planes_dev, nullptr, B, n->logits_dev, n->value_dev, nullptr, n->stream, err, fl.p);
+    if (rc != M0_OK) { m0_set_error(err); return rc; }
+    if (policy) M0_HIP(hs, hipMemcpyAsync(policy, n->logits_dev, (size_t)B * M0_POLICY_SIZE * 4, hipMemcpyDeviceToHost, n->stream));
+    if (value) M0_HIP(hs, hipMemcpyAsync(value, n->value_dev, (size_t)B * 4, hipMemcpyDeviceToHost, n->stream));
+    M0_HIP(hs, hipMemcpyAsync(flags, fl.p, (size_t)B, hipMemcpyDeviceToHost, n->stream));
+    if (!M0_HIP(hs, hipStreamSynchronize(n->stream))) return m0_hip_error(hs, "forward failed");
+    return M0_OK;
+}
+
+}
diff --git a/matrix0_amd/csrc/capi_selfplay.hip b/matrix0_amd/csrc/capi_selfplay.hip
--- a/matrix0_amd/csrc/capi_selfplay.hip
+++ b/matrix0_amd/csrc/capi_selfplay.hip
@@ -80,6 +80,8 @@
     sp->d.x0 = dalloc<_Float16>(sp, (size_t)(nreg * sp->rows_max + 4) * 64 * 32);
     sp->logits_dev = dalloc<float>(sp, (size_t)nreg * sp->rows_max * 4672);
     sp->values_dev = dalloc<float>(sp, (size_t)nreg * sp->rows_max + 4);
+    const char* rf = getenv("M0_ROW_FLAGS");
+    if (!(rf && rf[0] == '0')) sp->row_flags_dev = dalloc<uint8_t>(sp, (size_t)nreg * sp->rows_max);
     sp->d.net_row_base = sp->rows_max;
     if (sp->cfg.ssl_in_forward && sp->net && sp->net->ssl_channels_total() > 0)
         sp->ssl_dev = dalloc<float>(sp, (size_t)sp->rows_max * sp->net->ssl_channels_total() * 64);
@@ -91,7 +93,7 @@
     }
     sp->ids_dev = dalloc<int>(sp, sp->G);
     sp->roots_dev = dalloc<int>(sp, sp->G);
-    sp->d.logits = sp->logits_dev; sp->d.values = sp->values_dev;
+    sp->d.logits = sp->logits_dev; sp->d.values = sp->values_dev; sp->d.row_flags = sp->row_flags_dev;
     sp->d.G = sp->G; sp->d.L = sp->L;
     return hip_ok(sp, "hipMalloc failed for the batch buffers (lower concurrent_games or inference_batch_size)");
 }
@@ -185,6 +187,8 @@
     if (rows <= 0) return;
     M0_HIP(sp->hip, hipMemcpyAsync(sp->logits_dev + row_base * 4672, logits, (size_t)rows * 4672 * 4, hipMemcpyHostToDevice, sp->stream));
     M0_HIP(sp->hip, hipMemcpyAsync(sp->values_dev + row_base, values, (size_t)rows * 4, hipMemcpyHostToDevice, sp->stream));
+    if (sp->row_flags_dev)
+        M0_HIP(sp->hip, launch_logit_flags(sp->logits_dev + row_base * 4672, sp->row_flags_dev + row_base, rows, sp->stream));
 }
 
 int m0::ext_select_impl(m0_selfplay* sp, int* rows_a, int* rows_b, float* planes_a, float* planes_b, int max_rows) {
diff --git a/matrix0_amd/csrc/conv_epilogue.h b/matrix0_amd/csrc/conv_epilogue.h
--- a/matrix0_amd/csrc/conv_epilogue.h
+++ b/matrix0_amd/csrc/conv_epilogue.h
@@ -176,4 +176,36 @@
             }
         });
     }
-}
+    if constexpr (EPI == EPI_LOGITS) {
+        const int ldo = a.ldo;
+        const int rowbase = m0 + wm * 64 + 4 * half;
+        const float oscale = a.out_scale;
+        float* out = reinterpret_cast<float*>(a.out);
+        uint8_t* flags = a.row_flags;
+        uint32_t badm = 0;
+        static_for<0, NT>([&](auto ni_) __attribute__((always_inline)) {
+            constexpr int ni = decltype(ni_)::value;
+            const int col = colbase + ni * 32;
+            const float bias = a.bias != nullptr ? a.bias[col] : 0.f;
+            static_for<0, 2>([&](auto mi_) __attribute__((always_inline)) {
+                constexpr int mi = decltype(mi_)::value;
+                const float16v av = acc[mi][ni];
+                static_for<0, 16>([&](auto r_) __attribute__((always_inline)) {
+                    constexpr int r = decltype(r_)::value;
+                    const int row = rowbase + mi * 32 + (r & 3) + 8 * (r >> 2);
+                    float v = av[r] + bias;
+                    v *= oscale;
+                    if (row < a.Mvalid) out[(size_t)row * ldo + col] = v;
+                    badm |= (__builtin_bit_cast(uint32_t, v) & 0x7f800000u) == 0x7f800000u ? 1u << (mi * 16 + r) : 0u;
+                });
+            });
+        });
+        if (flags != nullptr && badm != 0) {
+            static_for<0, 32>([&](auto b_) __attribute__((always_inline)) {
+                constexpr int b = decltype(b_)::value;
+                const int row = rowbase + (b >> 4) * 32 + (b & 3) + 8 * ((b & 15) >> 2);
+                if (((badm >> b) & 1u) != 0 && row < a.Mvalid) flags[row] = 1;
+            });
+        }
+    }
+}
diff --git a/matrix0_amd/csrc/conv_gemm.hip b/matrix0_amd/csrc/conv_gemm.hip
--- a/matrix0_amd/csrc/conv_gemm.hip
+++ b/matrix0_amd/csrc/conv_gemm.hip
@@ -136,6 +136,8 @@
         int out_col0 = 0;
         if (a.out2 != nullptr && n0 + wn * NT * 32 >= a.nsplit) { o.out = a.out2; o.ldo = a.ldo2; out_col0 = a.nsplit; }
         conv_tile_epilogue<EPI_GN, ACT, NT>(acc, o, smem + wave * (64 * 64 * NT), m0, n0, wm, wn, lane, out_col0);
+    } else if constexpr (EPI == EPI_LOGITS) {
+        conv_tile_epilogue<EPI_LOGITS, ACT_NONE, NT>(acc, a, smem, m0, n0, wm, wn, lane);
     } else {
         conv_tile_epilogue<EPI_ELEMENT, ACT_NONE, NT>(acc, a, smem, m0, n0, wm, wn, lane);
     }
@@ -205,6 +207,11 @@
         return launch_conv_gemm_t<9, 1, 1, 32>(a, st);
     } else if (taps == 1) {
         if (big) return a.w_pp ? hipErrorInvalidValue : launch_conv_big(a, 1, st);
+        if (a.row_flags != nullptr) {
+            if (!a.out_f32 || a.mul != nullptr || a.out_stats != nullptr || a.epi_act != ACT_NONE || a.ksplit > 1)
+                return hipErrorInvalidValue;
+            return launch_conv_gemm_t<1, 1, 1, 32, EPI_LOGITS>(a, st);
+        }
         if (a.Mrows / 256 >= 256 && a.Npad % 64 == 0) return launch_conv_gemm_t<1, 1, 2, 32>(a, st);
         return launch_conv_gemm_t<1, 1, 1, 32>(a, st);
     }
diff --git a/matrix0_amd/csrc/net.h b/matrix0_amd/csrc/net.h
--- a/matrix0_amd/csrc/net.h
+++ b/matrix0_amd/csrc/net.h
@@ -80,7 +80,7 @@
     const std::vector<size_t>& device_buffer_bytes() const { return dev_sizes_; }
 
     int forward(const float* planes_dev, const _Float16* nhwc_dev, int B, float* logits_dev, float* value_dev,
-                float* ssl_dev, hipStream_t st, std::string& err);
+                float* ssl_dev, hipStream_t st, std::string& err, uint8_t* row_flags = nullptr);
     int ensure_workspace(int B, std::string& err);
     int ssl_channels_total() const;
     const m0_net_cfg& cfg() const { return cfg_; }
@@ -107,10 +107,11 @@
     int device_;
     hipStream_t stream_ = nullptr;
     HipStatus own_hip_, *hip_ = &own_hip_;
-    struct Switches { bool fuse_tail = true, fuse_attn = true; int attn_grid = 0; } sw_;
+    struct Switches { bool fuse_tail = true, fuse_attn = true, fuse_flags = true; int attn_grid = 0; } sw_;
     struct Plan {
         bool fuse_tail = false;
         bool fuse_attn = false;
+        bool fuse_flags = false;
         bool gn_small = false;
         int act = 0, vact = 0;
         int first_bn1 = -1;
diff --git a/matrix0_amd/csrc/net.hip b/matrix0_amd/csrc/net.hip
--- a/matrix0_amd/csrc/net.hip
+++ b/matrix0_amd/csrc/net.hip
@@ -23,6 +23,7 @@
     auto off = [](const char* name) { const char* e = getenv(name); return e && e[0] == '0'; };
     sw_.fuse_tail = !off("M0_FUSE_TAIL");
     sw_.fuse_attn = !off("M0_FUSE_ATTN");
+    sw_.fuse_flags = !off("M0_FUSE_FLAGS");
     if (const char* e = getenv("M0_ATTN_GRID")) sw_.attn_grid = std::max(0, atoi(e));
     C_ = cfg.channels;
     Cp_ = (C_ > 256 && C_ < 320) ? 320 : C_;
@@ -232,7 +233,7 @@
 }
 
 int Net::forward(const float* planes_dev, const _Float16* nhwc_dev, int B, float* logits_dev, float* value_dev,
-                 float* ssl_dev, hipStream_t st, std::string& err) {
+                 float* ssl_dev, hipStream_t st, std::string& err, uint8_t* row_flags) {
     if (!finalized_) { err = "weights not finalized"; return M0_ERR_STATE; }
     if (B <= 0) { err = "batch must be positive"; return M0_ERR_INVALID; }
     if (int rc = ensure_workspace(B, err)) return rc;
@@ -346,7 +347,13 @@
     const PackedGemm& plast = factored ? pfc2_ : pfc1_;
     GemmArgs pl = gemm_args(plast, factored ? F1_ : PH2_, logits_dev, Mfc);
     pl.Mvalid = B; pl.out_f32 = 1; pl.out_scale = logit_scale_;
+    const bool fused_flags = row_flags && plan_.fuse_flags;
+    if (fused_flags) {
+        pl.row_flags = row_flags;
+        M0_HIP(hs, hipMemsetAsync(row_flags, 0, (size_t)B, st));
+    }
     M0_HIP(hs, run_gemm(plast, pl, st));
+    if (row_flags && !fused_flags) M0_HIP(hs, launch_logit_flags(logits_dev, row_flags, B, st));
     if (!joint) M0_HIP(hs, conv_norm_act(vh0_, vh1_n_, xa, VH2_, VH_, Mc, st));
     _Float16* vflat = joint ? VH_ : VH2_;
     M0_HIP(hs, conv_norm_act(vh3_, vh4_n_, VH2_, vflat, VH_, Mc, st));
diff --git a/matrix0_amd/csrc/net_kernels.h b/matrix0_amd/csrc/net_kernels.h
--- a/matrix0_amd/csrc/net_kernels.h
+++ b/matrix0_amd/csrc/net_kernels.h
@@ -10,6 +10,7 @@
     EPI_ELEMENT,
     EPI_TAIL,
     EPI_TAIL_PRE,
+    EPI_LOGITS,
 };
 
 constexpr int TAIL_SE_HMAX = 96;
@@ -48,6 +49,7 @@
     void* out2;
     int ldo2;
     int nsplit;
+    uint8_t* row_flags;
 };
 
 struct EwArgs {
@@ -120,4 +122,5 @@
 hipError_t launch_se_gate(const SeGateArgs& a, hipStream_t st);
 hipError_t launch_attn_core(const AttnArgs& a, hipStream_t st);
 hipError_t launch_planes_to_nhwc(const float* x, void* y, int B, int P, hipStream_t st);
+hipError_t launch_logit_flags(const float* logits, uint8_t* flags, int rows, hipStream_t st);
 hipError_t launch_nhwc_to_nchw_f32(const void* x, float* y, int B, int ld, int n, int ctot, int coff, hipStream_t st);
diff --git a/matrix0_amd/csrc/net_pack.hip b/matrix0_amd/csrc/net_pack.hip
--- a/matrix0_amd/csrc/net_pack.hip
+++ b/matrix0_amd/csrc/net_pack.hip
@@ -194,6 +194,7 @@
     plan_.fuse_tail = big && sw_.fuse_tail &&
                       (!cfg_.se || (res_[0].se_hidden <= TAIL_SE_HMAX && res_[0].se_hidden % 4 == 0));
     plan_.fuse_attn = big && sw_.fuse_attn;
+    plan_.fuse_flags = big && sw_.fuse_flags && cfg_.policy_factor_rank > 0 && pfc2_.Cin == 128 && pfc2_.N == M0_POLICY_SIZE;
     plan_.gn_small = Cp_ % 64 == 0;
     plan_.act = cfg_.activation == M0_ACT_SILU ? ACT_SILU : ACT_RELU;
     plan_.vact = cfg_.value_activation == M0_ACT_SILU ? ACT_SILU : (cfg_.value_activation == M0_ACT_LEAKY ? ACT_LEAKY : ACT_RELU);
diff --git a/matrix0_amd/csrc/selfplay.hip b/matrix0_amd/csrc/selfplay.hip
--- a/matrix0_amd/csrc/selfplay.hip
+++ b/matrix0_amd/csrc/selfplay.hip
@@ -458,11 +458,13 @@
         if (tail_rows > 0 && !M0_HIP(sp->hip, hipEventRecord(sp->ev_sel, sp->stream)))
             return m0_hip_error(sp->hip, "step failed");
         m0_net_lock(sp->nethandle);
-        int rc = sp->net->forward(nullptr, sp->d.x0, main_rows, sp->logits_dev, sp->values_dev, ssl, sp->stream, err);
+        uint8_t* const flags = sp->row_flags_dev;
+        int rc = sp->net->forward(nullptr, sp->d.x0, main_rows, sp->logits_dev, sp->values_dev, ssl, sp->stream, err, flags);
         if (rc == M0_OK && tail_rows > 0 && M0_HIP(sp->hip, hipStreamWaitEvent(sp->stream_tail, sp->ev_sel, 0))) {
             const size_t sslw = ssl ? (size_t)sp->net->ssl_channels_total() * 64 : 0;
             rc = sp->net_tail->forward(nullptr, sp->d.x0 + (size_t)main_rows * 64 * 32, tail_rows, sp->logits_dev + (size_t)main_rows * 4672,
-                                       sp->values_dev + main_rows, ssl ? ssl + (size_t)main_rows * sslw : nullptr, sp->stream_tail, err);
+                                       sp->values_dev + main_rows, ssl ? ssl + (size_t)main_rows * sslw : nullptr, sp->stream_tail, err,
+                                       flags ? flags + main_rows : nullptr);
             M0_HIP(sp->hip, hipEventRecord(sp->ev_tail, sp->stream_tail));
             M0_HIP(sp->hip, hipStreamWaitEvent(sp->stream, sp->ev_tail, 0));
         }
@@ -476,7 +478,7 @@
         const size_t b = (size_t)sp->d.net_row_base;
         m0_net_lock(sp->nethandle_b);
         int rc = sp->net_b->forward(nullptr, sp->d.x0 + b * 64 * 32, sp->rows2[1], sp->logits_dev + b * 4672,
-                                    sp->values_dev + b, nullptr, sp->stream, err);
+                                    sp->values_dev + b, nullptr, sp->stream, err, sp->row_flags_dev ? sp->row_flags_dev + b : nullptr);
         m0_net_unlock(sp->nethandle_b);
         if (rc != M0_OK) { sp->hip.check(sp->net_b->hip()); m0_set_error(err); return rc; }
         rows += sp->rows2[1];
diff --git a/matrix0_amd/csrc/selfplay_engine.h b/matrix0_amd/csrc/selfplay_engine.h
--- a/matrix0_amd/csrc/selfplay_engine.h
+++ b/matrix0_amd/csrc/selfplay_engine.h
@@ -118,6 +118,7 @@
     std::vector<RootResult> hres;
     float* logits_dev = nullptr;
     float* values_dev = nullptr;
+    uint8_t* row_flags_dev = nullptr;
     float* ssl_dev = nullptr;
     m0::Pos* ssl_pos_dev = nullptr;
     float* ssl_out_dev = nullptr;
diff --git a/matrix0_amd/csrc/tree.h b/matrix0_amd/csrc/tree.h
--- a/matrix0_amd/csrc/tree.h
+++ b/matrix0_amd/csrc/tree.h
@@ -166,6 +166,7 @@
     _Float16* x0;
     const float* logits;
     const float* values;
+    const uint8_t* row_flags;
     int G;
     int L;
     const m0::TbSet* tb_set;
diff --git a/matrix0_amd/csrc/tree_expand.hip b/matrix0_amd/csrc/tree_expand.hip
--- a/matrix0_amd/csrc/tree_expand.hip
+++ b/matrix0_amd/csrc/tree_expand.hip
@@ -1,4 +1,5 @@
 #include "tree_device.h"
+#include "net_kernels.h"
 #include "tree_gumbel.h"
 #include "tree_proof.h"
 #include "eval_cache.h"
@@ -20,11 +21,14 @@
 };
 struct LeafLogits {
     const float* row;
+    const uint8_t* flag;
     const float* legal;
     float* store;
 };
-__device__ __forceinline__ LeafLogits logits_of_row(const float* row, float* store) { return LeafLogits{row, nullptr, store}; }
-__device__ __forceinline__ LeafLogits logits_of_cache(const float* payload) { return LeafLogits{nullptr, payload + EC_LOGITS, nullptr}; }
+__device__ __forceinline__ LeafLogits logits_of_row(const TreeDev& d, int row, float* store) {
+    return LeafLogits{d.logits + (size_t)row * M0_POLICY_SIZE, d.row_flags ? d.row_flags + row : nullptr, nullptr, store};
+}
+__device__ __forceinline__ LeafLogits logits_of_cache(const float* payload) { return LeafLogits{nullptr, nullptr, payload + EC_LOGITS, nullptr}; }
 
 static __device__ float np_sum_f32_dev(const float* a, int n) {
     auto block = [&](const float* b, int m) -> float {
@@ -214,7 +218,7 @@
     const int lane = E.lane;
     if (n <= 0) return true;
     bool bad = false;
-    if (!src.legal) bad = row_nonfinite(src.row, lane);
+    if (!src.legal) bad = src.flag ? *src.flag != 0 : row_nonfinite(src.row, lane);
     bad = __any(bad);
     if (lane == 0) E.X->bad = bad ? 1 : 0;
     float pr[CPL];
@@ -239,7 +243,7 @@
 }
 
 __device__ __forceinline__ bool expand_evaluated(const TreeDev& d, const TreeCfg& c, const ExpandEnv& E, int g, const Sample& smp,
-                                                 const uint16_t* moves, const float* lg, float v, double q0) {
+                                                 const uint16_t* moves, float v, double q0) {
     const Arena& A = E.A;
     GameDev* gd = E.gd;
     const int lane = E.lane, kind = smp.kind, leaf = smp.leaf;
@@ -252,7 +256,7 @@
         cw = ec_payload(d.ec, ce);
         ec_invalidate(d.ec, ce, lane);
     }
-    const bool ok = expand_node(E, c, leaf, pos, moves, smp.nlegal, logits_of_row(lg, cw), kind == SK_ROOT_INIT,
+    const bool ok = expand_node(E, c, leaf, pos, moves, smp.nlegal, logits_of_row(d, smp.row, cw), kind == SK_ROOT_INIT,
                                 !(kind == SK_ROOT_INIT && gd->root_fresh), q0);
     if (c.eval_cache && kind == SK_EVAL && lane == 0 && A.nch[leaf] < 0) A.cbase[leaf] = -1;
     const int sig = cw ? legal_sig(moves, smp.nlegal, lane) : 0;
@@ -262,15 +266,15 @@
     return ok;
 }
 
-__device__ __forceinline__ bool retry_refused_shared(const TreeCfg& c, const ExpandEnv& E, const Sample* S, int s, const uint16_t* LM,
-                                                     const float* logits, const int* path) {
+__device__ __forceinline__ bool retry_refused_shared(const TreeDev& d, const TreeCfg& c, const ExpandEnv& E, const Sample* S, int s,
+                                                     const uint16_t* LM, const int* path) {
     const int leaf = S[s].leaf, row = S[s].row;
     int s0 = 0;
     while (s0 < s && !(S[s0].kind == SK_EVAL && S[s0].row == row)) ++s0;
     if (s0 >= s) return true;
     const Pos pos = S[s].pos;
     return expand_node(E, c, leaf, pos, LM + (size_t)s0 * M0_MAX_CHILDREN, S[s].nlegal,
-                       logits_of_row(logits + (size_t)row * M0_POLICY_SIZE, nullptr), false, true,
+                       logits_of_row(d, row, nullptr), false, true,
                        child_seed_q(c, E.A, path, S[s].depth));
 }
 
@@ -322,7 +326,7 @@
             const float v = d.values[S[s].row];
             if (refused) {
                 __builtin_amdgcn_fence(__ATOMIC_SEQ_CST, "agent");
-                if (A.nch[S[s].leaf] < 0) retry_refused_shared(c, E, S, s, LM, d.logits, path);
+                if (A.nch[S[s].leaf] < 0) retry_refused_shared(d, c, E, S, s, LM, path);
             }
             backprop(A, path, S[s].depth, (double)v, lane, may_repeat, NoMirror{});
             ++sims; ++hits;
@@ -341,9 +345,8 @@
             __syncthreads();
         } else if (kind == SK_EVAL || kind == SK_ROOT_INIT) {
             const int leaf = S[s].leaf, depth = S[s].depth, row = S[s].row;
-            const float* lg = d.logits + (size_t)row * M0_POLICY_SIZE;
             const float v = d.values[row];
-            if (A.nch[leaf] < 0) refused |= !expand_evaluated(d, c, E, g, S[s], moves, lg, v, child_seed_q(c, A, path, depth));
+            if (A.nch[leaf] < 0) refused |= !expand_evaluated(d, c, E, g, S[s], moves, v, child_seed_q(c, A, path, depth));
             ++evals;
             if (kind == SK_EVAL) {
                 backprop(A, path, depth, (double)v, lane, may_repeat, NoMirror{});
@@ -386,3 +389,16 @@
     hipLaunchKernelGGL(expand_kernel, dim3(d.G), dim3(64), 0, st, d, c);
     return hipGetLastError();
 }
+
+__global__ __launch_bounds__(64) void logit_flags_kernel(const float* __restrict__ logits, uint8_t* __restrict__ flags, int rows) {
+    const int row = blockIdx.x, lane = threadIdx.x;
+    if (row >= rows) return;
+    const bool bad = __any(row_nonfinite(logits + (size_t)row * M0_POLICY_SIZE, lane));
+    if (lane == 0) flags[row] = bad ? 1 : 0;
+}
+
+hipError_t launch_logit_flags(const float* logits, uint8_t* flags, int rows, hipStream_t st) {
+    if (rows <= 0) return hipSuccess;
+    hipLaunchKernelGGL(logit_flags_kernel, dim3(rows), dim3(64), 0, st, logits, flags, rows);
+    return hipGetLastError();
+}
```
